# BauerLab/VARSCOT

Measured on AMD Instinct MI355X. Metric: guides/sec (candidate sites/sec alongside) at <=8 mismatches on a 3.0 Gbp reference, higher is better.
Workload: dtype u32

## Files before the change

### include/varscot_hip_debug.h

```cpp
#ifndef VARSCOT_HIP_DEBUG_H
#define VARSCOT_HIP_DEBUG_H

#include "varscot_hip.h"

#ifdef __cplusplus
extern "C" {
#endif

typedef struct {
    uint32_t seed_groups_per_cu;
    uint32_t seed_reserve;
    uint32_t sort_cap;
    uint32_t sort_max_bits;
    int32_t sort_xcd;
    uint32_t sort_debug;
    int32_t sort_optimistic;
    uint32_t sort_slot_cap;
    uint64_t score_chunk;
    int32_t score_slices;
    uint32_t score_slice_shift;
    int32_t seed_shared;
    int32_t seed_group_out;
    int32_t seed_tight;
    int32_t rf_form;
    uint32_t reserved[1];
} vsc_debug_params;

int vsc_ctx_set_debug_params(vsc_ctx *ctx, const vsc_debug_params *params);
int vsc_ctx_get_debug_params(const vsc_ctx *ctx, vsc_debug_params *out);

int vsc_ctx_create_masked(int device_id, const uint32_t *cu_mask, uint32_t n_words, vsc_ctx **out);

void vsc_debug_set_host_timing(int on);

typedef struct {
    int32_t rccl;
    const char *rccl_library;
} vsc_multi_debug_params;
int vsc_multi_create_debug(const int *device_ids, int n, const vsc_multi_debug_params *params, vsc_multi **out);

#ifdef __cplusplus
}
#endif
#endif
```

### varscot_amd/_lib.py

```python
import ctypes as C
import os

import numpy as np

_HERE = os.path.dirname(os.path.abspath(__file__))
LIB_PATH = os.environ.get("VSC_LIB_PATH") or os.path.join(_HERE, "libvarscot_hip.so")

VSC_OK = 0
ERRORS = {-22: "VSC_ERR_INVALID", -12: "VSC_ERR_NOMEM", -5: "VSC_ERR_DEVICE", -34: "VSC_ERR_RANGE",
          -19: "VSC_ERR_NODEVICE"}

HIT_DTYPE = np.dtype([("guide", "<u4"), ("contig", "<u4"), ("pos", "<u4"), ("info", "<u4")])
CONTIG_DTYPE = np.dtype([("offset", "<u8"), ("length", "<u4"), ("reserved", "<u4")])
N_FEATURES = 442
SUMMARY_DTYPE = np.dtype([("mit_sum", "<u8"), ("nm", "<u8", (9,)), ("mit_ub", "<u8"), ("on_target", "<u4"),
                          ("reserved", "<u4")])
assert SUMMARY_DTYPE.itemsize == 96
LOCUS_DTYPE = np.dtype([("contig", "<u4"), ("pos", "<u4"), ("strand", "<u4"), ("reserved", "<u4")])


class SearchParams(C.Structure):
    _fields_ = [("max_mismatches", C.c_uint32), ("has_extra_pam", C.c_uint8), ("extra_pam", C.c_char * 2),
                ("algorithm", C.c_uint8)]


ALGO_AUTO, ALGO_SCAN, ALGO_SEED = 0, 1, 2


class Select(C.Structure):
    _fields_ = [("top_k", C.c_uint32), ("min_score", C.c_uint32), ("reserved", C.c_uint32 * 2)]


SELECT = Select
assert C.sizeof(Select) == 16


class RfModel(C.Structure):
    _fields_ = [("n_trees", C.c_uint32), ("n_nodes", C.c_uint32), ("node_status", C.c_void_p), ("feature", C.c_void_p),
                ("left", C.c_void_p), ("right", C.c_void_p), ("split", C.c_void_p), ("node_class", C.c_void_p)]


class Timing(C.Structure):
    _fields_ = [("scan_ms", C.c_double), ("prep_ms", C.c_double), ("sort_ms", C.c_double),
                ("finalize_ms", C.c_double), ("score_ms", C.c_double), ("total_ms", C.c_double),
                ("index_ms", C.c_double), ("sites", C.c_uint64), ("pairs", C.c_uint64), ("hits", C.c_uint64),
                ("genome_bytes", C.c_uint64), ("passes", C.c_uint32), ("algorithm", C.c_uint32),
                ("sort_bytes", C.c_uint64), ("sort_levels", C.c_uint32), ("sort_bin_bits", C.c_uint32),
                ("read_passes", C.c_uint32), ("sort_fallbacks", C.c_uint32), ("list_entries", C.c_uint64), ("seed_cut", C.c_uint32),
                ("reserved", C.c_uint32)]

    def as_dict(self):
        return {k: getattr(self, k) for k, _ in self._fields_ if k != "reserved"}


class MultiTiming(C.Structure):
    _fields_ = [("search_wall_ms", C.c_double), ("search_ms_max", C.c_double), ("exchange_ms", C.c_double),
                ("merge_ms", C.c_double), ("total_ms", C.c_double), ("hits", C.c_uint64), ("exchanged_bytes", C.c_uint64),
                ("n_devices", C.c_uint32), ("used_rccl", C.c_uint32), ("score_ms_max", C.c_double), ("callback_ms", C.c_double),
                ("batches", C.c_uint32), ("reserved", C.c_uint32)]

    def as_dict(self):
        return {k: getattr(self, k) for k, _ in self._fields_ if k != "reserved"}


class MultiScore(C.Structure):
    _fields_ = [("mode", C.c_uint32), ("reserved", C.c_uint32), ("guide_activity", C.c_void_p), ("model", C.POINTER(RfModel))]


MULTI_SCORE_NONE, MULTI_SCORE_ROWS, MULTI_SCORE_VOTES = 0, 1, 2


class DebugParams(C.Structure):
    _fields_ = [("seed_groups_per_cu", C.c_uint32), ("seed_reserve", C.c_uint32), ("sort_cap", C.c_uint32),
                ("sort_max_bits", C.c_uint32), ("sort_xcd", C.c_int32), ("sort_debug", C.c_uint32),
                ("sort_optimistic", C.c_int32), ("sort_slot_cap", C.c_uint32), ("score_chunk", C.c_uint64),
                ("score_slices", C.c_int32), ("score_slice_shift", C.c_uint32), ("seed_shared", C.c_int32),
                ("seed_group_out", C.c_int32), ("seed_tight", C.c_int32), ("rf_form", C.c_int32),
                ("reserved", C.c_uint32 * 1)]
    SIGNED_DEFAULT = ("sort_xcd", "sort_optimistic", "score_slices", "seed_shared", "seed_group_out", "seed_tight", "rf_form")

    @classmethod
    def defaults(cls):
        d = cls()
        for k in cls.SIGNED_DEFAULT:
            setattr(d, k, -1)
        return d


class MultiDebugParams(C.Structure):
    _fields_ = [("rccl", C.c_int32), ("rccl_library", C.c_char_p)]


BATCH_FN = C.CFUNCTYPE(C.c_int, C.c_void_p, C.c_void_p, C.c_uint32, C.c_uint32)
ROWS_BATCH_FN = C.CFUNCTYPE(C.c_int, C.c_void_p, C.c_void_p, C.c_uint32, C.c_uint32, C.c_void_p)
MULTI_BATCH_FN = C.CFUNCTYPE(C.c_int, C.c_void_p, C.c_void_p, C.c_uint32, C.c_uint32, C.c_void_p)

_u32p = C.POINTER(C.c_uint32)
_vp = C.c_void_p
SYMBOLS = [
    ("vsc_abi_version", C.c_int, []),
    ("vsc_device_count", C.c_int, []),
    ("vsc_ctx_create", C.c_int, [C.c_int, C.POINTER(_vp)]),
    ("vsc_ctx_destroy", C.c_int, [_vp]),
    ("vsc_ctx_release_scratch", C.c_int, [_vp]),
    ("vsc_ctx_set_stream", C.c_int, [_vp, _vp]),
    ("vsc_last_error", C.c_char_p, [_vp]),
    ("vsc_ctx_timing", C.c_int, [_vp, C.POINTER(Timing)]),
    ("vsc_layout_contigs", C.c_uint64, [_vp, C.c_uint32, _vp]),
    ("vsc_planes_init", None, [_vp, _vp, _vp, C.c_uint64]),
    ("vsc_pack_bases", None, [C.c_char_p, C.c_uint64, C.c_uint64, _vp, _vp, _vp]),
    ("vsc_unpack_bases", None, [_vp, _vp, _vp, C.c_uint64, C.c_uint64, _vp]),
    ("vsc_pack_guide", C.c_uint64, [C.c_char_p]),
    ("vsc_genome_load", C.c_int, [_vp, _vp, _vp, _vp, C.c_uint64, C.c_uint64, C.c_uint64, _vp, C.c_uint32,
                                  C.POINTER(_vp)]),
    ("vsc_genome_free", C.c_int, [_vp]),
    ("vsc_genome_build_index", C.c_int, [_vp, _vp, C.POINTER(SearchParams)]),
    ("vsc_genome_index_save", C.c_int, [_vp, _vp, C.c_char_p]),
    ("vsc_genome_index_load", C.c_int, [_vp, _vp, C.c_char_p]),
    ("vsc_genome_device_bytes", C.c_uint64, [_vp]),
    ("vsc_search", C.c_int, [_vp, _vp, _vp, C.c_uint32, C.POINTER(SearchParams), C.POINTER(_vp)]),
    ("vsc_search_stream", C.c_int, [_vp, _vp, _vp, C.c_uint32, C.POINTER(SearchParams), C.c_uint32, BATCH_FN, _vp]),
    ("vsc_search_stream_rows", C.c_int, [_vp, _vp, _vp, C.c_uint32, C.POINTER(SearchParams), C.c_uint32, ROWS_BATCH_FN, _vp]),
    ("vsc_search_summary", C.c_int, [_vp, _vp, _vp, C.c_uint32, C.POINTER(SearchParams), _vp, _vp]),
    ("vsc_search_select", C.c_int, [_vp, _vp, _vp, C.c_uint32, C.POINTER(SearchParams), C.POINTER(Select), _vp, _vp, C.POINTER(_vp)]),
    ("vsc_mit_specificity", C.c_double, [C.c_uint64]),
    ("vsc_hits_count", C.c_uint64, [_vp]),
    ("vsc_hits_data_dev", _vp, [_vp]),
    ("vsc_hits_data", C.c_int, [_vp, C.POINTER(_vp)]),
    ("vsc_hits_copy", C.c_int, [_vp, _vp, C.c_int]),
    ("vsc_hits_merge", C.c_int, [_vp, _vp, C.c_int, _vp, C.c_uint32, C.c_uint32, C.POINTER(_vp)]),
    ("vsc_hits_pack_exchange", C.c_int, [_vp, _vp, _vp, C.c_uint32, _vp, C.c_int, _vp]),
    ("vsc_hits_merge_packed", C.c_int, [_vp, _vp, _vp, C.c_int, _vp, C.c_uint32, C.c_uint32, C.c_uint32, C.POINTER(_vp)]),
    ("vsc_hits_merge_packed_votes", C.c_int, [_vp, _vp, _vp, _vp, C.c_int, _vp, C.c_uint32, C.c_uint32, C.c_uint32, C.POINTER(_vp), _vp, C.c_int]),
    ("vsc_hits_free", C.c_int, [_vp]),
    ("vsc_score_hits", C.c_int, [_vp, _vp, _vp, _vp, C.c_uint32, C.c_uint64, C.c_uint64, _vp, _vp, _vp]),
    ("vsc_score_hits_packed", C.c_int, [_vp, _vp, _vp, _vp, C.c_uint32, C.c_uint64, C.c_uint64, _vp, _vp, _vp]),
    ("vsc_unpack_features", None, [_vp, C.c_uint64, _vp]),
    ("vsc_score_pairs", C.c_int, [_vp, _vp, _vp, _vp, C.c_uint64, _vp, _vp, _vp]),
    ("vsc_multi_create", C.c_int, [C.POINTER(C.c_int), C.c_int, C.POINTER(_vp)]),
    ("vsc_multi_destroy", C.c_int, [_vp]),
    ("vsc_multi_release_scratch", C.c_int, [_vp]),
    ("vsc_multi_size", C.c_int, [_vp]),
    ("vsc_multi_ctx", _vp, [_vp, C.c_int]),
    ("vsc_multi_result_ctx", _vp, [_vp]),
    ("vsc_multi_last_error", C.c_char_p, [_vp]),
    ("vsc_multi_uses_rccl", C.c_int, [_vp]),
    ("vsc_multi_get_timing", C.c_int, [_vp, C.POINTER(MultiTiming)]),
    ("vsc_multi_genome_load", C.c_int, [_vp, _vp, _vp, _vp, C.c_uint64, _vp, C.c_uint32, C.POINTER(_vp)]),
    ("vsc_multi_genome_free", C.c_int, [_vp]),
    ("vsc_multi_genome_build_index", C.c_int, [_vp, _vp, C.POINTER(SearchParams)]),
    ("vsc_multi_search", C.c_int, [_vp, _vp, _vp, C.c_uint32, C.POINTER(SearchParams), C.POINTER(_vp)]),
    ("vsc_multi_search_summary", C.c_int, [_vp, _vp, _vp, C.c_uint32, C.POINTER(SearchParams), _vp, _vp]),
    ("vsc_multi_search_select", C.c_int, [_vp, _vp, _vp, C.c_uint32, C.POINTER(SearchParams), C.POINTER(Select), _vp, _vp, C.POINTER(_vp)]),
    ("vsc_multi_search_stream", C.c_int, [_vp, _vp, _vp, C.c_uint32, C.POINTER(SearchParams), C.c_uint32, C.POINTER(MultiScore), MULTI_BATCH_FN, _vp]),
    ("vsc_windows_build", C.c_int, [C.c_char_p, C.c_uint32, C.c_uint32, C.c_uint32, _vp, _vp, _vp, _vp, _vp, C.c_uint32,
                                    C.POINTER(_vp), C.c_char_p, C.c_size_t]),
    ("vsc_windows_count", C.c_uint32, [_vp]),
    ("vsc_windows_words", C.c_uint64, [_vp]),
    ("vsc_windows_plane", _vp, [_vp, C.c_int]),
    ("vsc_windows_contigs", _vp, [_vp]),
    ("vsc_windows_name", _vp, [_vp, C.c_uint32, C.POINTER(C.c_uint32)]),
    ("vsc_windows_name_offsets", _vp, [_vp]),
    ("vsc_windows_free", None, [_vp]),
    ("vsc_rf_predict", C.c_int, [_vp, C.POINTER(RfModel), _vp, _vp, C.c_uint64, _vp, _vp, _vp]),
    ("vsc_rf_predict_packed", C.c_int, [_vp, C.POINTER(RfModel), _vp, C.c_int, _vp, C.c_uint64, _vp, _vp, _vp]),
    ("vsc_score_classify_hits", C.c_int, [_vp, _vp, _vp, _vp, C.c_uint32, _vp, C.POINTER(RfModel), C.c_uint64, C.c_uint64, _vp, _vp, _vp]),
    ("vsc_sam_order", None, [_vp, C.c_uint64, _vp, _vp]),
]
DEBUG_SYMBOLS = [
    ("vsc_ctx_set_debug_params", C.c_int, [_vp, C.POINTER(DebugParams)]),
    ("vsc_ctx_get_debug_params", C.c_int, [_vp, C.POINTER(DebugParams)]),
    ("vsc_debug_set_host_timing", None, [C.c_int]),
    ("vsc_ctx_create_masked", C.c_int, [C.c_int, _vp, C.c_uint32, C.POINTER(_vp)]),
    ("vsc_multi_create_debug", C.c_int, [C.POINTER(C.c_int), C.c_int, C.POINTER(MultiDebugParams), C.POINTER(_vp)]),
]

_lib = None


class VarscotError(RuntimeError):
    def __init__(self, code, message=""):
        self.code = code
        super().__init__("%s (%d)%s" % (ERRORS.get(code, "VSC_ERR"), code, ": " + message if message else ""))


def lib():
    global _lib
    if _lib is None:
        if not os.path.exists(LIB_PATH):
            raise ImportError(
                "libvarscot_hip.so is not built (%s). Build it with `make -C varscot_amd/csrc` or "
                "`python -c 'import __graft_entry__ as g; g.build()'`; there is no CPU fallback." % LIB_PATH)
        if os.environ.get("VSC_NO_TORCH_PRELOAD") != "1":
            try:
                import torch
            except ImportError:
                pass
        L = C.CDLL(LIB_PATH)
        for name, restype, argtypes in SYMBOLS + DEBUG_SYMBOLS:
            fn = getattr(L, name)
            fn.restype = restype
            fn.argtypes = argtypes
        _lib = L
    return _lib


def check(code, ctx=None):
    if code != VSC_OK:
        msg = ""
        if ctx:
            msg = lib().vsc_last_error(ctx).decode(errors="replace")
        raise VarscotError(code, msg)


def ptr(a):
    if a is None:
        return None
    assert a.flags["C_CONTIGUOUS"]
    return a.ctypes.data_as(C.c_void_p)
```

### varscot_amd/csrc/vsc_api.cpp

```cpp
#include <algorithm>
#include <atomic>
#include <chrono>
#include <cstdlib>
#include <cmath>
#include <cstdio>
#include <cstring>
#include <new>
#include <string>
#include <vector>

#include "vsc_internal.h"
#include "vsc_objects.h"

using namespace vsc;

namespace {

struct HostTimer {
    bool on = vsc::host_timing_on();
    std::chrono::steady_clock::time_point t0 = std::chrono::steady_clock::now();
    void lap(const char *what)
    {
        if (!on) return;
        auto t1 = std::chrono::steady_clock::now();
// ... 11 lines not shown

namespace {

int fail(vsc_ctx *ctx, int code, const char *what, hipError_t e = hipSuccess)
{
    if (ctx) {
        char buf[512];
        if (e != hipSuccess)
            std::snprintf(buf, sizeof buf, "%s: %s", what, hipGetErrorString(e));
        else
            std::snprintf(buf, sizeof buf, "%s", what);
        ctx->err = buf;
    }
    return code;
}

#define VSC_HIP(ctx, call)                                                 \
    do {                                                                   \
        hipError_t e_ = (call);                                            \
        if (e_ != hipSuccess) return fail((ctx), e_ == hipErrorOutOfMemory ? VSC_ERR_NOMEM : VSC_ERR_DEVICE, #call, e_); \
    } while (0)

hipError_t ensure_hl(vsc_ctx *ctx, const vsc_genome *genome)
{
    vsc_genome *g = const_cast<vsc_genome *>(genome);
    if (g->d_hl) return hipSuccess;
    hipError_t e = hipMalloc((void **)&g->d_hl, g->dev_words * sizeof(uint2));
    if (e != hipSuccess) return e;
    g->device_bytes += g->dev_words * sizeof(uint2);
    return launch_interleave(g->d_hi, g->d_lo, g->dev_words, g->d_hl, ctx->stream);
}

hipError_t take_records(vsc_ctx *ctx, vsc_hits *hits, uint64_t n)
{
    const size_t bytes = n * sizeof(vsc_hit);
    int best = -1;
    for (size_t i = 0; i < ctx->spare_records.size(); ++i)
        if (ctx->spare_records[i].cap >= bytes && (best < 0 || ctx->spare_records[i].cap < ctx->spare_records[best].cap))
            best = (int)i;
    if (best >= 0) {
        hits->storage = ctx->spare_records[best];
        ctx->spare_records.erase(ctx->spare_records.begin() + best);
    } else {
        for (auto &b : ctx->spare_records) b.release();
        ctx->spare_records.clear();
        hipError_t e = hits->storage.ensure(bytes);
        if (e != hipSuccess) return e;
    }
    hits->d_records = (vsc_hit *)hits->storage.p;
    return hipSuccess;
}

double hit_probability(unsigned m)
{
    double p = 0, c = 1;
    for (unsigned j = 0; j <= m && j <= 21; ++j) {
        if (j > 0) c = c * (21 - (j - 1)) / j;
        p += c * std::pow(0.75, (double)j) * std::pow(0.25, (double)(21 - j));
    }
    return p;
}

PamMasks pam_masks(int a, int b)
{
    PamMasks m;
    m.ah = (a & 2) ? 0xFFFFFFFFu : 0u;
    m.al = (a & 1) ? 0xFFFFFFFFu : 0u;
    m.bh = (b & 2) ? 0xFFFFFFFFu : 0u;
    m.bl = (b & 1) ? 0xFFFFFFFFu : 0u;
    return m;
}

int base_code(char c)
{
    switch (c) {
    case 'A': case 'a': return 0;
    case 'C': case 'c': return 1;
    case 'G': case 'g': return 2;
    case 'T': case 't': return 3;
    default: return 4;
    }
}

void guide_planes(uint64_t g, uint32_t *h, uint32_t *l)
{
    uint32_t hh = 0, ll = 0;
    for (int i = 0; i < VSC_READ_LEN; ++i) {
        const unsigned c = (unsigned)(g >> (2 * i)) & 3u;
        hh |= (c >> 1) << i;
        ll |= (c & 1u) << i;
    }
    *h = hh;
    *l = ll;
}

}

template <class F> int guarded(vsc_ctx *ctx, F &&body) noexcept
{
    try {
        return body();
    } catch (const std::bad_alloc &) {
        try {
            if (ctx) ctx->err = "out of host memory";
        } catch (...) {
        }
        return VSC_ERR_NOMEM;
    } catch (...) {
        try {
            if (ctx) ctx->err = "unexpected C++ exception";
        } catch (...) {
        }
        return VSC_ERR_DEVICE;
    }
}


extern "C" {

int vsc_abi_version(void) { return VSC_ABI_VERSION; }

int vsc_device_count(void)
{
    int n = 0;
    if (hipGetDeviceCount(&n) != hipSuccess) return 0;
    return n;
}

int vsc_ctx_create(int device_id, vsc_ctx **out) { return vsc_ctx_create_masked(device_id, nullptr, 0, out); }

int vsc_ctx_create_masked(int device_id, const uint32_t *cu_mask, uint32_t n_mask_words, vsc_ctx **out)
{
    if (!out) return VSC_ERR_INVALID;
    *out = nullptr;
    int n = 0;
    if (hipGetDeviceCount(&n) != hipSuccess || n <= 0) return VSC_ERR_NODEVICE;
    if (device_id < 0 || device_id >= n) return VSC_ERR_INVALID;
    vsc_ctx *ctx = new (std::nothrow) vsc_ctx();
    if (!ctx) return VSC_ERR_NOMEM;
    ctx->device = device_id;
    hipDeviceProp_t prop;
    if (hipSetDevice(device_id) != hipSuccess || hipGetDeviceProperties(&prop, device_id) != hipSuccess ||
        (cu_mask && n_mask_words ? hipExtStreamCreateWithCUMask(&ctx->stream, n_mask_words, cu_mask) : hipStreamCreate(&ctx->stream)) != hipSuccess) {
        delete ctx;
        return VSC_ERR_DEVICE;
    }
    ctx->own_stream = true;
    ctx->n_cus = prop.multiProcessorCount;
    for (auto &e : ctx->ev)
        if (hipEventCreate(&e) != hipSuccess) {
            vsc_ctx_destroy(ctx);
            return VSC_ERR_DEVICE;
        }
    *out = ctx;
    return VSC_OK;
}

int vsc_ctx_release_scratch(vsc_ctx *ctx)
{
    if (!ctx) return VSC_ERR_INVALID;
    (void)hipSetDevice(ctx->device);
    (void)hipStreamSynchronize(ctx->stream);
    for (DeviceBuf *b : {&ctx->counters, &ctx->guides, &ctx->score_guides, &ctx->keys_a, &ctx->keys_b, &ctx->vals_a, &ctx->vals_b,
                         &ctx->score_mit, &ctx->score_flags, &ctx->score_feat, &ctx->score_sched, &ctx->sort_segs, &ctx->sort_tabs,
                         &ctx->sort_over, &ctx->seed_off,
                         &ctx->seed_poff, &ctx->seed_lrest, &ctx->sum_rows, &ctx->sum_excl, &ctx->sel_hist, &ctx->sel_tabs, &ctx->sel_keys,
                         &ctx->sel_masks})
        b->release();
    for (auto &b : ctx->spare_records) b.release();
    ctx->spare_records.clear();
    ctx->forest.nodes.release();
    ctx->forest.ranks.release();
    ctx->forest.fingerprint = 0;
    return VSC_OK;
}

int vsc_ctx_destroy(vsc_ctx *ctx)
{
    if (!ctx) return VSC_OK;
    (void)vsc_ctx_release_scratch(ctx);
    for (auto &e : ctx->ev)
        if (e) (void)hipEventDestroy(e);
    if (ctx->own_stream && ctx->stream) (void)hipStreamDestroy(ctx->stream);
    delete ctx;
    return VSC_OK;
}

int vsc_ctx_set_stream(vsc_ctx *ctx, void *hip_stream)
{
    if (!ctx) return VSC_ERR_INVALID;
    if (ctx->own_stream && ctx->stream) {
        (void)hipStreamSynchronize(ctx->stream);
        (void)hipStreamDestroy(ctx->stream);
    }
    ctx->stream = (hipStream_t)hip_stream;
    ctx->own_stream = false;
    return VSC_OK;
}

const char *vsc_last_error(const vsc_ctx *ctx) { return ctx ? ctx->err.c_str() : "null context"; }

int vsc_ctx_set_debug_params(vsc_ctx *ctx, const vsc_debug_params *params)
{
    if (!ctx) return VSC_ERR_INVALID;
    ctx->dbg = params ? *params : default_debug_params();
    return VSC_OK;
}

int vsc_ctx_get_debug_params(const vsc_ctx *ctx, vsc_debug_params *out)
{
    if (!ctx || !out) return VSC_ERR_INVALID;
    *out = ctx->dbg;
    return VSC_OK;
}

void vsc_debug_set_host_timing(int on) { vsc::g_host_timing.store(on ? 1 : 0, std::memory_order_relaxed); }

int vsc_ctx_timing(const vsc_ctx *ctx, vsc_timing *out)
{
    if (!ctx || !out) return VSC_ERR_INVALID;
    *out = ctx->timing;
    return VSC_OK;
}

int vsc_genome_load(vsc_ctx *ctx, const uint32_t *hi, const uint32_t *lo, const uint32_t *nmask, uint64_t first_word,
                    uint64_t n_words, uint64_t own_words, const vsc_contig *contigs, uint32_t n_contigs,
                    vsc_genome **out)
{
    return guarded(ctx, [&]() -> int {
    if (!ctx || !out) return VSC_ERR_INVALID;
    *out = nullptr;
    ctx->err.clear();
    if (!hi || !lo || !nmask || !contigs || n_contigs == 0 || n_words == 0 || own_words == 0 || own_words > n_words)
        return fail(ctx, VSC_ERR_INVALID, "vsc_genome_load: null or empty argument");
    if (own_words < n_words && own_words % kTileWords != 0)
        return fail(ctx, VSC_ERR_INVALID, "vsc_genome_load: a shard followed by halo words must own a multiple of 64 words");
    const uint64_t n_tiles = (own_words + kTileWords - 1) / kTileWords;
    const uint64_t dev_words = std::max<uint64_t>(n_tiles * kTileWords, n_words) + kPadWords;
    if ((first_word + dev_words) * 32 >= (1ull << 32) - 4096)
        return fail(ctx, VSC_ERR_RANGE, "vsc_genome_load: genome exceeds the 32-bit position space (4 Gbases)");
    std::vector<uint32_t> off(n_contigs), end(n_contigs);
    for (uint32_t c = 0; c < n_contigs; ++c) {
        const uint64_t e = contigs[c].offset + contigs[c].length;
        if (e >= (1ull << 32) - 4096) return fail(ctx, VSC_ERR_RANGE, "vsc_genome_load: contig table exceeds 4 Gbases");
        if (c > 0 && contigs[c].offset < contigs[c - 1].offset + contigs[c - 1].length + 1)
            return fail(ctx, VSC_ERR_INVALID, "vsc_genome_load: contigs must be ascending and separated by >= 1 N position");
        off[c] = (uint32_t)contigs[c].offset;
        end[c] = (uint32_t)e;
    }
    VSC_HIP(ctx, hipSetDevice(ctx->device));
    vsc_genome *g = new (std::nothrow) vsc_genome();
    if (!g) return fail(ctx, VSC_ERR_NOMEM, "vsc_genome_load: out of host memory");
    g->ctx = ctx;
    g->first_word = first_word;
    g->own_words = own_words;
    g->dev_words = dev_words;
    g->n_tiles = (uint32_t)n_tiles;
    g->n_contigs = n_contigs;
    const size_t pb = dev_words * sizeof(uint32_t), cb = (size_t)n_contigs * sizeof(uint32_t);
    hipError_t e = hipSuccess;
    auto step = [&](hipError_t r) {
        if (e == hipSuccess) e = r;
    };
    step(hipMalloc((void **)&g->d_hi, pb));
    step(hipMalloc((void **)&g->d_lo, pb));
    step(hipMalloc((void **)&g->d_nm, pb));
    step(hipMalloc((void **)&g->d_contig_off, cb));
    step(hipMalloc((void **)&g->d_contig_end, cb));
    if (e == hipSuccess) {
        step(hipMemsetAsync(g->d_hi, 0, pb, ctx->stream));
        step(hipMemsetAsync(g->d_lo, 0, pb, ctx->stream));
        step(hipMemsetAsync(g->d_nm, 0xFF, pb, ctx->stream));
        step(hipMemcpyAsync(g->d_hi, hi, n_words * sizeof(uint32_t), hipMemcpyHostToDevice, ctx->stream));
        step(hipMemcpyAsync(g->d_lo, lo, n_words * sizeof(uint32_t), hipMemcpyHostToDevice, ctx->stream));
        step(hipMemcpyAsync(g->d_nm, nmask, n_words * sizeof(uint32_t), hipMemcpyHostToDevice, ctx->stream));
        step(hipMemcpyAsync(g->d_contig_off, off.data(), cb, hipMemcpyHostToDevice, ctx->stream));
        step(hipMemcpyAsync(g->d_contig_end, end.data(), cb, hipMemcpyHostToDevice, ctx->stream));
        step(hipStreamSynchronize(ctx->stream));
    }
    if (e != hipSuccess) {
        vsc_genome_free(g);
        return fail(ctx, e == hipErrorOutOfMemory ? VSC_ERR_NOMEM : VSC_ERR_DEVICE, "vsc_genome_load", e);
    }
    g->device_bytes = 3 * pb + 2 * cb;
    *out = g;
    return VSC_OK;
    });
}

}

int vsc::genome_table_only(vsc_ctx *ctx, const vsc_contig *contigs, uint32_t n_contigs, vsc_genome **out)
{
    if (!ctx || !out || !contigs || n_contigs == 0) return VSC_ERR_INVALID;
    *out = nullptr;
    std::vector<uint32_t> off(n_contigs), end(n_contigs);
    for (uint32_t c = 0; c < n_contigs; ++c) {
        off[c] = (uint32_t)contigs[c].offset;
        end[c] = (uint32_t)(contigs[c].offset + contigs[c].length);
    }
    VSC_HIP(ctx, hipSetDevice(ctx->device));
    vsc_genome *g = new (std::nothrow) vsc_genome();
    if (!g) return fail(ctx, VSC_ERR_NOMEM, "out of host memory");
    g->ctx = ctx;
    g->n_contigs = n_contigs;
    const size_t cb = (size_t)n_contigs * sizeof(uint32_t);
    hipError_t e = hipMalloc((void **)&g->d_contig_off, cb);
    if (e == hipSuccess) e = hipMalloc((void **)&g->d_contig_end, cb);
    if (e == hipSuccess) e = hipMemcpy(g->d_contig_off, off.data(), cb, hipMemcpyHostToDevice);
    if (e == hipSuccess) e = hipMemcpy(g->d_contig_end, end.data(), cb, hipMemcpyHostToDevice);
    if (e != hipSuccess) {
        vsc_genome_free(g);
        return fail(ctx, e == hipErrorOutOfMemory ? VSC_ERR_NOMEM : VSC_ERR_DEVICE, "contig table upload", e);
    }
    g->device_bytes = 2 * cb;
    *out = g;
    return VSC_OK;
}

extern "C" {

int vsc_genome_free(vsc_genome *g)
{
    if (!g) return VSC_OK;
    if (g->ctx) (void)hipSetDevice(g->ctx->device);
    for (void *p : {(void *)g->d_hi, (void *)g->d_lo, (void *)g->d_nm, (void *)g->d_contig_off, (void *)g->d_contig_end, (void *)g->d_hl,
                    (void *)g->d_ix_chunk_tab, (void *)g->d_ix_vert, (void *)g->d_ix_sites, (void *)g->d_ix_edge})
        if (p) (void)hipFree(p);
    delete g;
    return VSC_OK;
}

uint64_t vsc_genome_device_bytes(const vsc_genome *g) { return g ? g->device_bytes + g->index_bytes : 0; }

namespace {
// ... 392 lines not shown
        if (!why.empty()) return fail(ctx, VSC_ERR_RANGE, ("vsc_genome_build_index: " + why).c_str());
        return fail(ctx, e == hipErrorOutOfMemory ? VSC_ERR_NOMEM : VSC_ERR_DEVICE, "vsc_genome_build_index", e);
    }
    ctx->timing.index_ms = genome->index_ms;
    return VSC_OK;
    });
}

int vsc_genome_index_save(vsc_ctx *ctx, const vsc_genome *genome, const char *path)
{
    return guarded(ctx, [&]() -> int {
    if (!ctx || !genome || genome->ctx != ctx || !path) return VSC_ERR_INVALID;
    ctx->err.clear();
    if (!genome->has_index) return fail(ctx, VSC_ERR_INVALID, "vsc_genome_index_save: the genome has no seed index (vsc_genome_build_index)");
    VSC_HIP(ctx, hipSetDevice(ctx->device));
    IndexFileHeader h{};
    std::memcpy(h.magic, kIndexMagic, sizeof h.magic);
    h.abi = VSC_ABI_VERSION;
    h.seg_bases = kSegBases;
    h.sliced_chunk = kSlicedChunk;
    h.sliced_sites = kSlicedSites;
    h.layout = (uint8_t)kIndexLayout;
    h.sites = genome->index_sites;
    h.own_words = genome->own_words;
    h.vert_bytes = genome->ix_vert_bytes;
    h.edge_words = genome->ix_edge_words;
    h.chunks = genome->ix_chunks;
    h.n_contigs = genome->n_contigs;
    h.has_extra_pam = genome->index_has_extra_pam;
    h.extra_pam[0] = genome->index_extra_pam[0];
    h.extra_pam[1] = genome->index_extra_pam[1];
    VSC_HIP(ctx, genome_fingerprint(ctx, genome, &h.fingerprint));
    FileCloser fc{std::fopen(path, "wb")};
    if (!fc.f) return fail(ctx, VSC_ERR_INVALID, (std::string("vsc_genome_index_save: cannot write ") + path).c_str());
    bool ok = std::fwrite(&h, sizeof h, 1, fc.f) == 1;
    std::vector<char> host(kIndexIoChunk);
    const uint64_t S = genome->index_sites;
    if (ok) VSC_HIP(ctx, index_io(fc.f, genome->d_ix_sites, 3 * S * sizeof(uint2), true, host, &ok));
    if (ok) VSC_HIP(ctx, index_io(fc.f, genome->d_ix_edge, h.edge_words * sizeof(uint32_t), true, host, &ok));
    if (ok) VSC_HIP(ctx, index_io(fc.f, genome->d_ix_chunk_tab, (uint64_t)h.chunks * sizeof(uint4), true, host, &ok));
    if (ok) VSC_HIP(ctx, index_io(fc.f, genome->d_ix_vert, h.vert_bytes, true, host, &ok));
    if (ok) ok = std::fflush(fc.f) == 0;
    if (!ok) return fail(ctx, VSC_ERR_DEVICE, (std::string("vsc_genome_index_save: write to ") + path + " failed").c_str());
    return VSC_OK;
    });
}

int vsc_genome_index_load(vsc_ctx *ctx, vsc_genome *genome, const char *path)
{
    return guarded(ctx, [&]() -> int {
    if (!ctx || !genome || genome->ctx != ctx || !path) return VSC_ERR_INVALID;
    ctx->err.clear();
    VSC_HIP(ctx, hipSetDevice(ctx->device));
    const auto t0 = std::chrono::steady_clock::now();
    FileCloser fc{std::fopen(path, "rb")};
    if (!fc.f) return fail(ctx, VSC_ERR_INVALID, (std::string("vsc_genome_index_load: cannot read ") + path).c_str());
    IndexFileHeader h{};
    if (std::fread(&h, sizeof h, 1, fc.f) != 1 || std::memcmp(h.magic, kIndexMagic, sizeof h.magic) != 0)
        return fail(ctx, VSC_ERR_INVALID, (std::string("vsc_genome_index_load: ") + path + " is not a seed index file").c_str());
    if (h.abi != VSC_ABI_VERSION || h.seg_bases != (uint32_t)kSegBases || h.sliced_chunk != (uint32_t)kSlicedChunk ||
        h.sliced_sites != (uint32_t)kSlicedSites || h.layout != (uint8_t)kIndexLayout)
        return fail(ctx, VSC_ERR_INVALID, "vsc_genome_index_load: the file was written by another version of the library");
    uint64_t fp = 0;
    VSC_HIP(ctx, genome_fingerprint(ctx, genome, &fp));
    if (h.own_words != genome->own_words || h.n_contigs != genome->n_contigs || h.fingerprint != fp)
        return fail(ctx, VSC_ERR_INVALID, "vsc_genome_index_load: the file belongs to another genome");
    const uint64_t S = h.sites;
    if (3 * S >= (1ull << 32) || h.edge_words != (3 * S + 31) / 32 + 1 || h.vert_bytes % (kVertWords * sizeof(uint32_t)) != 0)
        return fail(ctx, VSC_ERR_INVALID, "vsc_genome_index_load: inconsistent header");
    {
        const long at = std::ftell(fc.f);
        const uint64_t want = (uint64_t)sizeof h + 3 * S * sizeof(uint2) + h.edge_words * sizeof(uint32_t) +
                              (uint64_t)h.chunks * sizeof(uint4) + h.vert_bytes;
        if (at < 0 || std::fseek(fc.f, 0, SEEK_END) != 0) return fail(ctx, VSC_ERR_INVALID, "vsc_genome_index_load: cannot seek in the file");
        const long size = std::ftell(fc.f);
        if (size < 0 || (uint64_t)size != want || std::fseek(fc.f, at, SEEK_SET) != 0)
            return fail(ctx, VSC_ERR_INVALID, (std::string("vsc_genome_index_load: ") + path + " is truncated or does not match its header").c_str());
    }
    free_index(genome);
    hipError_t e = hipSuccess;
    auto step = [&](hipError_t r) {
        if (e == hipSuccess) e = r;
    };
    const uint64_t sb = std::max<uint64_t>(3 * S, 1) * sizeof(uint2), eb = h.edge_words * sizeof(uint32_t);
    const uint64_t cb = std::max<uint64_t>(h.chunks, 1) * sizeof(uint4), vb = std::max<uint64_t>(h.vert_bytes, kVertWords * sizeof(uint32_t));
    step(hipMalloc((void **)&genome->d_ix_sites, sb));
    step(hipMalloc((void **)&genome->d_ix_edge, eb));
    step(hipMalloc((void **)&genome->d_ix_chunk_tab, cb));
    step(hipMalloc((void **)&genome->d_ix_vert, vb));
    bool ok = true;
    std::vector<char> host(kIndexIoChunk);
    if (e == hipSuccess) step(index_io(fc.f, genome->d_ix_sites, 3 * S * sizeof(uint2), false, host, &ok));
    if (e == hipSuccess && ok) step(index_io(fc.f, genome->d_ix_edge, eb, false, host, &ok));
    if (e == hipSuccess && ok) step(index_io(fc.f, genome->d_ix_chunk_tab, (uint64_t)h.chunks * sizeof(uint4), false, host, &ok));
    if (e == hipSuccess && ok) step(index_io(fc.f, genome->d_ix_vert, h.vert_bytes, false, host, &ok));
    if (e != hipSuccess || !ok) {
        free_index(genome);
        if (e != hipSuccess) return fail(ctx, e == hipErrorOutOfMemory ? VSC_ERR_NOMEM : VSC_ERR_DEVICE, "vsc_genome_index_load", e);
        return fail(ctx, VSC_ERR_INVALID, (std::string("vsc_genome_index_load: ") + path + " is truncated").c_str());
    }
    {
        std::vector<uint32_t> ctab((size_t)h.chunks * 4);
        if (h.chunks) VSC_HIP(ctx, hipMemcpy(ctab.data(), genome->d_ix_chunk_tab, ctab.size() * sizeof(uint32_t), hipMemcpyDeviceToHost));
        std::string why;
        if (!chunk_table_ok(ctab, S, h.vert_bytes, &why)) {
            free_index(genome);
            return fail(ctx, VSC_ERR_INVALID, (std::string("vsc_genome_index_load: ") + path + " is damaged (" + why + ")").c_str());
        }
        class_counts(genome, ctab);
    }
    genome->ix_chunks = h.chunks;
    genome->ix_vert_bytes = vb;
    genome->ix_edge_words = h.edge_words;
    genome->index_sites = S;
    genome->sites = S;
    genome->has_index = true;
    genome->index_has_extra_pam = h.has_extra_pam;
    genome->index_extra_pam[0] = h.extra_pam[0];
    genome->index_extra_pam[1] = h.extra_pam[1];
    genome->index_bytes = sb + eb + cb + vb;
    genome->index_ms = std::chrono::duration<double, std::milli>(std::chrono::steady_clock::now() - t0).count();
    ctx->timing.index_ms = genome->index_ms;
    return VSC_OK;
    });
}

}

namespace {

unsigned ceil_log2(uint64_t x)
{
    unsigned b = 0;
    while (b < 63 && (1ull << b) < x) ++b;
    return b;
}

struct SortRows {
    uint32_t *side_src = nullptr;
    DeviceBuf *side_other = nullptr;
    const uint2 *guides = nullptr;
    uint32_t guide_first = 0;
    uint4 *rows = nullptr;
    uint64_t rows_first = 0;
};

struct SortInfo {
    unsigned levels = 0;
    unsigned bin_bits = 0;
    uint64_t bytes = 0;
    unsigned slot_fallbacks = 0;
};

hipError_t bin_sort(vsc_ctx *ctx, const vsc_genome *genome, std::vector<SortSeg> segs, uint64_t *src, uint64_t *other,
                    unsigned key_bits, unsigned pos_pad, uint32_t pos_base, vsc_hit *out, hipEvent_t ev_sorted, SortInfo *info,
                    DeviceBuf *other_buf = nullptr, bool *slots = nullptr, const SortRows *rows = nullptr)
{
    uint32_t *side_src = rows ? rows->side_src : nullptr, *side_other = nullptr;
    hipStream_t st = ctx->stream;
    unsigned rem = key_bits;
    bool sorted_marked = false;
    const vsc_debug_params &dbg = ctx->dbg;
    uint64_t sort_cap = kSortCap;
    unsigned max_bits = kSortMaxBinBits;
    if (dbg.sort_cap) sort_cap = std::min<uint64_t>(kSortCap, std::max<uint32_t>(16, dbg.sort_cap));
    if (dbg.sort_max_bits) max_bits = std::min<unsigned>(kSortMaxBinBits, std::max<uint32_t>(1, dbg.sort_max_bits));
    uint64_t slot_cap = dbg.sort_slot_cap ? dbg.sort_slot_cap : (sort_cap + sort_cap / 4 + 15) / 16 * 16;
    slot_cap = std::max<uint64_t>(slot_cap, 16);
    for (unsigned level = 1; !segs.empty(); ++level) {
        if (level > 48) return hipErrorUnknown;
        uint64_t n_max = 0, n_all = 0;
        for (const SortSeg &s : segs) {
            n_max = std::max<uint64_t>(n_max, s.n_in);
            n_all += s.n_in;
        }
        unsigned bits = 0;
        if (n_max > sort_cap) {
            if (rem == 0) return hipErrorUnknown;
            const uint64_t want = std::max<uint64_t>(1, sort_cap * 7 / 10);
            bits = std::min<unsigned>({std::max(1u, ceil_log2((n_max + want - 1) / want)), max_bits, rem});
            while (bits > 1 && ((uint64_t)segs.size() << bits) > (1ull << 22)) --bits;
        }
        const size_t n_segs = segs.size();
        const size_t n_bins = n_segs << bits;
        bool use_slots = level == 1 && bits && slots && other_buf && (dbg.sort_optimistic == 1 || (dbg.sort_optimistic != 0 && *slots));
        if (level == 1 && bits && other_buf) {
            uint64_t span = 1;
            for (const SortSeg &sg : segs) span = std::max<uint64_t>(span, sg.out_off + sg.n_in);
            const uint64_t slot_records = (uint64_t)n_bins * slot_cap;
            if (use_slots && dbg.sort_optimistic != 1) {
                size_t free_b = 0, total_b = 0;
                if (hipMemGetInfo(&free_b, &total_b) != hipSuccess) free_b = 0;
                const uint64_t room = (uint64_t)free_b + other_buf->cap;
                const uint64_t slot_bytes = slot_records * (sizeof(uint64_t) + (rows ? sizeof(uint32_t) : 0));
                if (slot_records > 4 * n_all + (1ull << 20) || slot_bytes + (1ull << 30) > room + (rows ? rows->side_other->cap : 0)) {
                    use_slots = false;
                    *slots = false;
                }
            }
            hipError_t ge = other_buf->ensure((size_t)(use_slots ? std::max(slot_records, span) : span) * sizeof(uint64_t));
            if (ge == hipErrorOutOfMemory && use_slots) {
                (void)hipGetLastError();
                use_slots = false;
                *slots = false;
                ge = other_buf->ensure((size_t)span * sizeof(uint64_t));
            }
            if (ge != hipSuccess) return ge;
            other = (uint64_t *)other_buf->p;
            if (rows) {
                VSC_TRY(rows->side_other->ensure(other_buf->cap / sizeof(uint64_t) * sizeof(uint32_t)));
                side_other = (uint32_t *)rows->side_other->p;
            }
        }
        std::vector<uint32_t> &tile0 = ctx->host_tile0;
        tile0.assign(n_segs + 1, 0);
        uint64_t tiles = 0;
        for (size_t i = 0; i < n_segs; ++i) {
            tile0[i] = (uint32_t)tiles;
            tiles += (segs[i].n_in + kSortTile - 1) / kSortTile;
        }
        if (tiles >= (1ull << 31)) return hipErrorInvalidValue;
        tile0[n_segs] = (uint32_t)tiles;
        const size_t seg_bytes = (n_segs * sizeof(SortSeg) + 255) / 256 * 256;
        VSC_TRY(ctx->sort_segs.ensure(seg_bytes + tile0.size() * sizeof(uint32_t)));
        SortSeg *d_segs = (SortSeg *)ctx->sort_segs.p;
        uint32_t *d_tile0 = (uint32_t *)((char *)ctx->sort_segs.p + seg_bytes);
        ctx->host_segs = segs;
        VSC_TRY(hipMemcpyAsync(d_segs, ctx->host_segs.data(), n_segs * sizeof(SortSeg), hipMemcpyHostToDevice, st));
        VSC_TRY(hipMemcpyAsync(d_tile0, tile0.data(), tile0.size() * sizeof(uint32_t), hipMemcpyHostToDevice, st));
        VSC_TRY(ctx->sort_over.ensure(256 + n_bins * sizeof(SortSeg)));
        uint32_t *d_n_over = (uint32_t *)ctx->sort_over.p;
        if (bits) VSC_TRY(ctx->sort_tabs.ensure(3 * n_bins * sizeof(uint32_t)));
        uint32_t flags[3] = {0, 0, 0};
        for (;;) {
            if (dbg.sort_debug)
                std::fprintf(stderr, "[vsc sort] level %u: %zu segments, %llu records, largest %llu, %u bits (of %u left), cap %llu%s\n", level,
                             n_segs, (unsigned long long)n_all, (unsigned long long)n_max, bits, rem, (unsigned long long)sort_cap,
                             use_slots ? ", slot mode" : "");
            VSC_TRY(hipMemsetAsync(d_n_over, 0, 3 * sizeof(uint32_t), st));
            FinArgs f{};
            f.segs = d_segs;
            f.n_segs = (uint32_t)n_segs;
            f.src = src;
            f.side_src = side_src;
            if (rows) {
                f.guides = rows->guides;
                f.guide_first = rows->guide_first;
                f.rows = rows->rows;
                f.rows_first = rows->rows_first;
            }
            if (bits) {
                SortArgs a{};
                a.segs = d_segs;
                a.seg_tile0 = d_tile0;
                a.n_segs = (uint32_t)n_segs;
                a.n_tiles = (uint32_t)tiles;
                a.in = src;
                a.out = other;
                a.side_in = rows ? side_src : nullptr;
                a.side_out = rows ? side_other : nullptr;
                a.hist = (uint32_t *)ctx->sort_tabs.p;
                a.cursor = a.hist + n_bins;
                a.bin_start = a.cursor + n_bins;
                a.bin_bits = bits;
                a.bin_shift = kRecPosShift + pos_pad + rem - bits;
                if (dbg.sort_xcd != 0 && tiles >= 64) a.xcd_tiles = (uint32_t)((tiles + 7) / 8);
                if (use_slots) {
                    a.hist = a.cursor;
                    a.slot_cap = (uint32_t)slot_cap;
                    a.overflow = d_n_over + 2;
                    VSC_TRY(hipMemsetAsync(a.cursor, 0, n_bins * sizeof(uint32_t), st));
                    VSC_TRY(launch_bin_partition(a, st));
                    VSC_TRY(launch_bin_scan(a, st));
                } else {
                    VSC_TRY(hipMemsetAsync(a.hist, 0, n_bins * sizeof(uint32_t), st));
                    VSC_TRY(launch_bin_hist(a, st));
                    VSC_TRY(launch_bin_scan(a, st));
                    if (dbg.sort_debug >= 2) {
                        std::vector<uint32_t> h(n_bins);
                        VSC_TRY(hipMemcpyAsync(h.data(), a.hist, n_bins * sizeof(uint32_t), hipMemcpyDeviceToHost, st));
                        VSC_TRY(hipStreamSynchronize(st));
                        for (size_t i = 0; i < n_segs; ++i) {
                            std::vector<uint64_t> recs(segs[i].n_in);
                            VSC_TRY(hipMemcpy(recs.data(), src + segs[i].in_off, recs.size() * sizeof(uint64_t), hipMemcpyDeviceToHost));
                            std::vector<uint32_t> want((size_t)1 << bits, 0);
                            for (uint64_t r : recs) {
                                if (r >> 63) continue;
                                want[(r >> a.bin_shift) & (((uint64_t)1 << bits) - 1)]++;
                            }
                            for (size_t b = 0; b < want.size(); ++b)
                                if (want[b] != h[(i << bits) + b])
                                    std::fprintf(stderr, "[vsc sort]   seg %zu (in_off %llu n %u) bin %zu: device %u host %u\n", i,
                                                 (unsigned long long)segs[i].in_off, segs[i].n_in, b, h[(i << bits) + b], want[b]);
                        }
                    }
                    VSC_TRY(launch_bin_partition(a, st));
                }
                f.src = other;
                f.side_src = side_other;
                f.hist = a.hist;
                f.bin_start = a.bin_start;
                f.bin_bits = bits;
                f.slot_cap = a.slot_cap;
                f.overflow = a.overflow;
            }
            if (!sorted_marked && ev_sorted) {
                VSC_TRY(hipEventRecord(ev_sorted, st));
                sorted_marked = true;
            }
            const unsigned rem_after = rem - bits;
            f.sub_bits = std::min<unsigned>(rows ? kSortSubBitsRows : kSortSubBits, rem_after);
            f.sub_shift = kRecPosShift + pos_pad + rem_after - f.sub_bits;
            f.pos_pad = pos_pad;
            f.pos_base = pos_base;
            f.low_bits = rem_after - f.sub_bits;
            f.over = (SortSeg *)((char *)ctx->sort_over.p + 256);
            f.over_cap = (uint32_t)std::min<size_t>(n_bins, 0xFFFFFFFFu);
            f.n_over = d_n_over;
            f.cursor = d_n_over + 1;
            f.cap = (uint32_t)sort_cap;
            f.contig_off = genome->d_contig_off;
            f.n_contigs = genome->n_contigs;
            f.out = out;
            VSC_TRY(launch_bin_finalize(f, 2 * ctx->n_cus, st));
            if (bits) {
                VSC_TRY(hipMemcpyAsync(flags, d_n_over, sizeof flags, hipMemcpyDeviceToHost, st));
                VSC_TRY(hipStreamSynchronize(st));
                if (use_slots && flags[2]) {
                    use_slots = false;
                    *slots = false;
                    if (info) {
                        info->slot_fallbacks++;
                        info->bytes += 16 * n_all;
                    }
                    continue;
                }
            }
            if (info && bits) {
                if (info->levels == 0) info->bin_bits = bits;
                info->levels++;
                info->bytes += (use_slots ? 16 : 24) * n_all;
            }
            if (info) info->bytes += 24 * n_all;
            if (info && rows) info->bytes += (bits ? 8 : 0) * n_all + (4 + 12 + 64) * n_all;
            break;
        }
        if (!bits) break;
        rem -= bits;
        const uint32_t n_over = flags[0];
        if (n_over == 0) break;
        segs.resize(n_over);
        VSC_TRY(hipMemcpyAsync(segs.data(), (char *)ctx->sort_over.p + 256, (size_t)n_over * sizeof(SortSeg), hipMemcpyDeviceToHost, st));
        VSC_TRY(hipStreamSynchronize(st));
        std::swap(src, other);
        std::swap(side_src, side_other);
        if (rows && !side_other) {
            uint64_t span = 1;
            for (const SortSeg &sg : segs) span = std::max<uint64_t>(span, sg.out_off + sg.n_in);
            VSC_TRY(rows->side_other->ensure(span * sizeof(uint32_t)));
            side_other = (uint32_t *)rows->side_other->p;
        }
    }
    return hipSuccess;
}

hipError_t result_room(vsc_ctx *ctx, vsc_hits *hits, uint64_t used, uint64_t n, uint64_t projected)
{
    const uint64_t need = used + n;
    if (hits->storage.p && hits->storage.cap >= need * sizeof(vsc_hit)) return hipSuccess;
    if (used == 0) {
        if (hits->storage.p) {
            ctx->spare_records.push_back(hits->storage);
            hits->storage = DeviceBuf{};
        }
        VSC_TRY(take_records(ctx, hits, std::max(need, projected)));
        return hipSuccess;
    }
    DeviceBuf bigger;
    VSC_TRY(bigger.ensure(std::max(need, projected) * sizeof(vsc_hit)));
    hipError_t e = hipMemcpyAsync(bigger.p, hits->storage.p, used * sizeof(vsc_hit), hipMemcpyDeviceToDevice, ctx->stream);
    if (e == hipSuccess) e = hipStreamSynchronize(ctx->stream);
    if (e != hipSuccess) {
        bigger.release();
        return e;
    }
    hits->storage.release();
    hits->storage = bigger;
    hits->d_records = (vsc_hit *)bigger.p;
    return hipSuccess;
}

struct PassFound {
    HostTimer ht;
    int algo = 0, n_parts = 0;
    uint32_t max_mm = 0, guide_base = 0;
    uint64_t cap = 0, n = 0;
    std::vector<SortSeg> segs;
    unsigned key_bits = 0, pos_pad = 0;
    uint32_t pos_base = 0;
    bool bases = false;
    bool selected = false;
    std::vector<uint64_t> sel_off;
};

uint32_t neighbours(int k) { return k < 0 ? 0u : (k == 0 ? 1u : (k == 1 ? 22u : 211u)); }

SeedPlan seed_cut(const vsc_genome *genome, const uint32_t *gp, uint32_t n_guides, uint32_t m, int n_cus, const vsc_debug_params &dbg,
                  int *k2_max)
{
    SeedPlan plan{};
    plan.max_mm = m;
    ScanArgs pa{};
    vsc_search_params ip{};
    ip.has_extra_pam = genome->index_has_extra_pam;
    ip.extra_pam[0] = genome->index_extra_pam[0];
    ip.extra_pam[1] = genome->index_extra_pam[1];
    fill_pam(pa, &ip);
    plan.n_pam = pa.n_pam;
    plan.pam_codes = pam_code_set(pa);
    plan.tight = dbg.seed_tight != 0;
    if (!plan.tight) {
        plan.k0 = plan.k1 = m / kSegments;
        *k2_max = (int)plan.k0;
    } else {
        uint32_t left_reads[kSeedClasses][VSC_MAX_MISMATCHES + 1] = {};
        int left_max = -1;
        for (uint32_t i = 0; i < n_guides; ++i) {
            const uint32_t x = gp[2 * (size_t)i], l = gp[2 * (size_t)i + 1];
            const uint32_t mine = (((x >> 21) & 1u) << 3) | (((l >> 21) & 1u) << 2) | (((x >> 22) & 1u) << 1) | ((l >> 22) & 1u);
            for (uint32_t c = 0; c < plan.n_pam; ++c) {
                const uint32_t diff = mine ^ ((plan.pam_codes >> (4 * c)) & 15u);
                const uint32_t spent = ((diff & 12u) ? 1u : 0u) + ((diff & 3u) ? 1u : 0u);
                if (spent > m) continue;
                left_reads[c][m - spent]++;
                left_max = std::max(left_max, (int)(m - spent));
            }
        }
        double cost[9];
        double chunks_all = 0, sites_all = 0;
        uint64_t reads_any = 0;
        for (uint32_t c = 0; c < plan.n_pam; ++c) {
            chunks_all += (double)genome->ix_class_chunks[c] / kSegments;
            sites_all += (double)genome->ix_class_sites[c];
            uint64_t reads_c = 0;
            for (int left = 0; left <= (int)m; ++left) reads_c += left_reads[c][left];
            reads_any = std::max(reads_any, reads_c);
        }
        const double block_bytes = (double)kVertWords * 4 / kSlicedSites;
        for (int cut = 0; cut < 9; ++cut) {
            const int k0 = cut % 3, k1 = cut / 3;
            cost[cut] = -1;
            if (left_max - k0 - k1 - 2 > 2) continue;
            double bytes = 0, visits = 0;
            for (uint32_t c = 0; c < plan.n_pam; ++c) {
                double e2 = 0;
                for (int left = 0; left <= (int)m; ++left) e2 += (double)left_reads[c][left] * neighbours(left - k0 - k1 - 2);
                const double per_list = e2 / kBucketsPerSeg;
                bytes += (1.0 - std::exp(-per_list)) * (double)genome->ix_class_sites[c] * block_bytes;
                visits += per_list * (double)genome->ix_class_chunks[c] / kSegments;
            }
            for (int k : {k0, k1}) {
                const double per_list = (double)reads_any * neighbours(k) / kBucketsPerSeg;
                bytes += (1.0 - std::exp(-per_list)) * sites_all * block_bytes;
                visits += per_list * chunks_all;
            }
            cost[cut] = std::max(bytes / 4.2e12, visits * 215.0 / ((double)n_cus * 4 * 2.0e9));
        }
        int best = -1;
        for (int cut = 0; cut < 9; ++cut)
            if (cost[cut] >= 0 && (best < 0 || cost[cut] < cost[best])) best = cut;
        const int forced = dbg.seed_tight >= 1 ? dbg.seed_tight - 1 : -1;
        if (forced >= 0 && forced < 9 && cost[forced] >= 0) best = forced;
        if (best < 0) best = 4 * (int)(m ? (m - 1) / kSegments : 0u);
        plan.k0 = (uint32_t)(best % 3);
        plan.k1 = (uint32_t)(best / 3);
        *k2_max = std::min<int>(2, (int)m - (int)plan.k0 - (int)plan.k1 - 2);
    }
    plan.n_nbr = neighbours(std::max<int>(std::max<int>((int)plan.k0, (int)plan.k1), *k2_max));
    return plan;
}

hipError_t seed_plan(vsc_ctx *ctx, const vsc_genome *genome, const uint32_t *gp, uint32_t n_guides, const PassFound &f, SeedArgs &sa,
                     int *n_groups, bool *shared)
{
    int k2_max = 0;
    const SeedPlan plan = seed_cut(genome, gp, n_guides, f.max_mm, ctx->n_cus, ctx->dbg, &k2_max);
    const uint64_t n_pairs = (uint64_t)n_guides * (neighbours((int)plan.k0) + neighbours((int)plan.k1) + plan.n_pam * neighbours(k2_max));
    const uint64_t list_cap = n_pairs + (uint64_t)kLists * (kGuideUnroll - 1) + 2 * kGuideUnroll;
    VSC_TRY(ctx->seed_off.ensure((kLists + 1) * sizeof(uint32_t)));
    VSC_TRY(ctx->seed_poff.ensure((kLists + 1) * sizeof(uint32_t)));
    VSC_TRY(ctx->seed_lrest.ensure(list_cap * sizeof(uint2)));
    VSC_TRY(hipMemsetAsync(ctx->seed_lrest.p, 0xFF, list_cap * sizeof(uint2), ctx->stream));
    VSC_TRY(launch_seed_lists((const uint2 *)ctx->guides.p, n_guides, plan, (uint32_t *)ctx->seed_off.p, (uint32_t *)ctx->seed_poff.p,
                              (uint2 *)ctx->seed_lrest.p, ctx->stream));
    VSC_TRY(hipEventRecord(ctx->ev[7], ctx->stream));
    sa.chunk_tab = genome->d_ix_chunk_tab;
    sa.n_chunks = genome->ix_chunks;
    sa.vert = genome->d_ix_vert;
    sa.list_rest = (const uint2 *)ctx->seed_lrest.p;
    sa.sites = genome->d_ix_sites;
    sa.edge_bits = genome->d_ix_edge;
    sa.guides = (const uint2 *)ctx->guides.p;
    sa.poff = (const uint32_t *)ctx->seed_poff.p;
    sa.max_mm = f.max_mm;
    sa.k_half = f.max_mm / 2;
    sa.k_seg0 = plan.k0;
    sa.k_seg1 = plan.k1;
    sa.contig_end = genome->d_contig_end;
    sa.n_contigs = genome->n_contigs;
    sa.counters = (unsigned long long *)ctx->counters.p;
    sa.n_parts = (uint32_t)f.n_parts;
    uint32_t groups_per_cu = kSlicedWavesPerSimd;
    if (ctx->dbg.seed_groups_per_cu) groups_per_cu = ctx->dbg.seed_groups_per_cu;
    *shared = (uint64_t)n_guides * neighbours((int)std::max(plan.k0, plan.k1)) / kBucketsPerSeg >= 72;
    if (ctx->dbg.seed_shared >= 0) *shared = ctx->dbg.seed_shared == 1;
    const uint32_t n_grabs = (sa.n_chunks + kSlicedGrab - 1) / kSlicedGrab;
    const uint32_t n_waves_max = (uint32_t)ctx->n_cus * groups_per_cu * kWavesPerGroup;
    const uint32_t n_waves = std::max<uint32_t>(1, std::min<uint32_t>(n_waves_max, *shared ? n_grabs * kWavesPerGroup : n_grabs));
    *n_groups = (int)((n_waves + kWavesPerGroup - 1) / kWavesPerGroup);
    sa.group_out = *shared && ctx->dbg.seed_group_out != 0 ? 1u : 0u;
    const uint32_t owners = sa.group_out ? (uint32_t)*n_groups : (uint32_t)*n_groups * kWavesPerGroup;
    const uint64_t per_wave = f.cap / ((uint64_t)owners * 8 * f.n_parts);
    uint32_t want_reserve = (uint32_t)std::min<uint64_t>(f.n_parts > 8 ? (sa.group_out ? 1024 : 128) : 1024, std::max<uint64_t>(kWave, per_wave));
    if (ctx->dbg.seed_reserve) want_reserve = std::min<uint32_t>(1024, std::max<uint32_t>(kWave, ctx->dbg.seed_reserve));
    sa.reserve_log2 = 6;
    while ((2u << sa.reserve_log2) <= want_reserve) ++sa.reserve_log2;
    sa.reserve = 1u << sa.reserve_log2;
    sa.pos_pad = f.pos_pad;
    sa.pos_base = f.pos_base;
    uint64_t part_cap = f.cap / f.n_parts + f.cap / f.n_parts / 7 + 4096;
    part_cap = std::max<uint64_t>(part_cap, (uint64_t)(1.2 * genome->seen_rate[f.max_mm] * std::min<uint32_t>(n_guides, kRegionReads)) + 4096);
    sa.part_cap = part_cap + (uint64_t)owners * sa.reserve;
    return hipSuccess;
}

int find_pass(vsc_ctx *ctx, const vsc_genome *genome, const uint64_t *guides, uint32_t n_guides, uint32_t guide_base,
              const vsc_search_params *params, bool keep_bases, vsc_timing &t, PassFound &f)
{
    const int algo = (int)t.algorithm;
    const uint32_t m = params->max_mismatches;
    f.algo = algo;
    f.max_mm = m;
    f.guide_base = guide_base;
    f.bases = keep_bases;
    const uint32_t n_pad = (n_guides + kGuideUnroll - 1) / kGuideUnroll * kGuideUnroll;
    std::vector<uint32_t> gp((size_t)(n_pad + kGuideUnroll) * 2, 0xFFFFFFFFu);
    for (uint32_t i = 0; i < n_guides; ++i) guide_planes(guides[i], &gp[2 * (size_t)i], &gp[2 * (size_t)i + 1]);
    VSC_HIP(ctx, ctx->guides.ensure(gp.size() * sizeof(uint32_t)));
    VSC_HIP(ctx, ctx->counters.ensure(kCounterWords * sizeof(unsigned long long)));
    VSC_HIP(ctx, hipEventRecord(ctx->ev[0], ctx->stream));
    VSC_HIP(ctx, hipMemcpyAsync(ctx->guides.p, gp.data(), gp.size() * sizeof(uint32_t), hipMemcpyHostToDevice, ctx->stream));

    const double own_bases = (double)genome->n_tiles * kTileBases;
    const double sites_est = genome->sites ? (double)genome->sites : own_bases / 4;
    f.cap = (uint64_t)(1.5 * sites_est * n_guides * hit_probability(m)) + (1u << 20);
    const double seen_rate = genome->seen_rate[m];
    if (algo == VSC_ALGO_SCAN) f.cap = std::max<uint64_t>(f.cap, (uint64_t)(1.2 * seen_rate * n_guides) + 4096);
    unsigned long long cnt[kCntPart + 4 * kParts] = {};
    f.n_parts = (int)((n_guides + kRegionReads - 1) / kRegionReads);
    f.pos_base = (uint32_t)(genome->first_word * 32);
    const unsigned pos_bits = std::max(1u, ceil_log2((uint64_t)genome->dev_words * 32));
    f.pos_pad = pos_bits < 32 ? 32 - pos_bits : 0;
    f.key_bits = pos_bits + 1 + ceil_log2(std::min<uint32_t>(n_guides, kRegionReads));

    ScanArgs a{};
    SeedArgs sa{};
    int n_groups = 1;
    bool seed_shared = false;
    if (algo == VSC_ALGO_SCAN) {
        fill_pam(a, params);
        fill_genome(a, ctx, genome);
        a.guides = (const uint4 *)ctx->guides.p;
        a.n_guides_padded = n_pad;
        a.max_mm = m;
        a.k_half = m / 2;
        n_groups = scan_groups(ctx, a.n_tiles);
        t.genome_bytes += (uint64_t)genome->n_tiles * kTileWords * 3 * sizeof(uint32_t);
        VSC_HIP(ctx, hipEventRecord(ctx->ev[7], ctx->stream));
    } else {
        VSC_HIP(ctx, seed_plan(ctx, genome, gp.data(), n_guides, f, sa, &n_groups, &seed_shared));
        f.cap = sa.part_cap * f.n_parts;
    }

    f.ht.lap("prep enqueue");
    uint32_t list_total = 0;
    for (unsigned tries = 0;; ++tries) {
        if (algo == VSC_ALGO_SEED && (sa.part_cap >= (1ull << 32) - (1u << 20) || sa.part_cap >= ((uint64_t)sa.reserve << 20) - sa.reserve))
            return fail(ctx, VSC_ERR_RANGE, "vsc_search: more than 2^32 hits in a block of 64 reads");
        VSC_HIP(ctx, ctx->keys_a.ensure(f.cap * sizeof(uint64_t)));
        VSC_HIP(ctx, hipMemsetAsync(ctx->counters.p, 0, kCounterWords * sizeof(unsigned long long), ctx->stream));
        VSC_HIP(ctx, hipEventRecord(ctx->ev[1], ctx->stream));
        if (algo == VSC_ALGO_SCAN) {
            VSC_HIP(ctx, ctx->vals_a.ensure(f.cap * sizeof(uint32_t)));
            a.hit_keys = (uint64_t *)ctx->keys_a.p;
            a.hit_vals = (uint32_t *)ctx->vals_a.p;
            a.hit_cap = f.cap;
            VSC_HIP(ctx, launch_scan(a, n_groups, false, ctx->stream));
        } else {
            sa.hit_recs = (uint64_t *)ctx->keys_a.p;
            if (keep_bases) {
                VSC_HIP(ctx, ctx->vals_a.ensure(f.cap * sizeof(uint32_t)));
                sa.hit_side = (uint32_t *)ctx->vals_a.p;
            }
            VSC_HIP(ctx, launch_seed_sliced(sa, n_groups, seed_shared, ctx->stream));
        }
        VSC_HIP(ctx, hipEventRecord(ctx->ev[2], ctx->stream));
        VSC_HIP(ctx, hipMemcpyAsync(cnt, ctx->counters.p, sizeof cnt, hipMemcpyDeviceToHost, ctx->stream));
        if (algo == VSC_ALGO_SEED)
            VSC_HIP(ctx, hipMemcpyAsync(&list_total, (const uint32_t *)ctx->seed_poff.p + kLists, sizeof list_total, hipMemcpyDeviceToHost, ctx->stream));
        VSC_HIP(ctx, hipStreamSynchronize(ctx->stream));
        f.ht.lap("search kernel + sync");
        t.passes++;
        if (!cnt[kCntOverflow]) break;
        if (tries >= 2) return fail(ctx, VSC_ERR_DEVICE, "vsc_search: hit buffer overflowed repeatedly");
        if (algo == VSC_ALGO_SEED) {
            uint64_t need = 0;
            for (int q = 0; q < f.n_parts; ++q) need = std::max<uint64_t>(need, cnt[kCntPart + 4 * q] + cnt[kCntPart + 4 * q + 2]);
            sa.part_cap = need + (need >> 6) + 4096 + (uint64_t)(sa.group_out ? n_groups : n_groups * kWavesPerGroup) * sa.reserve;
            f.cap = sa.part_cap * f.n_parts;
        } else {
            f.cap = cnt[kCntHits] + (cnt[kCntHits] >> 6) + 4096;
        }
    }
    float ms = 0;
    VSC_HIP(ctx, hipEventElapsedTime(&ms, ctx->ev[0], ctx->ev[7]));
    t.prep_ms += ms;
    VSC_HIP(ctx, hipEventElapsedTime(&ms, ctx->ev[1], ctx->ev[2]));
    t.scan_ms += ms;

    if (algo == VSC_ALGO_SCAN) {
        genome->sites = cnt[kCntSites];
        t.sites = cnt[kCntSites];
        t.pairs += cnt[kCntSites] * n_guides;
        f.n = cnt[kCntHits];
        genome->seen_rate[m] = (double)f.n / n_guides;
        if (f.n >= (1ull << 32)) return fail(ctx, VSC_ERR_RANGE, "vsc_search: more than 2^32 hits in one scan pass (split the read set)");
        if (f.n > 0) f.segs.push_back(SortSeg{0, 0, 0, (uint32_t)f.n, guide_base});
    } else {
        t.list_entries = list_total;
        t.seed_cut = sa.k_seg0 | (sa.k_seg1 << 4);
        t.sites = genome->index_sites;
        t.pairs += cnt[kCntSites];
        t.genome_bytes += cnt[kCntVisited] * kVertWords * sizeof(uint32_t) / kSlicedSites;
        double fullest = 0;
        for (int q = 0; q < f.n_parts; ++q) {
            const uint64_t placed = cnt[kCntPart + 4 * q], real = placed - cnt[kCntPart + 4 * q + 1];
            fullest = std::max(fullest, (double)placed / std::min<uint32_t>(kRegionReads, n_guides - (uint32_t)q * kRegionReads));
            if (placed) f.segs.push_back(SortSeg{(uint64_t)q * sa.part_cap, (uint64_t)q * sa.part_cap, f.n, (uint32_t)placed,
                                                 guide_base + (uint32_t)q * kRegionReads});
            f.n += real;
        }
        genome->seen_rate[m] = fullest;
    }
    t.hits += f.n;
    return VSC_OK;
}

hipError_t end_pass(vsc_ctx *ctx, PassFound &f, const char *lap, vsc_timing &t)
{
    VSC_TRY(hipEventRecord(ctx->ev[4], ctx->stream));
    VSC_TRY(hipStreamSynchronize(ctx->stream));
    f.ht.lap(lap);
    float ms = 0;
    VSC_TRY(hipEventElapsedTime(&ms, ctx->ev[3], ctx->ev[4]));
    t.finalize_ms += ms;
    VSC_TRY(hipEventElapsedTime(&ms, ctx->ev[0], ctx->ev[4]));
    t.total_ms += ms;
    t.read_passes++;
    return hipSuccess;
}

int sort_pass(vsc_ctx *ctx, const vsc_genome *genome, PassFound &f, vsc_hits *hits, uint64_t used, uint64_t projected, vsc_timing &t)
{
    SortInfo info;
    if (f.n > 0) {
        uint64_t *src = (uint64_t *)ctx->keys_a.p, *other = nullptr;
        if (f.algo == VSC_ALGO_SCAN && !f.selected) {
            VSC_HIP(ctx, ctx->keys_b.ensure(f.cap * sizeof(uint64_t)));
            const unsigned bits0 = ceil_log2((uint64_t)f.n_parts);
            const size_t n_bins = (size_t)1 << bits0;
            VSC_HIP(ctx, ctx->sort_segs.ensure(512));
            VSC_HIP(ctx, ctx->sort_tabs.ensure(3 * n_bins * sizeof(uint32_t)));
            const uint32_t tile0[2] = {0u, (uint32_t)((f.n + kSortTile - 1) / kSortTile)};
            VSC_HIP(ctx, hipMemcpyAsync(ctx->sort_segs.p, f.segs.data(), sizeof(SortSeg), hipMemcpyHostToDevice, ctx->stream));
            VSC_HIP(ctx, hipMemcpyAsync((char *)ctx->sort_segs.p + 256, tile0, sizeof tile0, hipMemcpyHostToDevice, ctx->stream));
            SortArgs l0{};
            l0.segs = (const SortSeg *)ctx->sort_segs.p;
            l0.seg_tile0 = (const uint32_t *)((char *)ctx->sort_segs.p + 256);
            l0.n_segs = 1;
            l0.n_tiles = tile0[1];
            l0.pair_keys = (const uint64_t *)ctx->keys_a.p;
            l0.pair_vals = (const uint32_t *)ctx->vals_a.p;
            l0.out = (uint64_t *)ctx->keys_b.p;
            l0.hist = (uint32_t *)ctx->sort_tabs.p;
            l0.cursor = l0.hist + n_bins;
            l0.bin_start = l0.cursor + n_bins;
            l0.bin_bits = bits0;
            l0.bin_shift = kRecKeyBits;
            l0.pos_pad = f.pos_pad;
            l0.pos_base = f.pos_base;
            VSC_HIP(ctx, hipMemsetAsync(l0.hist, 0, n_bins * sizeof(uint32_t), ctx->stream));
            VSC_HIP(ctx, launch_bin_hist(l0, ctx->stream));
            VSC_HIP(ctx, launch_bin_scan(l0, ctx->stream));
            VSC_HIP(ctx, launch_bin_partition(l0, ctx->stream));
            std::vector<uint32_t> tabs(3 * n_bins);
            VSC_HIP(ctx, hipMemcpyAsync(tabs.data(), l0.hist, tabs.size() * sizeof(uint32_t), hipMemcpyDeviceToHost, ctx->stream));
            VSC_HIP(ctx, hipStreamSynchronize(ctx->stream));
            f.segs.clear();
            for (int q = 0; q < f.n_parts; ++q) {
                const uint32_t count = tabs[q], start = tabs[2 * n_bins + q];
                if (count) f.segs.push_back(SortSeg{start, start, start, count, f.guide_base + (uint32_t)q * kRegionReads});
            }
            src = (uint64_t *)ctx->keys_b.p;
            other = (uint64_t *)ctx->keys_a.p;
            info.bytes += 12 * f.n + 20 * f.n;
        }
        for (SortSeg &s : f.segs) s.final_off += used;
        f.ht.lap("sort buffers");
        VSC_HIP(ctx, result_room(ctx, hits, used, f.n, projected));
        f.ht.lap("record storage");
        bool *slots = f.algo == VSC_ALGO_SEED && !f.selected ? &genome->sort_slots_ok[f.max_mm] : nullptr;
        SortRows rows;
        if (f.bases) {
            if (ctx->score_feat.ensure(f.n * VSC_PACKED_FEATURE_BYTES) != hipSuccess) {
                (void)hipGetLastError();
                for (auto &b : ctx->spare_records) b.release();
                ctx->spare_records.clear();
                for (DeviceBuf *b : {&ctx->score_mit, &ctx->score_flags, &ctx->score_sched, &ctx->keys_b, &ctx->vals_b}) b->release();
                VSC_HIP(ctx, ctx->score_feat.ensure(f.n * VSC_PACKED_FEATURE_BYTES));
            }
            rows.side_src = (uint32_t *)ctx->vals_a.p;
            rows.side_other = &ctx->vals_b;
            rows.guides = (const uint2 *)ctx->guides.p;
            rows.guide_first = f.guide_base;
            rows.rows = (uint4 *)ctx->score_feat.p;
            rows.rows_first = used;
        }
        VSC_HIP(ctx, bin_sort(ctx, genome, std::move(f.segs), src, other, f.key_bits, f.pos_pad, f.pos_base, hits->d_records, ctx->ev[3],
                              &info, f.algo == VSC_ALGO_SEED || f.selected ? &ctx->keys_b : nullptr, slots, f.bases ? &rows : nullptr));
    } else {
        VSC_HIP(ctx, hipEventRecord(ctx->ev[3], ctx->stream));
    }
    VSC_HIP(ctx, end_pass(ctx, f, "sort + finalize + sync", t));
    float ms = 0;
    VSC_HIP(ctx, hipEventElapsedTime(&ms, ctx->ev[2], ctx->ev[3]));
    t.sort_ms += ms;
    t.sort_levels = std::max(t.sort_levels, info.levels);
    t.sort_bin_bits = std::max(t.sort_bin_bits, info.bin_bits);
    t.sort_bytes += info.bytes;
    t.sort_fallbacks += info.slot_fallbacks;
    return VSC_OK;
}

int summarize_pass(vsc_ctx *ctx, PassFound &f, bool excluded, vsc_timing &t, bool last = true)
{
    std::vector<SumSeg> ss;
    std::vector<uint32_t> tile0(1, 0);
    for (const SortSeg &sg : f.segs) {
        ss.push_back(SumSeg{sg.in_off, sg.n_in, sg.guide_base - f.guide_base});
        tile0.push_back(tile0.back() + (sg.n_in + kSumTile - 1) / kSumTile);
    }
    SummaryArgs a{};
    if (!ss.empty()) {
        const size_t tile0_at = (ss.size() * sizeof(SumSeg) + 255) / 256 * 256;
        VSC_HIP(ctx, ctx->sort_segs.ensure(tile0_at + tile0.size() * sizeof(uint32_t)));
        VSC_HIP(ctx, hipMemcpyAsync(ctx->sort_segs.p, ss.data(), ss.size() * sizeof(SumSeg), hipMemcpyHostToDevice, ctx->stream));
        VSC_HIP(ctx, hipMemcpyAsync((char *)ctx->sort_segs.p + tile0_at, tile0.data(), tile0.size() * sizeof(uint32_t),
                                    hipMemcpyHostToDevice, ctx->stream));
        a.recs = (const uint64_t *)ctx->keys_a.p;
        a.vals = f.algo == VSC_ALGO_SCAN ? (const uint32_t *)ctx->vals_a.p : nullptr;
        a.segs = (const SumSeg *)ctx->sort_segs.p;
        a.seg_tile0 = (const uint32_t *)((char *)ctx->sort_segs.p + tile0_at);
        a.n_segs = (uint32_t)ss.size();
        a.n_tiles = tile0.back();
        a.pos_pad = f.pos_pad;
        a.pos_base = f.pos_base;
        a.excl = excluded ? (const uint64_t *)ctx->sum_excl.p + f.guide_base : nullptr;
        a.out = (unsigned long long *)ctx->sum_rows.p + (size_t)f.guide_base * kSumWords;
    }
    VSC_HIP(ctx, hipEventRecord(ctx->ev[3], ctx->stream));
    VSC_HIP(ctx, launch_summary(a, ctx->stream));
    if (last) VSC_HIP(ctx, end_pass(ctx, f, "summary + sync", t));
    else VSC_HIP(ctx, hipStreamSynchronize(ctx->stream));
    return VSC_OK;
}

int select_pass(vsc_ctx *ctx, PassFound &f, uint32_t n_reads, const vsc_select &sel, bool excluded)
{
    f.selected = true;
    if (f.n == 0) return VSC_OK;
    hipStream_t st = ctx->stream;
    std::vector<SumSeg> ss;
    std::vector<uint32_t> tile0(1, 0);
    for (const SortSeg &sg : f.segs) {
        ss.push_back(SumSeg{sg.in_off, sg.n_in, sg.guide_base - f.guide_base});
        tile0.push_back(tile0.back() + (sg.n_in + kSumTile - 1) / kSumTile);
    }
    const size_t tile0_at = (ss.size() * sizeof(SumSeg) + 255) / 256 * 256;
    VSC_HIP(ctx, ctx->sort_segs.ensure(tile0_at + tile0.size() * sizeof(uint32_t)));
    VSC_HIP(ctx, hipMemcpyAsync(ctx->sort_segs.p, ss.data(), ss.size() * sizeof(SumSeg), hipMemcpyHostToDevice, st));
    VSC_HIP(ctx, hipMemcpyAsync((char *)ctx->sort_segs.p + tile0_at, tile0.data(), tile0.size() * sizeof(uint32_t), hipMemcpyHostToDevice, st));
    const size_t words = ((size_t)n_reads + 63) / 64 * 64;
    VSC_HIP(ctx, ctx->sel_tabs.ensure(4 * words * sizeof(uint32_t) + 2 * words * sizeof(uint64_t)));
    VSC_HIP(ctx, ctx->sel_hist.ensure((size_t)n_reads * kSelBins * sizeof(uint32_t)));
    VSC_HIP(ctx, ctx->vals_b.ensure((size_t)tile0.back() * kSumTile * sizeof(uint32_t)));
    SelectArgs a{};
    a.recs = (const uint64_t *)ctx->keys_a.p;
    a.vals = f.algo == VSC_ALGO_SCAN ? (const uint32_t *)ctx->vals_a.p : nullptr;
    a.segs = (const SumSeg *)ctx->sort_segs.p;
    a.seg_tile0 = (const uint32_t *)((char *)ctx->sort_segs.p + tile0_at);
    a.n_segs = (uint32_t)ss.size();
    a.n_tiles = tile0.back();
    a.pos_pad = f.pos_pad;
    a.pos_base = f.pos_base;
    a.excl = excluded ? (const uint64_t *)ctx->sum_excl.p + f.guide_base : nullptr;
    a.min_score = sel.min_score;
    a.top_k = sel.top_k;
    a.n_reads = n_reads;
    a.tiles_per_block = std::min<uint32_t>(kSelMaxTilesPerBlock, std::max<uint32_t>(kSelMinTilesPerBlock, a.n_tiles / (16u * (uint32_t)ctx->n_cus)));
    a.score = (uint32_t *)ctx->vals_b.p;
    a.hist = (uint32_t *)ctx->sel_hist.p;
    a.thr = (uint32_t *)ctx->sel_tabs.p;
    a.count = a.thr + words;
    a.cursor = a.count + words;
    a.thr_region = a.cursor + words;
    uint64_t *d_off = (uint64_t *)(a.thr_region + words);
    a.cand_off = d_off;
    a.surv_off = d_off + words;
    VSC_HIP(ctx, hipMemsetAsync(a.hist, 0, (size_t)n_reads * kSelBins * sizeof(uint32_t), st));
    VSC_HIP(ctx, hipMemsetAsync(a.cursor, 0, words * sizeof(uint32_t), st));
    VSC_HIP(ctx, hipMemsetAsync(a.thr_region, 0xFF, words * sizeof(uint32_t), st));
    VSC_HIP(ctx, launch_select_score(a, st));
    VSC_HIP(ctx, launch_select_threshold(a, st));
    std::vector<uint32_t> count(n_reads);
    VSC_HIP(ctx, hipMemcpyAsync(count.data(), a.count, (size_t)n_reads * sizeof(uint32_t), hipMemcpyDeviceToHost, st));
    VSC_HIP(ctx, hipStreamSynchronize(st));
    f.ht.lap("select: scores + thresholds + sync");
    f.sel_off.assign(2 * words, 0);
    uint64_t n_cand = 0, n_surv = 0;
    for (uint32_t i = 0; i < n_reads; ++i) {
        f.sel_off[i] = n_cand;
        f.sel_off[words + i] = n_surv;
        n_cand += count[i];
        n_surv += sel.top_k ? std::min<uint32_t>(count[i], sel.top_k) : count[i];
    }
    f.segs.clear();
    for (uint32_t q = 0; q * (uint32_t)kRegionReads < n_reads; ++q) {
        const uint64_t begin = f.sel_off[words + (size_t)q * kRegionReads];
        const uint32_t next = (q + 1) * (uint32_t)kRegionReads;
        const uint64_t end = next < n_reads ? f.sel_off[words + next] : n_surv;
        if (end - begin >= (1ull << 32)) return fail(ctx, VSC_ERR_RANGE, "vsc_search_select: more than 2^32 selected hits in a block of 64 reads");
        if (end > begin) f.segs.push_back(SortSeg{begin, begin, begin, (uint32_t)(end - begin), f.guide_base + q * (uint32_t)kRegionReads});
    }
    f.n = n_surv;
    f.cap = n_surv;
    if (n_surv == 0) return VSC_OK;
    VSC_HIP(ctx, ctx->sel_keys.ensure(n_cand * sizeof(uint64_t)));
    VSC_HIP(ctx, ctx->sel_masks.ensure(n_cand * sizeof(uint32_t)));
    a.cand_key = (uint64_t *)ctx->sel_keys.p;
    a.cand_mask = (uint32_t *)ctx->sel_masks.p;
    a.out = (uint64_t *)ctx->keys_a.p;
    VSC_HIP(ctx, hipMemcpyAsync(d_off, f.sel_off.data(), f.sel_off.size() * sizeof(uint64_t), hipMemcpyHostToDevice, st));
    VSC_HIP(ctx, launch_select_compact(a, st));
    VSC_HIP(ctx, launch_select_resolve(a, st));
    return VSC_OK;
}

int excluded_loci(vsc_ctx *ctx, const vsc_genome *genome, const vsc_locus *exclude, uint32_t n_guides, const char *who, std::vector<uint64_t> &excl)
{
    if (!exclude || !n_guides) return VSC_OK;
    std::vector<uint32_t> off(genome->n_contigs), end(genome->n_contigs);
    if (genome->n_contigs) {
        VSC_HIP(ctx, hipMemcpy(off.data(), genome->d_contig_off, off.size() * sizeof(uint32_t), hipMemcpyDeviceToHost));
        VSC_HIP(ctx, hipMemcpy(end.data(), genome->d_contig_end, end.size() * sizeof(uint32_t), hipMemcpyDeviceToHost));
    }
    excl.assign(n_guides, ~0ull);
    for (uint32_t i = 0; i < n_guides; ++i) {
        const vsc_locus &l = exclude[i];
        if (l.contig == UINT32_MAX) continue;
        if (l.contig >= genome->n_contigs || l.strand > 1)
            return fail(ctx, VSC_ERR_INVALID, (std::string(who) + ": excluded locus outside the genome's contigs or strands").c_str());
        if (l.pos >= end[l.contig] - off[l.contig]) continue;
        excl[i] = (uint64_t)l.strand << 32 | (off[l.contig] + l.pos);
    }
    return VSC_OK;
}

int upload_summary_state(vsc_ctx *ctx, uint32_t n_guides, bool rows, const std::vector<uint64_t> &excl)
{
    if (!n_guides) return VSC_OK;
    if (rows) {
        const size_t row_bytes = (size_t)n_guides * sizeof(vsc_guide_summary);
        VSC_HIP(ctx, ctx->sum_rows.ensure(row_bytes));
        VSC_HIP(ctx, hipMemsetAsync(ctx->sum_rows.p, 0, row_bytes, ctx->stream));
    }
    if (!excl.empty()) {
        VSC_HIP(ctx, ctx->sum_excl.ensure(excl.size() * sizeof(uint64_t)));
        VSC_HIP(ctx, hipMemcpyAsync(ctx->sum_excl.p, excl.data(), excl.size() * sizeof(uint64_t), hipMemcpyHostToDevice, ctx->stream));
    }
    return VSC_OK;
}

int search_setup(vsc_ctx *ctx, const vsc_genome *genome, const uint64_t *guides, uint32_t n_guides,
                 const vsc_search_params *params, const char *who, vsc_timing *t)
{
    ctx->err.clear();
    if (!genome || !params || (n_guides && !guides)) return fail(ctx, VSC_ERR_INVALID, (std::string(who) + ": null argument").c_str());
    if (genome->ctx != ctx) return fail(ctx, VSC_ERR_INVALID, (std::string(who) + ": genome belongs to another context").c_str());
    if (params->max_mismatches > VSC_MAX_MISMATCHES)
        return fail(ctx, VSC_ERR_INVALID, "Maximum number of mismatches must lie between 0 and 8.");
    if (params->algorithm > VSC_ALGO_SEED) return fail(ctx, VSC_ERR_INVALID, (std::string(who) + ": unknown algorithm").c_str());
    if (n_guides >= (1u << 31)) return fail(ctx, VSC_ERR_RANGE, (std::string(who) + ": too many reads").c_str());
    VSC_HIP(ctx, hipSetDevice(ctx->device));
    *t = vsc_timing{};
    t->index_ms = ctx->timing.index_ms;
    const double own_bases = (double)genome->n_tiles * kTileBases;
    int algo = params->algorithm;
    if (algo == VSC_ALGO_AUTO) {
        const bool worth_building = (double)n_guides * own_bases >= 2.0e10;
        algo = (index_matches(genome, params) || worth_building) ? VSC_ALGO_SEED : VSC_ALGO_SCAN;
    }
    if (n_guides && algo == VSC_ALGO_SEED && !index_matches(genome, params)) {
        std::string why;
        hipError_t e = build_index(ctx, const_cast<vsc_genome *>(genome), params, &why);
        if (e != hipSuccess) {
            if (params->algorithm == VSC_ALGO_SEED || why.empty())
                return fail(ctx, e == hipErrorOutOfMemory ? VSC_ERR_NOMEM : VSC_ERR_DEVICE,
                            why.empty() ? "vsc_search: building the seed index" : why.c_str(), why.empty() ? e : hipSuccess);
            algo = VSC_ALGO_SCAN;
        } else {
            t->index_ms = genome->index_ms;
        }
    }
    t->algorithm = (uint32_t)algo;
    return VSC_OK;
}

template <class Deliver>
int stream_batches(vsc_ctx *ctx, const vsc_genome *genome, const uint64_t *guides, uint32_t n_guides, const vsc_search_params *params,
                   uint32_t batch_reads, bool rows, const char *who, bool have_callback, Deliver &&deliver)
{
    return guarded(ctx, [&]() -> int {
    if (!ctx) return VSC_ERR_INVALID;
    vsc_timing t{};
    const int rc = search_setup(ctx, genome, guides, n_guides, params, who, &t);
    if (rc != VSC_OK) return rc;
    if (!have_callback) return fail(ctx, VSC_ERR_INVALID, (std::string(who) + ": null callback").c_str());
    if (batch_reads == 0 || batch_reads > (uint32_t)kMaxPassReads) batch_reads = kMaxPassReads;
    for (uint32_t first = 0; first < n_guides; first += batch_reads) {
        const uint32_t count = std::min<uint32_t>(batch_reads, n_guides - first);
        vsc_hits *hits = new (std::nothrow) vsc_hits();
        if (!hits) return fail(ctx, VSC_ERR_NOMEM, (std::string(who) + ": out of host memory").c_str());
        hits->ctx = ctx;
        PassFound f;
        int prc = find_pass(ctx, genome, guides + first, count, first, params, rows && t.algorithm == VSC_ALGO_SEED, t, f);
        if (prc == VSC_OK) prc = sort_pass(ctx, genome, f, hits, 0, 0, t);
        if (prc == VSC_OK) {
            hits->n = f.n;
            if (f.n == 0) hits->host_valid = true;
            ctx->timing = t;
            ctx->timing.score_ms = 0;
            prc = deliver(hits, first, count, t);
            if (prc != VSC_OK && ctx->err.empty()) ctx->err = std::string(who) + ": the batch callback failed";
        }
        vsc_hits_free(hits);
        if (prc != VSC_OK) return prc;
    }
    ctx->timing = t;
    return VSC_OK;
    });
}

}

extern "C" {

int vsc_search(vsc_ctx *ctx, const vsc_genome *genome, const uint64_t *guides, uint32_t n_guides,
               const vsc_search_params *params, vsc_hits **out)
{
    return guarded(ctx, [&]() -> int {
    if (!ctx || !out) return VSC_ERR_INVALID;
    *out = nullptr;
    vsc_timing t{};
    const int rc = search_setup(ctx, genome, guides, n_guides, params, "vsc_search", &t);
    if (rc != VSC_OK) return rc;
    vsc_hits *hits = new (std::nothrow) vsc_hits();
    if (!hits) return fail(ctx, VSC_ERR_NOMEM, "vsc_search: out of host memory");
    hits->ctx = ctx;
    uint64_t used = 0;
    for (uint32_t first = 0; first < n_guides; first += kMaxPassReads) {
        const uint32_t count = std::min<uint32_t>(kMaxPassReads, n_guides - first);
        const uint64_t projected = first ? (uint64_t)((double)used / first * n_guides * 1.02) + 4096 : 0;
        PassFound f;
        int prc = find_pass(ctx, genome, guides + first, count, first, params, false, t, f);
        if (prc == VSC_OK) prc = sort_pass(ctx, genome, f, hits, used, projected, t);
        if (prc != VSC_OK) {
            vsc_hits_free(hits);
            return prc;
        }
        used += f.n;
    }
    hits->n = used;
    if (used == 0) hits->host_valid = true;
    ctx->timing = t;
    *out = hits;
    return VSC_OK;
    });
}

int vsc_search_summary(vsc_ctx *ctx, const vsc_genome *genome, const uint64_t *guides, uint32_t n_guides,
                       const vsc_search_params *params, const vsc_locus *exclude, vsc_guide_summary *out)
{
    return guarded(ctx, [&]() -> int {
    if (!ctx) return VSC_ERR_INVALID;
    if (n_guides && !out) return fail(ctx, VSC_ERR_INVALID, "vsc_search_summary: null argument");
    vsc_timing t{};
    const int rc = search_setup(ctx, genome, guides, n_guides, params, "vsc_search_summary", &t);
    if (rc != VSC_OK) return rc;
    std::vector<uint64_t> excl;
    const int erc = excluded_loci(ctx, genome, exclude, n_guides, "vsc_search_summary", excl);
    if (erc != VSC_OK) return erc;
    const int urc = upload_summary_state(ctx, n_guides, true, excl);
    if (urc != VSC_OK) return urc;
    for (uint32_t first = 0; first < n_guides; first += kMaxPassReads) {
        const uint32_t count = std::min<uint32_t>(kMaxPassReads, n_guides - first);
        PassFound f;
        int prc = find_pass(ctx, genome, guides + first, count, first, params, false, t, f);
        if (prc == VSC_OK) prc = summarize_pass(ctx, f, !excl.empty(), t);
        if (prc != VSC_OK) return prc;
    }
    if (n_guides) {
        VSC_HIP(ctx, hipMemcpyAsync(out, ctx->sum_rows.p, (size_t)n_guides * sizeof(vsc_guide_summary), hipMemcpyDeviceToHost, ctx->stream));
        VSC_HIP(ctx, hipStreamSynchronize(ctx->stream));
    }
    ctx->timing = t;
    return VSC_OK;
    });
}

int vsc_search_select(vsc_ctx *ctx, const vsc_genome *genome, const uint64_t *guides, uint32_t n_guides,
                      const vsc_search_params *params, const vsc_select *select, const vsc_locus *exclude,
                      vsc_guide_summary *summary, vsc_hits **out)
{
    return guarded(ctx, [&]() -> int {
    if (!ctx || !out) return VSC_ERR_INVALID;
    *out = nullptr;
    vsc_timing t{};
    const int rc = search_setup(ctx, genome, guides, n_guides, params, "vsc_search_select", &t);
    if (rc != VSC_OK) return rc;
    if (!select) return fail(ctx, VSC_ERR_INVALID, "vsc_search_select: null argument");
    if (select->reserved[0] || select->reserved[1]) return fail(ctx, VSC_ERR_INVALID, "vsc_search_select: reserved fields must be 0");
    std::vector<uint64_t> excl;
    const int erc = excluded_loci(ctx, genome, exclude, n_guides, "vsc_search_select", excl);
    if (erc != VSC_OK) return erc;
    const int urc = upload_summary_state(ctx, n_guides, summary != nullptr, excl);
    if (urc != VSC_OK) return urc;
    const bool selecting = select->top_k || select->min_score || !excl.empty();
    vsc_hits *hits = new (std::nothrow) vsc_hits();
    if (!hits) return fail(ctx, VSC_ERR_NOMEM, "vsc_search_select: out of host memory");
    hits->ctx = ctx;
    uint64_t used = 0;
    for (uint32_t first = 0; first < n_guides; first += kMaxPassReads) {
        const uint32_t count = std::min<uint32_t>(kMaxPassReads, n_guides - first);
        const uint64_t projected = first ? (uint64_t)((double)used / first * n_guides * 1.02) + 4096 : 0;
        PassFound f;
        int prc = find_pass(ctx, genome, guides + first, count, first, params, false, t, f);
        if (prc == VSC_OK && summary) prc = summarize_pass(ctx, f, !excl.empty(), t, false);
        if (prc == VSC_OK && selecting) prc = select_pass(ctx, f, count, *select, !excl.empty());
        if (prc == VSC_OK) prc = sort_pass(ctx, genome, f, hits, used, projected, t);
        if (prc != VSC_OK) {
            vsc_hits_free(hits);
            return prc;
        }
        used += f.n;
    }
    if (summary && n_guides) {
        hipError_t e = hipMemcpyAsync(summary, ctx->sum_rows.p, (size_t)n_guides * sizeof(vsc_guide_summary), hipMemcpyDeviceToHost, ctx->stream);
        if (e == hipSuccess) e = hipStreamSynchronize(ctx->stream);
        if (e != hipSuccess) {
            vsc_hits_free(hits);
            VSC_HIP(ctx, e);
        }
    }
    hits->n = used;
    if (used == 0) hits->host_valid = true;
    ctx->timing = t;
    *out = hits;
    return VSC_OK;
    });
}

double vsc_mit_specificity(uint64_t mit_sum)
{
    return (100.0 / (100.0 + (double)mit_sum * 0x1p-24)) * 100.0;
}

int vsc_search_stream(vsc_ctx *ctx, const vsc_genome *genome, const uint64_t *guides, uint32_t n_guides,
                      const vsc_search_params *params, uint32_t batch_reads, vsc_batch_fn on_batch, void *user)
{
    return stream_batches(ctx, genome, guides, n_guides, params, batch_reads, false, "vsc_search_stream", on_batch != nullptr,
                          [&](vsc_hits *hits, uint32_t first, uint32_t count, vsc_timing &t) {
                              const int prc = on_batch(user, hits, first, count);
                              t.score_ms += ctx->timing.score_ms;
                              return prc;
                          });
}

int vsc_search_stream_rows(vsc_ctx *ctx, const vsc_genome *genome, const uint64_t *guides, uint32_t n_guides,
                           const vsc_search_params *params, uint32_t batch_reads, vsc_rows_batch_fn on_batch, void *user)
{
    return stream_batches(ctx, genome, guides, n_guides, params, batch_reads, true, "vsc_search_stream_rows", on_batch != nullptr,
                          [&](vsc_hits *hits, uint32_t first, uint32_t count, vsc_timing &t) {
                              if (hits->n && t.algorithm != VSC_ALGO_SEED) {
                                  int prc = vsc_score_hits_packed(ctx, genome, hits, guides, n_guides, 0, hits->n, nullptr, nullptr, nullptr);
                                  if (prc == VSC_OK && ctx->score_feat.cap < hits->n * VSC_PACKED_FEATURE_BYTES)
                                      prc = fail(ctx, VSC_ERR_NOMEM, "vsc_search_stream_rows: the batch's rows do not fit the device at once (smaller batches)");
                                  t.score_ms += ctx->timing.score_ms;
                                  if (prc != VSC_OK) return prc;
                              }
                              return on_batch(user, hits, first, count, hits->n ? ctx->score_feat.p : nullptr);
                          });
}

uint64_t vsc_hits_count(const vsc_hits *hits) { return hits ? hits->n : 0; }

const void *vsc_hits_data_dev(const vsc_hits *hits) { return hits ? hits->d_records : nullptr; }

int vsc_hits_data(vsc_hits *hits, const vsc_hit **out)
{
    return guarded(nullptr, [&]() -> int {
    if (!hits || !out) return VSC_ERR_INVALID;
    *out = nullptr;
    if (!hits->host_valid) {
        vsc_ctx *ctx = hits->ctx;
        try {
            hits->host.resize(hits->n);
        } catch (...) {
            return fail(ctx, VSC_ERR_NOMEM, "vsc_hits_data: out of host memory");
        }
        if (hits->n) {
            VSC_HIP(ctx, hipSetDevice(ctx->device));
            VSC_HIP(ctx, hipMemcpyAsync(hits->host.data(), hits->d_records, hits->n * sizeof(vsc_hit),
                                        hipMemcpyDeviceToHost, ctx->stream));
            VSC_HIP(ctx, hipStreamSynchronize(ctx->stream));
        }
        hits->host_valid = true;
    }
// ... 886 lines not shown
```

### varscot_amd/csrc/vsc_internal.h

```cpp
#pragma once

#include <hip/hip_runtime.h>
#include <stdint.h>

#include "varscot_hip.h"

namespace vsc {

constexpr int kWave = 64;
constexpr int kWavesPerGroup = 4;
constexpr int kSitesPerLane = 8;
constexpr int kBatch = kWave * kSitesPerLane;
constexpr int kQueueCap = kBatch + kWave;
constexpr int kHitCap = 128;
constexpr int kTileWords = kWave;
constexpr int kTileBases = kTileWords * 32;
constexpr int kChunkTiles = 8;
constexpr int kGuideUnroll = 4;
constexpr uint32_t kMask23 = 0x7FFFFFu;
constexpr int kSiteStrandBit = 23;
constexpr int kSiteEdgeBit = 24;
constexpr uint32_t kPadWords = 4;

constexpr int kSegments = 3;
constexpr int kSegBases = 7;
constexpr int kBucketsPerSeg = 1 << (2 * kSegBases);
constexpr int kBuckets = kSegments * kBucketsPerSeg;
constexpr int kSeedHitCap = 256;
constexpr int kSlicedSites = 32;
constexpr int kSlicedChunk = kWave * kSlicedSites;
constexpr int kRestBases = VSC_READ_LEN - kSegBases;
constexpr int kCmpBases = 2 * kSegBases;
constexpr int kVertWords = 2 * kCmpBases;
constexpr int kSeedClasses = 3;
constexpr int kLists = (kSegments - 1 + kSeedClasses) * kBucketsPerSeg;
constexpr int kListBudgetShift = 16;
constexpr uint32_t kListNoBudget = 15;
constexpr int kTokLaneShift = 26;
constexpr int kTokSlotShift = 14;
constexpr uint32_t kTokReadMask = (1u << kTokSlotShift) - 1u;
constexpr int kSlicedResolve = 3;
constexpr int kSlicedTokCap = 512;
constexpr uint32_t kChunkBucketMask = 0xFFFFu;
constexpr int kChunkMinusShift = 16;
constexpr int kChunkEdgeBit = 28;
constexpr int kChunkClassShift = 29;
constexpr uint32_t kIndexLayout = 2;
constexpr int kSlicedWavesPerSimd = 6;
constexpr int kSlicedGrab = 8;

enum { kCntHits = 0, kCntChunk = 1, kCntSites = 2, kCntOverflow = 3, kCntVisited = 4, kCntPad = 5, kCntLost = 6, kCntGroups = 7, kCntSlots = 8 };
constexpr int kRegionBits = 6;
constexpr int kRegionReads = 1 << kRegionBits;
constexpr int kParts = 256;
constexpr int kMaxPassReads = kParts * kRegionReads;
constexpr int kCntPart = 8;
constexpr int kCursors = 32;
constexpr int kCursorStride = 16;
constexpr int kCursorBase = kCntPart + 4 * kParts + 8;
constexpr int kCounterWords = kCursorBase + kCursors * kCursorStride;

constexpr int kRecPosShift = 23;
constexpr int kRecStrandShift = 55;
constexpr int kRecReadShift = 56;
constexpr int kRecKeyBits = 33 + kRegionBits;
constexpr uint64_t kRecSentinel = ~0ull;

constexpr int kSortThreads = 512;
constexpr int kSortItems = 16;
constexpr int kSortTile = kSortThreads * kSortItems;
constexpr int kFinThreads = 512;
constexpr int kFinItems = 16;
constexpr int kSortCap = kFinThreads * kFinItems - 128;
constexpr int kSortMaxBinBits = 11;
constexpr int kSortSubBits = 13;
constexpr int kSortSubBitsRows = 12;
constexpr int kHistTiles = 8;

struct PamMasks {
    uint32_t ah, al;
    uint32_t bh, bl;
};

struct ScanArgs {
    const uint32_t *hi, *lo, *nm;
    uint32_t first_pos;
    uint32_t n_tiles;
    const uint4 *guides;
    uint32_t n_guides_padded;
    uint32_t max_mm;
    uint32_t k_half;
    uint32_t n_pam;
    PamMasks pam[3];
    const uint32_t *contig_end;
    uint32_t n_contigs;
    uint64_t *hit_keys;
    uint32_t *hit_vals;
    unsigned long long hit_cap;
    unsigned long long *counters;
    uint32_t *site_x, *site_l, *site_pos;
};

struct SortSeg {
    uint64_t in_off;
    uint64_t out_off;
    uint64_t final_off;
    uint32_t n_in;
    uint32_t guide_base;
};

struct SortArgs {
    const SortSeg *segs;
    const uint32_t *seg_tile0;
    uint32_t n_segs, n_tiles;
    const uint64_t *in;
    const uint64_t *pair_keys;
    const uint32_t *pair_vals;
    uint64_t *out;
    const uint32_t *side_in;
    uint32_t *side_out;
    uint32_t *hist;
    uint32_t *cursor;
    uint32_t *bin_start;
    uint32_t bin_bits, bin_shift;
    uint32_t pos_pad;
    uint32_t pos_base;
    uint32_t xcd_tiles;
    uint32_t slot_cap;
    uint32_t *overflow;
};

struct FinArgs {
    const SortSeg *segs;
    uint32_t n_segs;
    const uint64_t *src;
    const uint32_t *hist;
    const uint32_t *bin_start;
    uint32_t bin_bits;
    uint32_t sub_shift, sub_bits;
    uint32_t low_bits;
    uint32_t pos_pad;
    uint32_t pos_base;
    SortSeg *over;
    uint32_t over_cap;
    uint32_t cap;
    uint32_t *n_over;
    uint32_t *cursor;
    const uint32_t *contig_off;
    uint32_t n_contigs;
    vsc_hit *out;
    uint32_t slot_cap;
    const uint32_t *overflow;
    const uint32_t *side_src;
    const uint2 *guides;
    uint32_t guide_first;
    uint4 *rows;
    uint64_t rows_first;
};

struct ScoreArgs {
    const vsc_hit *hits;
    uint64_t n;
    const uint2 *hl;
    uint32_t first_pos;
    uint64_t n_plane_words;
    const uint32_t *contig_off;
    const uint2 *guides;
    double *mit;
    uint8_t *mit_flags;
    uint8_t *features;
    const uint64_t *seg_prefix;
    const uint64_t *seg_start;
    uint32_t n_segs;
};

struct SeedPlan {
    uint32_t max_mm, k0, k1, tight;
    uint32_t n_nbr;
    uint32_t n_pam;
    uint32_t pam_codes;
};

struct SeedArgs {
    const uint4 *chunk_tab;
    const uint32_t *vert;
    const uint2 *list_rest;
    const uint2 *sites;
    const uint32_t *edge_bits;
    const uint2 *guides;
    uint32_t n_chunks;
    const uint32_t *poff;
    uint32_t max_mm, k_half;
    uint32_t k_seg0, k_seg1;
    const uint32_t *contig_end;
    uint32_t n_contigs;
    uint64_t *hit_recs;
    uint32_t *hit_side;
    uint32_t group_out;
    uint32_t reserve;
    uint32_t reserve_log2;
    uint32_t pos_pad;
    uint32_t pos_base;
    uint32_t n_parts;
    unsigned long long part_cap;
    unsigned long long *counters;
};

constexpr int kRfRows = 512;
constexpr int kRfMaxTests = 1024;
constexpr int kRfMaxNodes = 1024;
constexpr int kRfTileBytes = 26624;
constexpr int kRfPairFirstBit = 3;
constexpr int kRfPairMaxTests = 8 * (32 - kRfPairFirstBit);
constexpr int kRfPairBitsBytes = 16384;
constexpr int kRfPairTileBytes = 24512;
constexpr int kRfChains = 2;
constexpr int kRfRowWords = 20;
struct RfTest {
    uint8_t word, shift, width, thr;
    uint16_t dense_col;
    uint16_t pad;
};

struct RfArgs {
    const uint32_t *nodes;
    const uint8_t *depth;
    uint32_t n_trees, n_nodes;
    uint32_t compact;
    const RfTest *tests;
    const uint32_t *test_begin;
    uint32_t n_tests;
    const uint8_t *dense;
    const uint4 *packed;
    const uint8_t *act_rank;
    uint64_t n;
    uint32_t *votes;
    uint16_t *votes16;
    uint32_t tree_splits;
    ScoreArgs score;
};

constexpr int kSumWords = 12;
constexpr int kSumCounts = 11;
constexpr int kSumThreads = 256;
constexpr int kSumItems = 8;
constexpr int kSumTile = kSumThreads * kSumItems;
constexpr int kSumTilesPerBlock = 8;
constexpr int kSumCountBits = 7;

struct SumSeg {
    uint64_t in_off;
    uint32_t n;
    uint32_t first_read;
};

struct SummaryArgs {
    const uint64_t *recs;
    const uint32_t *vals;
    const SumSeg *segs;
    const uint32_t *seg_tile0;
    uint32_t n_segs, n_tiles;
    uint32_t pos_pad, pos_base;
    const uint64_t *excl;
    unsigned long long *out;
};

constexpr int kSelBins = 128;
constexpr int kSelThreads = 256;
constexpr int kSelMaxTilesPerBlock = 128;
constexpr int kSelMinTilesPerBlock = 8;
constexpr uint32_t kSelDropped = ~0u;
constexpr int kSelKeyPosBits = 33;

struct SelectArgs {
    const uint64_t *recs;
    const uint32_t *vals;
    const SumSeg *segs;
    const uint32_t *seg_tile0;
    uint32_t n_segs, n_tiles;
    uint32_t pos_pad, pos_base;
    const uint64_t *excl;
    uint32_t min_score;
    uint32_t top_k;
    uint32_t n_reads;
    uint32_t tiles_per_block;
    uint32_t *score;
    uint32_t *hist;
    uint32_t *thr;
    uint32_t *thr_region;
    uint32_t *count;
    uint32_t *cursor;
    const uint64_t *cand_off;
    const uint64_t *surv_off;
    uint64_t *cand_key;
    uint32_t *cand_mask;
    uint64_t *out;
};

hipError_t launch_scan(const ScanArgs &args, int n_groups, bool extract, hipStream_t stream);
hipError_t launch_summary(const SummaryArgs &args, hipStream_t stream);
hipError_t launch_select_score(const SelectArgs &args, hipStream_t stream);
hipError_t launch_select_threshold(const SelectArgs &args, hipStream_t stream);
hipError_t launch_select_compact(const SelectArgs &args, hipStream_t stream);
hipError_t launch_select_resolve(const SelectArgs &args, hipStream_t stream);
hipError_t launch_bin_hist(const SortArgs &args, hipStream_t stream);
hipError_t launch_bin_scan(const SortArgs &args, hipStream_t stream);
hipError_t launch_bin_partition(const SortArgs &args, hipStream_t stream);
hipError_t launch_bin_finalize(const FinArgs &args, int max_groups, hipStream_t stream);
hipError_t launch_rf_predict(const RfArgs &args, hipStream_t stream);
hipError_t launch_interleave(const uint32_t *hi, const uint32_t *lo, uint64_t n, uint2 *hl, hipStream_t stream);
hipError_t launch_score(const ScoreArgs &args, hipStream_t stream);
hipError_t launch_score_packed(const ScoreArgs &args, uint4 *packed, hipStream_t stream);
hipError_t launch_score_schedule(const ScoreArgs &args, uint32_t g_lo, uint32_t g_hi, uint32_t slice_shift, uint32_t n_slices,
                                 uint64_t *bounds, uint64_t *seg_start, uint64_t *seg_prefix, hipStream_t stream);
hipError_t launch_score_pairs(const uint2 *on, const uint2 *off, const uint32_t *masks, uint64_t n, double *mit,
                              uint8_t *mit_flags, uint8_t *features, hipStream_t stream);
hipError_t launch_xpack(const vsc_hit *in, uint64_t n, const uint32_t *contig_off, uint64_t *out, hipStream_t stream);
hipError_t launch_key_bounds(const vsc_hit *in, const uint64_t *range_dev, uint32_t K, uint64_t *bound, hipStream_t stream);
hipError_t launch_merge_packed(const uint64_t *seg_src, const uint64_t *seg_dst, const uint32_t *seg_n, uint32_t n_segs, uint32_t n_shards,
                               uint32_t first_key, const uint32_t *contig_off, const uint32_t *contig_end, uint32_t n_contigs, vsc_hit *out,
                               uint32_t *bad , const uint64_t *seg_side, uint16_t *side_out, hipStream_t stream);
hipError_t launch_plane_hash(const uint32_t *hi, const uint32_t *lo, const uint32_t *nm, uint64_t n_words, unsigned long long *out,
                             hipStream_t stream);
hipError_t launch_seed_keys(const uint4 *rec, uint64_t n, int seg, uint32_t pam_codes, uint32_t n_pam, uint64_t *sort_records, hipStream_t stream);
hipError_t launch_seed_lists(const uint2 *guides, uint32_t n_guides, const SeedPlan &plan, uint32_t *count, uint32_t *poff, uint2 *list_rest,
                             hipStream_t stream);
hipError_t launch_seed_pack16(const uint32_t *x, const uint32_t *l, const uint32_t *pos, uint64_t n, uint4 *rec, hipStream_t stream);
hipError_t launch_seed_gather16(const uint4 *rec, const uint64_t *sorted, uint64_t n, uint4 *out, hipStream_t stream);
hipError_t launch_seed_compact(const uint4 *sites16, uint64_t n_per_table, uint64_t n, uint2 *sites8, uint32_t *edge_bits,
                               hipStream_t stream);
hipError_t launch_seed_chunk_flags(uint4 *chunk_tab, uint32_t n_chunks, const uint32_t *edge_bits, hipStream_t stream);
hipError_t launch_seed_transpose(const uint4 *sites, const uint4 *chunk_tab, uint32_t n_chunks, uint32_t *vert,
                                 hipStream_t stream);
hipError_t launch_seed_sliced(const SeedArgs &args, int n_groups, bool shared, hipStream_t stream);
hipError_t launch_merge(const vsc_hit *in, const uint64_t *shard_off_dev, uint32_t n_shards, uint32_t K, uint64_t *bound,
                        uint64_t *key_off, vsc_hit *out, hipStream_t stream);

}
```

### varscot_amd/csrc/vsc_objects.h

```cpp
#pragma once

#include <string>
#include <vector>

#include "varscot_hip_debug.h"
#include "vsc_internal.h"

namespace vsc {

struct DeviceBuf {
    void *p = nullptr;
    size_t cap = 0;
    hipError_t ensure(size_t bytes)
    {
        if (bytes <= cap) return hipSuccess;
        if (p) (void)hipFree(p);
        p = nullptr;
        cap = 0;
        size_t want = bytes + (bytes < ((size_t)32 << 30) ? bytes / 8 : bytes / 32);
        hipError_t e = hipMalloc(&p, want);
        if (e != hipSuccess && want != bytes) {
            (void)hipGetLastError();
            want = bytes;
            e = hipMalloc(&p, want);
        }
        if (e == hipSuccess) cap = want;
        return e;
    }
    void release()
    {
        if (p) (void)hipFree(p);
        p = nullptr;
        cap = 0;
    }
};

inline vsc_debug_params default_debug_params()
{
    vsc_debug_params d{};
    d.sort_xcd = -1;
    d.sort_optimistic = -1;
    d.score_slices = -1;
    d.seed_shared = -1;
    d.seed_group_out = -1;
    d.seed_tight = -1;
    d.rf_form = -1;
    return d;
}

bool host_timing_on();

}

struct vsc_ctx {
    int device = 0;
    int n_cus = 0;
    hipStream_t stream = nullptr;
    bool own_stream = false;
    hipEvent_t ev[8] = {nullptr, nullptr, nullptr, nullptr, nullptr, nullptr, nullptr, nullptr};
    std::string err;
    vsc_timing timing{};
    vsc_debug_params dbg = vsc::default_debug_params();
    vsc::DeviceBuf counters, guides, keys_a, keys_b, vals_a, score_mit, score_flags, score_feat;
    vsc::DeviceBuf vals_b;
    vsc::DeviceBuf score_guides;
    uint64_t score_guides_hash = 0;
    uint32_t score_guides_n = ~0u;
    vsc::DeviceBuf sort_segs, sort_tabs, sort_over, score_sched;
    std::vector<vsc::SortSeg> host_segs;
    std::vector<uint32_t> host_tile0;
    vsc::DeviceBuf seed_off, seed_poff, seed_lrest;
    vsc::DeviceBuf sum_rows, sum_excl;
    vsc::DeviceBuf sel_hist, sel_tabs, sel_keys, sel_masks;
    struct Forest {
        vsc::DeviceBuf nodes, ranks;
        size_t depth_at = 0, tests_at = 0, begin_at = 0;
        uint32_t n_tests = 0, n_trees = 0, n_nodes = 0;
        uint32_t form = 0;
        uint32_t node_stride = 0;
        std::vector<double> thresholds;
        uint64_t fingerprint = 0;
        uint64_t ranks_key = 0;
        uint32_t ranks_n = ~0u;
    } forest;
    std::vector<vsc::DeviceBuf> spare_records;
};

struct vsc_genome {
    vsc_ctx *ctx = nullptr;
    uint32_t *d_hi = nullptr, *d_lo = nullptr, *d_nm = nullptr;
    uint32_t *d_contig_off = nullptr, *d_contig_end = nullptr;
    uint2 *d_hl = nullptr;
    uint64_t first_word = 0, own_words = 0, dev_words = 0;
    uint32_t n_tiles = 0, n_contigs = 0;
    uint64_t device_bytes = 0;
    mutable uint64_t sites = 0;
    mutable double seen_rate[VSC_MAX_MISMATCHES + 1] = {};
    mutable bool sort_slots_ok[VSC_MAX_MISMATCHES + 1] = {true, true, true, true, true, true, true, true, true};
    bool has_index = false;
    uint8_t index_has_extra_pam = 0;
    char index_extra_pam[2] = {0, 0};
    uint64_t index_sites = 0;
    uint4 *d_ix_chunk_tab = nullptr;
    uint32_t *d_ix_vert = nullptr;
    uint2 *d_ix_sites = nullptr;
    uint32_t *d_ix_edge = nullptr;
    uint32_t ix_chunks = 0;
    uint64_t ix_class_sites[4] = {};
    uint64_t ix_class_chunks[4] = {};
    uint64_t ix_vert_bytes = 0, ix_edge_words = 0;
    uint64_t index_bytes = 0;
    double index_ms = 0;
};

struct vsc_hits {
    vsc_ctx *ctx = nullptr;
    vsc_hit *d_records = nullptr;
    vsc::DeviceBuf storage;
    uint64_t n = 0;
    std::vector<vsc_hit> host;
    bool host_valid = false;
};


namespace vsc {
int genome_table_only(vsc_ctx *ctx, const vsc_contig *contigs, uint32_t n_contigs, vsc_genome **out);
int merge_packed_shards(vsc_ctx *ctx, const vsc_genome *genome, const void *const *shard_records, const void *const *shard_side,
                        const uint32_t *key_counts, uint32_t n_shards, uint32_t first_key, uint32_t n_keys, vsc_hits **out,
                        DeviceBuf *side_out);
}
```

### varscot_amd/csrc/vsc_seed.hip

```cpp
#include "vsc_internal.h"
#include "vsc_device.h"

#include <type_traits>

namespace vsc {

__device__ __forceinline__ uint32_t segment_key(uint32_t x, uint32_t l, int s)
{
    return (((x >> (kSegBases * s)) & 0x7Fu) << kSegBases) | ((l >> (kSegBases * s)) & 0x7Fu);
}

__device__ __forceinline__ uint32_t pam_code(uint32_t x, uint32_t l)
{
    return (((x >> 21) & 1u) << 3) | (((l >> 21) & 1u) << 2) | (((x >> 22) & 1u) << 1) | ((l >> 22) & 1u);
}

__global__ __launch_bounds__(256) void seed_key_kernel(const uint4 *rec, uint64_t n, int seg, uint32_t pam_codes, uint32_t n_pam, uint64_t *out)
{
    const uint64_t i = (uint64_t)blockIdx.x * blockDim.x + threadIdx.x;
    if (i >= n) return;
    const uint4 r = rec[i];
    const uint32_t code = pam_code(r.x, r.y);
    uint32_t cls = 0;
    for (uint32_t c = n_pam; c-- > 0;)
// ... 453 lines not shown

__device__ __forceinline__ uint32_t ring_slot(uint32_t p)
{
    return p & (uint32_t)(kSlicedTokCap - 1);
}

template <bool kFull>
__device__ __forceinline__ SlicedFetch sliced_fetch(const SeedArgs &a, const SeedWave &w, uint32_t head, uint32_t n)
{
    SlicedFetch f;
    if (!kFull) {
        f.word = 0;
        f.hi = 0;
        f.site0 = 0;
        f.gp = make_uint2(0u, 0u);
        f.rec = make_uint2(0u, 0u);
    }
    if (kFull || w.lane < n) {
        const uint2 tk = w.tok[ring_slot(head + w.lane)];
        f.word = tk.x;
        f.hi = tk.y;
        f.gp = a.guides[tk.y & kTokReadMask];
        f.site0 = w.first[(tk.y >> kTokSlotShift) & (uint32_t)(kSlicedGrab - 1)] + (tk.y >> kTokLaneShift) * kSlicedSites;
        f.rec = a.sites[f.site0 + (uint32_t)__builtin_ctz(tk.x)];
    }
    return f;
}

__device__ __forceinline__ uint32_t ring_tail(const SeedWave &w) { return ring_slot(w.thead + w.ntok); }

template <bool kFull>
__device__ __forceinline__ void sliced_consume(const SeedArgs &a, SeedWave &w, const SlicedFetch &f)
{
    bool hit = kFull || f.word != 0;
    const uint32_t rest = f.word & (f.word - 1);
    const uint64_t again = __ballot(rest != 0);
    if (again != 0) {
        if (rest != 0) w.tok[ring_slot(lanes_below(again, ring_tail(w)))] = make_uint2(rest, f.hi);
        w.ntok += (uint32_t)__popcll(again);
    }
    const uint32_t gid_of = f.hi & kTokReadMask;
    const uint32_t info = w.info[(f.hi >> kTokSlotShift) & (uint32_t)(kSlicedGrab - 1)];
    const uint32_t bucket = info & kChunkBucketMask;
    const uint32_t sh = (uint32_t)kSegBases * (bucket >> (2 * kSegBases));
    const uint32_t low = (1u << sh) - 1u;
    const uint32_t rest_hi = f.rec.x & 0xFFFFu, rest_lo = f.rec.x >> 16;
    const uint32_t site_hi = (rest_hi & low) | (((bucket >> kSegBases) & 0x7Fu) << sh) | ((rest_hi >> sh) << (sh + kSegBases));
    const uint32_t site_lo = (rest_lo & low) | ((bucket & 0x7Fu) << sh) | ((rest_lo >> sh) << (sh + kSegBases));
    const uint32_t t = ((site_hi ^ f.gp.x) | (site_lo ^ f.gp.y)) & kMask23;
    const uint32_t rank_in_chunk = (f.hi >> kTokLaneShift) * kSlicedSites + (uint32_t)__builtin_ctz(f.word | 0x80000000u);
    const uint32_t strand = rank_in_chunk >= ((info >> kChunkMinusShift) & 0xFFFu) ? 1u : 0u;
    const uint32_t pos = f.rec.y;
    const uint32_t mask = strand ? reverse23(t) : t;
    const bool maybe_edge = hit && ((info >> kChunkEdgeBit) & 1u) && (uint32_t)__popc(mask >> (VSC_READ_LEN / 2)) > a.k_half;
    if (__ballot(maybe_edge) != 0) {
        if (maybe_edge) {
            const uint32_t site = f.site0 + (uint32_t)__builtin_ctz(f.word);
            if (((a.edge_bits[site >> 5] >> (site & 31u)) & 1u) && is_contig_end(a.contig_end, a.n_contigs, pos + VSC_READ_LEN)) hit = false;
        }
    }
    const uint32_t low23 = a.hit_side ? (site_hi & kMask23) : mask;
    const uint64_t rec = ((uint64_t)(gid_of & (uint32_t)(kRegionReads - 1)) << kRecReadShift) | ((uint64_t)strand << kRecStrandShift) |
                         ((uint64_t)((pos - a.pos_base) << a.pos_pad) << kRecPosShift) | low23;
    sliced_store(a, w, hit, gid_of >> kRegionBits, rec, site_lo & kMask23);
}

template <bool kDrain>
__device__ __forceinline__ void sliced_resolve(const SeedArgs &a, SeedWave &w)
{
    wave_sync();
    bool have = false;
    SlicedFetch f = sliced_fetch<false>(a, w, 0, 0);
    for (;;) {
        uint32_t n = min(w.ntok, (uint32_t)kWave);
        if (!kDrain && n < (uint32_t)kWave) n = 0;
        if (n == 0 && !have) break;
        SlicedFetch nf = f;
        if (kDrain) nf = sliced_fetch<false>(a, w, w.thead, n);
        else if (n) nf = sliced_fetch<true>(a, w, w.thead, n);
        w.thead = ring_slot(w.thead + n);
        w.ntok -= n;
        if (have) sliced_consume<!kDrain>(a, w, f);
        wave_sync();
        f = nf;
        have = n != 0;
    }
    w.ntok = uniform(w.ntok);
    w.thead = uniform(w.thead);
}

__device__ __forceinline__ uint2 sliced_load_list(const SeedArgs &a, uint32_t g0, uint32_t g1, uint32_t lane)
{
    uint2 e = make_uint2(0xFFFFFFFFu, 0xFFFFFFFFu);
    if (g0 + lane < g1) e = a.list_rest[g0 + lane];
    return e;
}

__device__ __forceinline__ void sliced_load_sites(const SeedArgs &a, const v4u &ct, bool wanted, uint32_t lane,
                                                  uint32_t (&v)[kVertWords])
{
    const uint32_t nb = (ct.y + kSlicedSites - 1) / kSlicedSites;
    const bool mine = wanted && lane < nb;
    const uint4 *vp = (const uint4 *)(a.vert + (size_t)ct.w * kVertWords) + lane;
#pragma unroll
    for (int j = 0; j < kVertWords / 4; ++j) {
        uint4 x = make_uint4(0u, 0u, 0u, 0u);
        if (mine) x = vp[(size_t)j * nb];
        v[4 * j] = x.x;
        v[4 * j + 1] = x.y;
        v[4 * j + 2] = x.z;
        v[4 * j + 3] = x.w;
    }
}


static_assert(kMaxPassReads <= (1 << kTokSlotShift) && kSlicedGrab <= 8 && kTokSlotShift + 3 <= kTokLaneShift, "token fields");
static_assert((kSlicedTokCap & (kSlicedTokCap - 1)) == 0 && kSlicedTokCap >= (kSlicedResolve + kGuideUnroll) * kWave, "token ring");
template <bool kShared>
__global__ __launch_bounds__(kWave *kWavesPerGroup) __attribute__((amdgpu_waves_per_eu(kSlicedWavesPerSimd, kSlicedWavesPerSimd))) void seed_sliced_kernel(
    const SeedArgs a)
{
    __shared__ uint32_t s_grab[2];
    __shared__ uint2 s_tok[kWavesPerGroup][kSlicedTokCap];
    __shared__ uint2 s_list[kWavesPerGroup][kWave];
    __shared__ uint32_t s_parts[kWavesPerGroup][kParts];
    __shared__ uint32_t s_first[kWavesPerGroup][2 * kSlicedGrab];

    const uint32_t wave = threadIdx.x / kWave;
    SeedWave w;
    w.lane = threadIdx.x % kWave;
    w.tok = s_tok[wave];
    w.ntok = 0;
    w.thead = 0;
    w.parts = s_parts[kShared && a.group_out ? 0u : wave];
    w.first = s_first[wave];
    w.info = s_first[wave] + kSlicedGrab;
    for (uint32_t q = w.lane; q < (uint32_t)kParts; q += kWave) w.parts[q] = a.reserve;

    uint2 *const lt = s_list[wave];
    uint32_t kv[4];
#pragma unroll
    for (int i = 0; i < 4; ++i) asm volatile("v_mov_b32 %0, %1" : "=v"(kv[i]) : "s"(spread(i < 2 ? a.k_seg0 : a.k_seg1, i & 1)));
    const const_v4u_ptr ctab = (const_v4u_ptr)(uintptr_t)a.chunk_tab;
    const const_u32_ptr poff = (const_u32_ptr)(uintptr_t)a.poff;
    const const_v8u_ptr lgrp = (const_v8u_ptr)(uintptr_t)a.list_rest;
    constexpr bool kScalarLists = kShared;
    auto list_of = [](uint32_t z) {
        const uint32_t bucket = z & kChunkBucketMask;
        return bucket + (bucket >= 2u * kBucketsPerSeg ? ((z >> kChunkClassShift) & 3u) * (uint32_t)kBucketsPerSeg : 0u);
    };
    const uint32_t lane_tag = w.lane << kTokLaneShift;
    unsigned long long pairs = 0, visited = 0;

    const uint32_t slice_len = (a.n_chunks + kCursors - 1) / kCursors;
    uint32_t slice = uniform((kShared ? blockIdx.x : blockIdx.x * kWavesPerGroup + wave) % kCursors), exhausted = 0;
    const uint32_t wave_u = uniform(wave);
    for (uint32_t iter = 0;; ++iter) {
        uint32_t off = 0;
        if (kShared) {
            if (threadIdx.x == 0)
                s_grab[iter & 1u] = (uint32_t)atomicAdd(&a.counters[kCursorBase + slice * kCursorStride], (unsigned long long)kSlicedGrab);
            block_sync();
            off = s_grab[iter & 1u];
        } else if (w.lane == 0) {
            off = (uint32_t)atomicAdd(&a.counters[kCursorBase + slice * kCursorStride], (unsigned long long)kSlicedGrab);
        }
        off = uniform(off);
        const uint32_t slice_begin = slice * slice_len, slice_end = min(slice_begin + slice_len, a.n_chunks);
        if (slice_begin + off >= slice_end) {
            if (++exhausted == (uint32_t)kCursors) break;
            slice = (slice + 1) % kCursors;
            continue;
        }
        const uint32_t first = slice_begin + off;
        const uint32_t last = min(first + (uint32_t)kSlicedGrab, slice_end);
        auto my_part = [&](uint32_t g0, uint32_t g1, uint32_t r, uint32_t &q0, uint32_t &q1) {
            if (!kShared) {
                q0 = g0;
                q1 = g1;
                return;
            }
            const uint32_t n4 = (g1 - g0) / (uint32_t)kGuideUnroll;
            const uint32_t base = n4 / (uint32_t)kWavesPerGroup, rem = n4 % (uint32_t)kWavesPerGroup;
            q0 = g0 + (r * base + min(r, rem)) * (uint32_t)kGuideUnroll;
            q1 = q0 + (base + (r < rem ? 1u : 0u)) * (uint32_t)kGuideUnroll;
        };
        v4u t0 = ctab[first];
        v4u t1 = ctab[min(first + 1, last - 1)];
        uint32_t p0a, p0b;
        my_part(poff[list_of(t0.z)], poff[list_of(t0.z) + 1], wave_u, p0a, p0b);
        uint2 nl = make_uint2(0u, 0u);
        v8u ng = {};
        if (kScalarLists) ng = lgrp[(p0a < p0b ? p0a : 0u) / (uint32_t)kGuideUnroll];
        else nl = sliced_load_list(a, p0a, p0b, w.lane);
        uint32_t p1a = poff[list_of(t1.z)], p1b = poff[list_of(t1.z) + 1];
        v4u t2 = ctab[min(first + 2, last - 1)];
        for (uint32_t c = first; c < last; ++c) {
            const v4u cur = t0;
            const uint32_t g0 = p0a, g1 = p0b;
            uint32_t v[kVertWords];
            sliced_load_sites(a, cur, g0 != g1, w.lane, v);
            t0 = t1;
            my_part(p1a, p1b, (wave_u + (c + 1 - first)) % (uint32_t)kWavesPerGroup, p0a, p0b);
            uint2 tile = nl;
            v8u grp = ng;
            if (kScalarLists) ng = lgrp[(p0a < p0b && c + 1 < last ? p0a : 0u) / (uint32_t)kGuideUnroll];
            else nl = sliced_load_list(a, p0a, c + 1 < last ? p0b : p0a, w.lane);
            t1 = t2;
            p1a = poff[list_of(t1.z)];
            p1b = poff[list_of(t1.z) + 1];
            t2 = ctab[min(c + 3, last - 1)];
            if (g0 == g1) continue;
            const uint32_t slot_tag = (c - first) << kTokSlotShift;
            if (w.lane == 0) {
                w.first[c - first] = cur.x;
                w.info[c - first] = cur.z;
            }
            wave_sync();
            const uint32_t seg = uniform((cur.z & kChunkBucketMask) / (uint32_t)kBucketsPerSeg);
            const uint32_t budget_field = uniform((kListBudgetShift + 4u * ((cur.z >> kChunkClassShift) & 3u)) | (4u << 16));
            const int32_t left = (int32_t)cur.y - (int32_t)(w.lane * kSlicedSites);
            const uint32_t valid = left >= kSlicedSites ? 0xFFFFFFFFu : (left > 0 ? (1u << left) - 1u : 0u);
            pairs += (unsigned long long)cur.y * (g1 - g0);
            if (!kShared || (wave_u + (c - first)) % (uint32_t)kWavesPerGroup == 0) visited += cur.y;
            auto compare_four = [&](const uint32_t (&ex)[kGuideUnroll], const uint32_t (&ey)[kGuideUnroll]) {
                const uint32_t tail0 = uniform(w.thead + w.ntok);
                uint32_t tail = tail0;
                auto compare_group = [&](auto segment) {
                    constexpr uint32_t kSeg = decltype(segment)::value;
#pragma unroll
                    for (int u = 0; u < kGuideUnroll; ++u) {
                        const uint32_t ry = ey[u];
                        uint32_t budget;
                        asm("s_bfe_u32 %0, %1, %2" : "=s"(budget) : "s"(ry), "s"(budget_field) : "scc");
                        if (budget == kListNoBudget) continue;
                        const uint32_t word = sliced_within<kSeg>(v, ex[u], budget, valid, kv);
                        const uint64_t b = __ballot(word != 0);
                        if (b == 0) continue;
                        const uint32_t gid = ry & kTokReadMask;
                        if (word != 0) w.tok[ring_slot(lanes_below(b, tail))] = make_uint2(word, gid | slot_tag | lane_tag);
                        const uint32_t cnt = (uint32_t)__popcll(b);
                        const uint32_t tail_was = tail;
                        uint32_t tail_now;
                        asm("s_add_i32 %0, %1, %2" : "=s"(tail_now) : "s"(tail_was), "s"(cnt) : "scc");
                        tail = tail_now;
                    }
                };
                if (seg == 0) compare_group(std::integral_constant<uint32_t, 0>{});
                else if (seg == 1) compare_group(std::integral_constant<uint32_t, 1>{});
                else compare_group(std::integral_constant<uint32_t, 2>{});
                w.ntok += tail - tail0;
                if (w.ntok >= (uint32_t)kSlicedResolve * kWave) sliced_resolve<false>(a, w);
            };
            if (kScalarLists) {
                for (uint32_t gi = g0; gi < g1; gi += kGuideUnroll) {
                    const v8u e = grp;
                    grp = lgrp[(gi + kGuideUnroll < g1 ? gi + kGuideUnroll : gi) / (uint32_t)kGuideUnroll];
                    const uint32_t ex[kGuideUnroll] = {e[0], e[2], e[4], e[6]}, ey[kGuideUnroll] = {e[1], e[3], e[5], e[7]};
                    compare_four(ex, ey);
                }
                continue;
            }
            for (uint32_t tg = g0; tg < g1; tg += kWave) {
                wave_sync();
                lt[w.lane] = tile;
                wave_sync();
                if (tg + kWave < g1) tile = sliced_load_list(a, tg + kWave, g1, w.lane);
                const uint32_t in_tile = min(g1 - tg, (uint32_t)kWave);
                for (uint32_t gi = 0; gi < in_tile; gi += kGuideUnroll) {
                    uint2 rd[kGuideUnroll];
#pragma unroll
                    for (int u = 0; u < kGuideUnroll; ++u) rd[u] = lt[gi + u];
                    uint32_t ex[kGuideUnroll], ey[kGuideUnroll];
#pragma unroll
                    for (int u = 0; u < kGuideUnroll; ++u) {
                        ex[u] = uniform(rd[u].x);
                        ey[u] = uniform(rd[u].y);
                    }
                    compare_four(ex, ey);
                }
            }
        }
        if (w.ntok) sliced_resolve<true>(a, w);
    }
    if (kShared && a.group_out) {
        block_sync();
        sliced_finish_hits(a, w, wave_u, kWavesPerGroup);
    } else {
        sliced_finish_hits(a, w, 0, 1);
    }
    if (w.lane == 0 && pairs) {
        atomicAdd(&a.counters[kCntSites], pairs);
        atomicAdd(&a.counters[kCntVisited], visited);
    }
}

hipError_t launch_seed_sliced(const SeedArgs &args, int n_groups, bool shared, hipStream_t stream)
{
    const dim3 grid(n_groups), block(kWave * kWavesPerGroup);
    if (shared) hipLaunchKernelGGL((seed_sliced_kernel<true>), grid, block, 0, stream, args);
    else hipLaunchKernelGGL((seed_sliced_kernel<false>), grid, block, 0, stream, args);
    return hipGetLastError();
}

}
```

### varscot_amd/csrc/vsc_sort.hip

```cpp
#include "vsc_internal.h"
#include "vsc_device.h"

namespace vsc {

namespace {

constexpr int kLaneRun = 2;
__device__ __forceinline__ uint32_t tile_record(int k, uint32_t t)
{
    return (uint32_t)(k / kLaneRun) * (uint32_t)(kLaneRun * kSortThreads) + t * (uint32_t)kLaneRun + (uint32_t)(k % kLaneRun);
}

template <int kThreads>
__device__ __forceinline__ uint32_t block_exclusive_scan(uint32_t *s, uint32_t n, uint32_t *s_wave)
{
    const uint32_t t = threadIdx.x, lane = t % kWave, wave = t / kWave;
    const uint32_t per = n > (uint32_t)kThreads ? n / kThreads : 1u;
    const bool mine = t * per < n;
    uint32_t v[4] = {0u, 0u, 0u, 0u};
    uint32_t sum = 0;
    if (mine)
        for (uint32_t i = 0; i < per; ++i) {
            v[i] = s[t * per + i];
            sum += v[i];
        }
    uint32_t inc = sum;
#pragma unroll
    for (int d = 1; d < kWave; d <<= 1) {
        const uint32_t o = __shfl_up(inc, d, kWave);
        if (lane >= (uint32_t)d) inc += o;
    }
    if (lane == kWave - 1) s_wave[wave] = inc;
    block_sync();
    uint32_t before = 0, total = 0;
#pragma unroll
    for (int w = 0; w < kThreads / kWave; ++w) {
        const uint32_t x = s_wave[w];
        before += (uint32_t)w < wave ? x : 0u;
        total += x;
    }
    uint32_t run = before + inc - sum;
    if (mine)
        for (uint32_t i = 0; i < per; ++i) {
            s[t * per + i] = run;
            run += v[i];
        }
    block_sync();
    return total;
}

__device__ __forceinline__ uint32_t segment_of_tile(const uint32_t *seg_tile0, uint32_t n_segs, uint32_t tile)
{
    uint32_t lo = 0, hi = n_segs;
    while (hi - lo > 1) {
        const uint32_t mid = (lo + hi) >> 1;
        if (seg_tile0[mid] <= tile) lo = mid; else hi = mid;
    }
    return lo;
}

__device__ __forceinline__ uint64_t pack_pair(uint64_t key, uint32_t val, uint32_t pos_pad, uint32_t pos_base)
{
    const uint64_t high = (key >> 32) & ((1ull << (kRecKeyBits - 32)) - 1ull);
    return (((high << 32) | (uint32_t)(((uint32_t)key - pos_base) << pos_pad)) << kRecPosShift) | (val & kMask23);
}

}

template <bool kPairs>
__global__ __launch_bounds__(kSortThreads) void bin_hist_kernel(const SortArgs a)
{
    __shared__ uint32_t s_hist[1 << kSortMaxBinBits];
    const uint32_t t = threadIdx.x;
    const uint32_t nbins = 1u << a.bin_bits;
    for (uint32_t b = t; b < nbins; b += kSortThreads) s_hist[b] = 0;
    block_sync();
    const uint32_t tile_begin = blockIdx.x * kHistTiles, tile_end = min(tile_begin + (uint32_t)kHistTiles, a.n_tiles);
    uint32_t seg = segment_of_tile(a.seg_tile0, a.n_segs, tile_begin);
    for (uint32_t tile = tile_begin; tile < tile_end; ++tile) {
        if (tile >= a.seg_tile0[seg + 1]) {
            block_sync();
            for (uint32_t b = t; b < nbins; b += kSortThreads) {
                const uint32_t c = s_hist[b];
                if (c) atomicAdd(&a.hist[((size_t)seg << a.bin_bits) + b], c);
                s_hist[b] = 0;
            }
            block_sync();
            seg = segment_of_tile(a.seg_tile0, a.n_segs, tile);
        }
        const SortSeg sg = a.segs[seg];
        const uint32_t first = (tile - a.seg_tile0[seg]) * (uint32_t)kSortTile;
        const uint32_t n = min(sg.n_in - first, (uint32_t)kSortTile);
        uint64_t r[kSortItems];
#pragma unroll
        for (int k = 0; k < kSortItems; ++k) {
            const uint32_t i = tile_record(k, t);
            const uint64_t at = sg.in_off + first + (i < n ? i : 0u);
            const uint64_t v = kPairs ? a.pair_keys[at] : a.in[at];
            r[k] = i < n ? v : kRecSentinel;
        }
#pragma unroll
        for (int k = 0; k < kSortItems; ++k) {
            if (kPairs) {
                if (tile_record(k, t) < n) atomicAdd(&s_hist[(uint32_t)(r[k] >> a.bin_shift)], 1u);
            } else {
                if (!(r[k] >> 63)) atomicAdd(&s_hist[(uint32_t)(r[k] >> a.bin_shift) & (nbins - 1u)], 1u);
            }
        }
    }
    block_sync();
    for (uint32_t b = t; b < nbins; b += kSortThreads) {
        const uint32_t c = s_hist[b];
        if (c) atomicAdd(&a.hist[((size_t)seg << a.bin_bits) + b], c);
    }
}

hipError_t launch_bin_hist(const SortArgs &args, hipStream_t stream)
{
    if (args.n_tiles == 0) return hipSuccess;
    const unsigned blocks = (args.n_tiles + kHistTiles - 1) / kHistTiles;
    if (args.pair_keys)
        hipLaunchKernelGGL(bin_hist_kernel<true>, dim3(blocks), dim3(kSortThreads), 0, stream, args);
    else
        hipLaunchKernelGGL(bin_hist_kernel<false>, dim3(blocks), dim3(kSortThreads), 0, stream, args);
    return hipGetLastError();
}

__global__ __launch_bounds__(512) void bin_scan_kernel(const SortArgs a)
{
    __shared__ uint32_t s_cnt[1 << kSortMaxBinBits];
    __shared__ uint32_t s_wave[512 / kWave];
    const uint32_t nbins = 1u << a.bin_bits;
    const size_t base = (size_t)blockIdx.x << a.bin_bits;
    for (uint32_t b = threadIdx.x; b < nbins; b += 512) s_cnt[b] = a.hist[base + b];
    block_sync();
    block_exclusive_scan<512>(s_cnt, nbins, s_wave);
    for (uint32_t b = threadIdx.x; b < nbins; b += 512) {
        a.bin_start[base + b] = s_cnt[b];
        if (!a.slot_cap) a.cursor[base + b] = s_cnt[b];
    }
}

hipError_t launch_bin_scan(const SortArgs &args, hipStream_t stream)
{
    if (args.n_segs == 0) return hipSuccess;
    hipLaunchKernelGGL(bin_scan_kernel, dim3(args.n_segs), dim3(512), 0, stream, args);
    return hipGetLastError();
}

template <bool kPairs, bool kSide = false>
__global__ __launch_bounds__(kSortThreads) void bin_partition_kernel(const SortArgs a)
{
    __shared__ uint64_t s_rec[kSortTile];
    __shared__ uint32_t s_cnt[(1 << kSortMaxBinBits) + kWave];
    __shared__ uint32_t s_gbase[kPairs ? (1 << kSortMaxBinBits) : 1];
    __shared__ uint32_t s_over[(1 << kSortMaxBinBits) / 32 + 1];
    __shared__ uint32_t s_wave[kSortThreads / kWave];
    const uint32_t t = threadIdx.x;
    const uint32_t nbins = 1u << a.bin_bits;
    uint32_t tile = blockIdx.x;
    if (a.xcd_tiles) {
        tile = (blockIdx.x & 7u) * a.xcd_tiles + (blockIdx.x >> 3);
        if ((blockIdx.x >> 3) >= a.xcd_tiles || tile >= a.n_tiles) return;
    }
    const uint32_t seg = segment_of_tile(a.seg_tile0, a.n_segs, tile);
    const SortSeg sg = a.segs[seg];
    const uint32_t first = (tile - a.seg_tile0[seg]) * (uint32_t)kSortTile;
    const uint32_t n = min(sg.n_in - first, (uint32_t)kSortTile);
    for (uint32_t b = t; b < nbins + kWave; b += kSortThreads) s_cnt[b] = 0;
    for (uint32_t b = t; b < (1u << kSortMaxBinBits) / 32u + 1u; b += kSortThreads) s_over[b] = 0;
    block_sync();
    uint64_t r[kSortItems];
    uint32_t bin[kSortItems];
    uint32_t side[kSide ? kSortItems : 1];
#pragma unroll
    for (int k = 0; k < kSortItems; ++k) {
        const uint32_t i = tile_record(k, t);
        const bool in_tile = i < n;
        const uint64_t at = sg.in_off + first + (in_tile ? i : 0u);
        if (kSide) side[k] = a.side_in[at];
        if (kPairs) {
            const uint64_t key = a.pair_keys[at];
            r[k] = in_tile ? pack_pair(key, a.pair_vals[at], a.pos_pad, a.pos_base) : kRecSentinel;
            bin[k] = in_tile ? (uint32_t)(key >> a.bin_shift) : 0u;
        } else {
            const uint64_t v = a.in[at];
            r[k] = in_tile ? v : kRecSentinel;
            bin[k] = (uint32_t)(r[k] >> a.bin_shift) & (nbins - 1u);
        }
    }
    const uint32_t spare = nbins + (t % kWave);
#pragma unroll
    for (int k = 0; k < kSortItems; ++k) {
        const bool real = !(r[k] >> 63);
        const uint32_t rank = atomicAdd(&s_cnt[real ? bin[k] : spare], real ? 1u : 0u);
        bin[k] |= rank << 16;
    }
    block_sync();
    constexpr int kOwnBins = (1 << kSortMaxBinBits) / kSortThreads;
    uint32_t own_at[kOwnBins];
#pragma unroll
    for (int j = 0; j < kOwnBins; ++j) {
        const uint32_t b = t + (uint32_t)j * kSortThreads;
        const uint32_t c = b < nbins ? s_cnt[b] : 0u;
        uint32_t at = c ? atomicAdd(&a.cursor[((size_t)seg << a.bin_bits) + b], c) : 0u;
        if (a.slot_cap && c && at + c > a.slot_cap) {
            atomicOr(a.overflow, 1u);
            atomicOr(&s_over[b >> 5], 1u << (b & 31u));
            s_over[(1u << kSortMaxBinBits) / 32u] = 1u;
        }
        own_at[j] = at;
        if (kPairs && b < nbins) s_gbase[b] = at;
    }
    const uint32_t total = block_exclusive_scan<kSortThreads>(s_cnt, nbins, s_wave);
#pragma unroll
    for (int k = 0; k < kSortItems; ++k) {
        const uint32_t slot = s_cnt[bin[k] & 0xFFFFu] + (bin[k] >> 16);
        if (!(r[k] >> 63)) s_rec[slot] = r[k];
        if (kSide) bin[k] = slot;
    }
    block_sync();
    if (!kPairs) {
#pragma unroll
        for (int j = 0; j < kOwnBins; ++j) {
            const uint32_t b = t + (uint32_t)j * kSortThreads;
            if (b < nbins) s_cnt[b] = own_at[j] - s_cnt[b];
        }
        block_sync();
    }
    const bool any_over = s_over[(1u << kSortMaxBinBits) / 32u] != 0u;
    uint32_t slot_bin[kSide ? kSortItems / 2 : 1];
    if (kSide) {
#pragma unroll
        for (int j = 0; j < kSortItems / 2; ++j) slot_bin[j] = 0;
    }
    for (uint32_t i = t; i < total; i += kSortThreads) {
        const uint64_t x = s_rec[i];
        uint32_t b;
        if (kPairs) {
            uint32_t lo = 0, hi = nbins;
            while (hi - lo > 1) {
                const uint32_t mid = (lo + hi) >> 1;
                if (s_cnt[mid] <= i) lo = mid; else hi = mid;
            }
            b = lo;
        } else {
            b = (uint32_t)(x >> a.bin_shift) & (nbins - 1u);
        }
        const uint32_t in_bin = kPairs ? s_gbase[b] + (i - s_cnt[b]) : s_cnt[b] + i;
        const bool skip = any_over && ((s_over[b >> 5] >> (b & 31u)) & 1u);
        if (a.slot_cap) {
            if (!skip) a.out[(((uint64_t)seg << a.bin_bits) + b) * a.slot_cap + in_bin] = x;
        } else {
            a.out[sg.out_off + in_bin] = x;
        }
        if (kSide) {
            const uint32_t j = i / kSortThreads;
#pragma unroll
            for (int q = 0; q < kSortItems / 2; ++q)
                if ((uint32_t)q == (j >> 1)) slot_bin[q] |= b << ((j & 1u) * 16u);
        }
    }
    if (kSide) {
        block_sync();
        uint32_t *const s_side = (uint32_t *)s_rec;
#pragma unroll
        for (int k = 0; k < kSortItems; ++k)
            if (!(r[k] >> 63)) s_side[bin[k]] = side[k];
        block_sync();
#pragma unroll
        for (int j = 0; j < kSortItems; ++j) {
            const uint32_t i = t + (uint32_t)j * kSortThreads;
            if (i < total) {
                const uint32_t b = (slot_bin[j >> 1] >> ((j & 1) * 16)) & 0xFFFFu;
                const uint32_t in_bin = s_cnt[b] + i;
                const bool skip = any_over && ((s_over[b >> 5] >> (b & 31u)) & 1u);
                if (a.slot_cap) {
                    if (!skip) a.side_out[(((uint64_t)seg << a.bin_bits) + b) * a.slot_cap + in_bin] = s_side[i];
                } else {
                    a.side_out[sg.out_off + in_bin] = s_side[i];
                }
            }
        }
    }
}

hipError_t launch_bin_partition(const SortArgs &args, hipStream_t stream)
{
    if (args.n_tiles == 0) return hipSuccess;
    const unsigned blocks = args.xcd_tiles ? 8u * args.xcd_tiles : args.n_tiles;
    if (args.pair_keys)
        hipLaunchKernelGGL(bin_partition_kernel<true>, dim3(blocks), dim3(kSortThreads), 0, stream, args);
    else if (args.side_in)
        hipLaunchKernelGGL((bin_partition_kernel<false, true>), dim3(blocks), dim3(kSortThreads), 0, stream, args);
    else
        hipLaunchKernelGGL(bin_partition_kernel<false>, dim3(blocks), dim3(kSortThreads), 0, stream, args);
    return hipGetLastError();
}

__device__ __forceinline__ uint32_t sub_slot(const uint32_t *s_sub, uint32_t sb)
{
    return (s_sub[sb >> 1] >> ((sb & 1u) * 16u)) & 0xFFFFu;
}

constexpr int kFinalizeAhead = 4;
constexpr int kFinalizeNear = 4;
constexpr int kFinalizeRange = 64;

template <bool kRows>
__device__ __forceinline__ void finalize_bin(const FinArgs &a, const uint32_t which)
{
    __shared__ uint64_t s_rec[kSortCap];
    __shared__ uint32_t s_sub[(1 << (kRows ? kSortSubBitsRows : kSortSubBits)) / 2 + 1 + kWave];
    __shared__ uint4 s_stage[kRows ? (kFinThreads / kWave) * 64 : 1];
    __shared__ uint32_t s_wave[kFinThreads / kWave];
    __shared__ uint32_t s_range[2 + kFinalizeRange];
    __shared__ uint32_t s_edge[4];
    uint32_t t_ = threadIdx.x;
    asm volatile("" : "+v"(t_));
    const uint32_t t = t_;
    const uint32_t seg = which >> a.bin_bits, bin = which & ((1u << a.bin_bits) - 1u);
    const SortSeg sg = a.segs[seg];
    uint64_t src = sg.in_off, dst = sg.final_off;
    uint64_t compact = sg.in_off;
    uint32_t n_src = sg.n_in;
    if (a.hist) {
        const size_t idx = ((size_t)seg << a.bin_bits) + bin;
        n_src = a.hist[idx];
        const uint32_t st = a.bin_start[idx];
        src = a.slot_cap ? (uint64_t)idx * a.slot_cap : sg.out_off + st;
        dst = sg.final_off + st;
        compact = sg.in_off + st;
    }
    if (n_src == 0) return;
    if (n_src > a.cap) {
        if (t == 0) {
            const uint32_t slot = atomicAdd(a.n_over, 1u);
            if (slot < a.over_cap) {
                SortSeg o;
                o.in_off = src;
                o.out_off = a.slot_cap ? compact : src;
                o.final_off = dst;
                o.n_in = n_src;
                o.guide_base = sg.guide_base;
                a.over[slot] = o;
            }
        }
        return;
    }
    const uint32_t nsub = 1u << a.sub_bits;
    const uint32_t nwords = nsub > 1u ? nsub / 2u : 1u;
    for (uint32_t i = t; i <= nwords + kWave; i += kFinThreads) s_sub[i] = 0;
    if (t < 4) s_edge[t] = 0;
    const bool few_contigs = a.n_contigs <= (uint32_t)kFinThreads;
    const uint32_t my_contig = (few_contigs && t < a.n_contigs) ? a.contig_off[t] : 0xFFFFFFFFu;
    block_sync();
    const uint64_t *const in = a.src + src;
    uint64_t r[kFinItems];
    uint32_t rk[kFinItems];
#pragma unroll
    for (int k = 0; k < kFinItems; ++k) {
        const uint32_t i = k * kFinThreads + t;
        const uint64_t v = in[i < n_src ? i : 0u];
        r[k] = i < n_src ? v : kRecSentinel;
    }
    if (t == 0) {
        const uint32_t free_bits = a.sub_bits + a.low_bits;
        const uint32_t any = (uint32_t)(r[0] >> kRecPosShift) >> a.pos_pad;
        const uint32_t p_lo = free_bits >= 32u ? 0u : (any >> free_bits) << free_bits;
        const uint64_t p_hi = free_bits >= 32u ? 0xFFFFFFFFull : (uint64_t)(p_lo | ((1u << free_bits) - 1u)) + a.pos_base;
        s_edge[0] = free_bits >= 32u ? 0u : (uint32_t)min((uint64_t)p_lo + a.pos_base, (uint64_t)0xFFFFFFFFull);
        s_edge[1] = (uint32_t)min(p_hi, (uint64_t)0xFFFFFFFFull);
    }
#pragma unroll
    for (int k = 0; k < kFinItems; ++k) {
        const bool real = !(r[k] >> 63);
        const uint32_t sb = (uint32_t)(r[k] >> a.sub_shift) & (nsub - 1u);
        const uint32_t sh = (sb & 1u) * 16u;
        rk[k] = (atomicAdd(&s_sub[real ? sb >> 1 : nwords + 1u + (t % kWave)], real ? 1u << sh : 0u) >> sh) & 0xFFFFu;
    }
    block_sync();
    if (few_contigs) {
        const uint32_t p_lo = s_edge[0], p_hi = s_edge[1];
        const bool mine = t < a.n_contigs;
        const uint64_t le_lo = __ballot(mine && my_contig <= p_lo), le_hi = __ballot(mine && my_contig <= p_hi);
        if (t % kWave == 0) {
            if (le_lo) atomicAdd(&s_edge[2], (uint32_t)__popcll(le_lo));
            if (le_hi) atomicAdd(&s_edge[3], (uint32_t)__popcll(le_hi));
        }
    }
    uint32_t n;
    {
        const uint32_t per = nwords > (uint32_t)kFinThreads ? nwords / kFinThreads : 1u;
        static_assert((1 << kSortSubBits) / 2 <= 8 * kFinThreads, "a thread scans at most 8 words of the sub-bin table");
        const bool mine = t * per < nwords;
        uint32_t w[8];
        uint32_t sum = 0;
#pragma unroll
        for (int i = 0; i < 8; ++i) {
            w[i] = (mine && (uint32_t)i < per) ? s_sub[t * per + i] : 0u;
            sum += (w[i] & 0xFFFFu) + (w[i] >> 16);
        }
        const uint32_t lane = t % kWave, wave = t / kWave;
        uint32_t inc = sum;
#pragma unroll
        for (int d = 1; d < kWave; d <<= 1) {
            const uint32_t o = __shfl_up(inc, d, kWave);
            if (lane >= (uint32_t)d) inc += o;
        }
        if (lane == kWave - 1) s_wave[wave] = inc;
        block_sync();
        uint32_t before = 0, total = 0;
#pragma unroll
        for (int q = 0; q < kFinThreads / kWave; ++q) {
            const uint32_t x = s_wave[q];
            before += (uint32_t)q < wave ? x : 0u;
            total += x;
        }
        n = total;
        uint32_t run = before + inc - sum;
#pragma unroll
        for (int i = 0; i < 8; ++i) {
            const uint32_t lo = run;
            run += w[i] & 0xFFFFu;
            const uint32_t hi = run;
            run += w[i] >> 16;
            if (mine && (uint32_t)i < per) s_sub[t * per + i] = lo | (hi << 16);
        }
        if (t == 0 && nsub > 1u) s_sub[nwords] = n;
        if (few_contigs) {
            const uint32_t c_lo = max(s_edge[2], 1u) - 1u, c_hi = max(s_edge[3], 1u) - 1u;
            if (t == 0) {
                s_range[0] = c_lo;
                s_range[1] = c_hi - c_lo + 1u;
            }
            if (t >= c_lo && t < c_lo + (uint32_t)kFinalizeRange && t < a.n_contigs) s_range[2 + t - c_lo] = my_contig;
            if (t < (uint32_t)kFinalizeRange && a.n_contigs - c_lo + t < (uint32_t)kFinalizeRange) s_range[2 + a.n_contigs - c_lo + t] = 0xFFFFFFFFu;
        } else if (t == 0) {
            const uint32_t p_lo = s_edge[0], p_hi = s_edge[1];
            uint32_t lo = 0, hi = a.n_contigs;
            while (hi - lo > 1) {
                const uint32_t mid = (lo + hi) >> 1;
                if (a.contig_off[mid] <= p_lo) lo = mid; else hi = mid;
// ... 253 lines not shown
```

Baseline: 288,200.

## Overlap seed search with level-one sort partition by splitting chunks into pieces

Splits the seed-search chunk range into pieces: after the first piece finishes, its candidate records are partitioned on a second stream while the remaining chunks are searched. A small-block, raised-priority variant of the bin partition kernel lets the partition run beside the seed kernel. The intent is to hide level-one sort time behind the search. In exchange it adds a second stream, events, per-piece reserve capacity in the output buffer and more host bookkeeping, with possible contention between the two kernels.

Result: slower. 275,100 (-4.6%).

```diff
diff --git a/include/varscot_hip_debug.h b/include/varscot_hip_debug.h
--- a/include/varscot_hip_debug.h
+++ b/include/varscot_hip_debug.h
@@ -23,7 +23,7 @@
     int32_t seed_group_out;
     int32_t seed_tight;
     int32_t rf_form;
-    uint32_t reserved[1];
+    uint32_t seed_pieces;
 } vsc_debug_params;
 
 int vsc_ctx_set_debug_params(vsc_ctx *ctx, const vsc_debug_params *params);
diff --git a/varscot_amd/_lib.py b/varscot_amd/_lib.py
--- a/varscot_amd/_lib.py
+++ b/varscot_amd/_lib.py
@@ -76,7 +76,7 @@
                 ("sort_optimistic", C.c_int32), ("sort_slot_cap", C.c_uint32), ("score_chunk", C.c_uint64),
                 ("score_slices", C.c_int32), ("score_slice_shift", C.c_uint32), ("seed_shared", C.c_int32),
                 ("seed_group_out", C.c_int32), ("seed_tight", C.c_int32), ("rf_form", C.c_int32),
-                ("reserved", C.c_uint32 * 1)]
+                ("seed_pieces", C.c_uint32)]
     SIGNED_DEFAULT = ("sort_xcd", "sort_optimistic", "score_slices", "seed_shared", "seed_group_out", "seed_tight", "rf_form")
 
     @classmethod
diff --git a/varscot_amd/csrc/vsc_api.cpp b/varscot_amd/csrc/vsc_api.cpp
--- a/varscot_amd/csrc/vsc_api.cpp
+++ b/varscot_amd/csrc/vsc_api.cpp
@@ -187,6 +187,10 @@
             vsc_ctx_destroy(ctx);
             return VSC_ERR_DEVICE;
         }
+    if ((cu_mask && n_mask_words ? hipExtStreamCreateWithCUMask(&ctx->stream2, n_mask_words, cu_mask) : hipStreamCreate(&ctx->stream2)) != hipSuccess) {
+        vsc_ctx_destroy(ctx);
+        return VSC_ERR_DEVICE;
+    }
     *out = ctx;
     return VSC_OK;
 }
@@ -196,6 +200,8 @@
     if (!ctx) return VSC_ERR_INVALID;
     (void)hipSetDevice(ctx->device);
     (void)hipStreamSynchronize(ctx->stream);
+    if (ctx->stream2) (void)hipStreamSynchronize(ctx->stream2);
+    ctx->piece_tabs.release();
     for (DeviceBuf *b : {&ctx->counters, &ctx->guides, &ctx->score_guides, &ctx->keys_a, &ctx->keys_b, &ctx->vals_a, &ctx->vals_b,
                          &ctx->score_mit, &ctx->score_flags, &ctx->score_feat, &ctx->score_sched, &ctx->sort_segs, &ctx->sort_tabs,
                          &ctx->sort_over, &ctx->seed_off,
@@ -216,6 +222,10 @@
     (void)vsc_ctx_release_scratch(ctx);
     for (auto &e : ctx->ev)
         if (e) (void)hipEventDestroy(e);
+    for (auto &e : ctx->piece_ev)
+        if (e) (void)hipEventDestroy(e);
+    if (ctx->piece_snap) (void)hipHostFree(ctx->piece_snap);
+    if (ctx->stream2) (void)hipStreamDestroy(ctx->stream2);
     if (ctx->own_stream && ctx->stream) (void)hipStreamDestroy(ctx->stream);
     delete ctx;
     return VSC_OK;
@@ -914,21 +924,122 @@
     unsigned slot_fallbacks = 0;
 };
 
+struct PieceSort {
+    bool active = false;
+    bool declined = false;
+    unsigned bits = 0;
+    uint64_t part_cap = 0;
+    std::vector<uint32_t> done;
+    unsigned launched = 0;
+    unsigned first = 0;
+};
+
+struct SortCaps {
+    uint64_t sort_cap, slot_cap;
+    unsigned max_bits;
+};
+
+SortCaps sort_caps(const vsc_debug_params &dbg)
+{
+    SortCaps c{kSortCap, 0, kSortMaxBinBits};
+    if (dbg.sort_cap) c.sort_cap = std::min<uint64_t>(kSortCap, std::max<uint32_t>(16, dbg.sort_cap));
+    if (dbg.sort_max_bits) c.max_bits = std::min<unsigned>(kSortMaxBinBits, std::max<uint32_t>(1, dbg.sort_max_bits));
+    c.slot_cap = dbg.sort_slot_cap ? dbg.sort_slot_cap : (c.sort_cap + c.sort_cap / 4 + 15) / 16 * 16;
+    c.slot_cap = std::max<uint64_t>(c.slot_cap, 16);
+    return c;
+}
+
+unsigned level_bits(const SortCaps &c, uint64_t n_max, unsigned rem, size_t n_segs)
+{
+    if (n_max <= c.sort_cap || rem == 0) return 0;
+    const uint64_t want = std::max<uint64_t>(1, c.sort_cap * 7 / 10);
+    unsigned bits = std::min<unsigned>({std::max(1u, ceil_log2((n_max + want - 1) / want)), c.max_bits, rem});
+    while (bits > 1 && ((uint64_t)n_segs << bits) > (1ull << 22)) --bits;
+    return bits;
+}
+
+hipError_t size_level1(vsc_ctx *ctx, const SortCaps &c, size_t n_bins, uint64_t n_all, uint64_t span, bool with_side, size_t side_cap,
+                       DeviceBuf *other_buf, bool *slots, bool &use_slots)
+{
+    const vsc_debug_params &dbg = ctx->dbg;
+    const uint64_t slot_records = (uint64_t)n_bins * c.slot_cap;
+    if (use_slots && dbg.sort_optimistic != 1) {
+        size_t free_b = 0, total_b = 0;
+        if (hipMemGetInfo(&free_b, &total_b) != hipSuccess) free_b = 0;
+        const uint64_t room = (uint64_t)free_b + other_buf->cap;
+        const uint64_t slot_bytes = slot_records * (sizeof(uint64_t) + (with_side ? sizeof(uint32_t) : 0));
+        if (slot_records > 4 * n_all + (1ull << 20) || slot_bytes + (1ull << 30) > room + side_cap) {
+            use_slots = false;
+            *slots = false;
+        }
+    }
+    hipError_t ge = other_buf->ensure((size_t)(use_slots ? std::max(slot_records, span) : span) * sizeof(uint64_t));
+    if (ge == hipErrorOutOfMemory && use_slots) {
+        (void)hipGetLastError();
+        use_slots = false;
+        *slots = false;
+        ge = other_buf->ensure((size_t)span * sizeof(uint64_t));
+    }
+    return ge;
+}
+
+hipError_t piece_partition(vsc_ctx *ctx, const PieceSort &ps, unsigned slot, uint64_t part_cap, const std::vector<uint32_t> &to, const uint64_t *src,
+                           uint64_t *dst, unsigned bin_shift, uint64_t slot_cap, bool small, hipStream_t st)
+{
+    const size_t n_segs = to.size(), n_bins = n_segs << ps.bits;
+    const uint32_t tile_records = small ? kSortTileSmall : kSortTile;
+    if (ctx->piece_segs.size() < kMaxPieces) {
+        ctx->piece_segs.resize(kMaxPieces);
+        ctx->piece_tile0.resize(kMaxPieces);
+    }
+    VSC_TRY(ctx->piece_tabs.ensure(kMaxPieces * kPieceTabBytes));
+    std::vector<SortSeg> &segs = ctx->piece_segs[slot];
+    std::vector<uint32_t> &tile0 = ctx->piece_tile0[slot];
+    segs.resize(n_segs);
+    tile0.assign(n_segs + 1, 0);
+    uint64_t tiles = 0;
+    for (size_t q = 0; q < n_segs; ++q) {
+        const uint32_t n = to[q] - ps.done[q];
+        segs[q] = SortSeg{q * part_cap + ps.done[q], q * part_cap, 0, n, 0};
+        tile0[q] = (uint32_t)tiles;
+        tiles += (n + tile_records - 1) / tile_records;
+    }
+    if (tiles >= (1ull << 31)) return hipErrorInvalidValue;
+    tile0[n_segs] = (uint32_t)tiles;
+    if (tiles == 0) return hipSuccess;
+    char *const tab = (char *)ctx->piece_tabs.p + (size_t)slot * kPieceTabBytes;
+    VSC_TRY(hipMemcpyAsync(tab, segs.data(), n_segs * sizeof(SortSeg), hipMemcpyHostToDevice, st));
+    VSC_TRY(hipMemcpyAsync(tab + kParts * sizeof(SortSeg), tile0.data(), tile0.size() * sizeof(uint32_t), hipMemcpyHostToDevice, st));
+    SortArgs a{};
+    a.segs = (const SortSeg *)tab;
+    a.seg_tile0 = (const uint32_t *)(tab + kParts * sizeof(SortSeg));
+    a.n_segs = (uint32_t)n_segs;
+    a.n_tiles = (uint32_t)tiles;
+    a.in = src;
+    a.out = dst;
+    a.cursor = (uint32_t *)ctx->sort_tabs.p + n_bins;
+    a.hist = a.cursor;
+    a.bin_start = a.cursor + n_bins;
+    a.bin_bits = ps.bits;
+    a.bin_shift = bin_shift;
+    if (ctx->dbg.sort_xcd != 0 && tiles >= 64) a.xcd_tiles = (uint32_t)((tiles + 7) / 8);
+    a.slot_cap = (uint32_t)slot_cap;
+    a.overflow = (uint32_t *)ctx->sort_over.p + 2;
+    a.tile_records = tile_records;
+    return launch_bin_partition(a, st);
+}
+
 hipError_t bin_sort(vsc_ctx *ctx, const vsc_genome *genome, std::vector<SortSeg> segs, uint64_t *src, uint64_t *other,
                     unsigned key_bits, unsigned pos_pad, uint32_t pos_base, vsc_hit *out, hipEvent_t ev_sorted, SortInfo *info,
-                    DeviceBuf *other_buf = nullptr, bool *slots = nullptr, const SortRows *rows = nullptr)
+                    DeviceBuf *other_buf = nullptr, bool *slots = nullptr, const SortRows *rows = nullptr, const PieceSort *ps = nullptr)
 {
     uint32_t *side_src = rows ? rows->side_src : nullptr, *side_other = nullptr;
     hipStream_t st = ctx->stream;
     unsigned rem = key_bits;
     bool sorted_marked = false;
     const vsc_debug_params &dbg = ctx->dbg;
-    uint64_t sort_cap = kSortCap;
-    unsigned max_bits = kSortMaxBinBits;
-    if (dbg.sort_cap) sort_cap = std::min<uint64_t>(kSortCap, std::max<uint32_t>(16, dbg.sort_cap));
-    if (dbg.sort_max_bits) max_bits = std::min<unsigned>(kSortMaxBinBits, std::max<uint32_t>(1, dbg.sort_max_bits));
-    uint64_t slot_cap = dbg.sort_slot_cap ? dbg.sort_slot_cap : (sort_cap + sort_cap / 4 + 15) / 16 * 16;
-    slot_cap = std::max<uint64_t>(slot_cap, 16);
+    const SortCaps caps = sort_caps(dbg);
+    const uint64_t sort_cap = caps.sort_cap, slot_cap = caps.slot_cap;
     for (unsigned level = 1; !segs.empty(); ++level) {
         if (level > 48) return hipErrorUnknown;
         uint64_t n_max = 0, n_all = 0;
@@ -936,38 +1047,18 @@
             n_max = std::max<uint64_t>(n_max, s.n_in);
             n_all += s.n_in;
         }
-        unsigned bits = 0;
-        if (n_max > sort_cap) {
-            if (rem == 0) return hipErrorUnknown;
-            const uint64_t want = std::max<uint64_t>(1, sort_cap * 7 / 10);
-            bits = std::min<unsigned>({std::max(1u, ceil_log2((n_max + want - 1) / want)), max_bits, rem});
-            while (bits > 1 && ((uint64_t)segs.size() << bits) > (1ull << 22)) --bits;
-        }
+        if (n_max > sort_cap && rem == 0) return hipErrorUnknown;
+        const bool pieces = level == 1 && ps && ps->active;
+        const unsigned bits = pieces ? ps->bits : level_bits(caps, n_max, rem, segs.size());
         const size_t n_segs = segs.size();
         const size_t n_bins = n_segs << bits;
-        bool use_slots = level == 1 && bits && slots && other_buf && (dbg.sort_optimistic == 1 || (dbg.sort_optimistic != 0 && *slots));
-        if (level == 1 && bits && other_buf) {
+        bool use_slots = pieces || (level == 1 && bits && slots && other_buf && (dbg.sort_optimistic == 1 || (dbg.sort_optimistic != 0 && *slots)));
+        if (pieces) {
+            other = (uint64_t *)other_buf->p;
+        } else if (level == 1 && bits && other_buf) {
             uint64_t span = 1;
             for (const SortSeg &sg : segs) span = std::max<uint64_t>(span, sg.out_off + sg.n_in);
-            const uint64_t slot_records = (uint64_t)n_bins * slot_cap;
-            if (use_slots && dbg.sort_optimistic != 1) {
-                size_t free_b = 0, total_b = 0;
-                if (hipMemGetInfo(&free_b, &total_b) != hipSuccess) free_b = 0;
-                const uint64_t room = (uint64_t)free_b + other_buf->cap;
-                const uint64_t slot_bytes = slot_records * (sizeof(uint64_t) + (rows ? sizeof(uint32_t) : 0));
-                if (slot_records > 4 * n_all + (1ull << 20) || slot_bytes + (1ull << 30) > room + (rows ? rows->side_other->cap : 0)) {
-                    use_slots = false;
-                    *slots = false;
-                }
-            }
-            hipError_t ge = other_buf->ensure((size_t)(use_slots ? std::max(slot_records, span) : span) * sizeof(uint64_t));
-            if (ge == hipErrorOutOfMemory && use_slots) {
-                (void)hipGetLastError();
-                use_slots = false;
-                *slots = false;
-                ge = other_buf->ensure((size_t)span * sizeof(uint64_t));
-            }
-            if (ge != hipSuccess) return ge;
+            VSC_TRY(size_level1(ctx, caps, n_bins, n_all, span, rows != nullptr, rows ? rows->side_other->cap : 0, other_buf, slots, use_slots));
             other = (uint64_t *)other_buf->p;
             if (rows) {
                 VSC_TRY(rows->side_other->ensure(other_buf->cap / sizeof(uint64_t) * sizeof(uint32_t)));
@@ -994,12 +1085,13 @@
         uint32_t *d_n_over = (uint32_t *)ctx->sort_over.p;
         if (bits) VSC_TRY(ctx->sort_tabs.ensure(3 * n_bins * sizeof(uint32_t)));
         uint32_t flags[3] = {0, 0, 0};
+        if (pieces && ps->launched) VSC_TRY(hipStreamWaitEvent(st, ctx->piece_ev[3 * (ps->first + ps->launched - 1) + 2], 0));
         for (;;) {
             if (dbg.sort_debug)
                 std::fprintf(stderr, "[vsc sort] level %u: %zu segments, %llu records, largest %llu, %u bits (of %u left), cap %llu%s\n", level,
                              n_segs, (unsigned long long)n_all, (unsigned long long)n_max, bits, rem, (unsigned long long)sort_cap,
                              use_slots ? ", slot mode" : "");
-            VSC_TRY(hipMemsetAsync(d_n_over, 0, 3 * sizeof(uint32_t), st));
+            VSC_TRY(hipMemsetAsync(d_n_over, 0, (pieces && use_slots ? 2 : 3) * sizeof(uint32_t), st));
             FinArgs f{};
             f.segs = d_segs;
             f.n_segs = (uint32_t)n_segs;
@@ -1031,8 +1123,15 @@
                     a.hist = a.cursor;
                     a.slot_cap = (uint32_t)slot_cap;
                     a.overflow = d_n_over + 2;
-                    VSC_TRY(hipMemsetAsync(a.cursor, 0, n_bins * sizeof(uint32_t), st));
-                    VSC_TRY(launch_bin_partition(a, st));
+                    if (pieces) {
+                        std::vector<uint32_t> to(n_segs);
+                        for (size_t i = 0; i < n_segs; ++i) to[i] = segs[i].n_in;
+                        VSC_TRY(piece_partition(ctx, *ps, kMaxPieces - 1, ps->part_cap, to, src, other, a.bin_shift,
+                                                slot_cap, false, st));
+                    } else {
+                        VSC_TRY(hipMemsetAsync(a.cursor, 0, n_bins * sizeof(uint32_t), st));
+                        VSC_TRY(launch_bin_partition(a, st));
+                    }
                     VSC_TRY(launch_bin_scan(a, st));
                 } else {
                     VSC_TRY(hipMemsetAsync(a.hist, 0, n_bins * sizeof(uint32_t), st));
@@ -1163,6 +1262,7 @@
     bool bases = false;
     bool selected = false;
     std::vector<uint64_t> sel_off;
+    PieceSort pieces;
 };
 
 uint32_t neighbours(int k) { return k < 0 ? 0u : (k == 0 ? 1u : (k == 1 ? 22u : 211u)); }
@@ -1296,8 +1396,24 @@
     return hipSuccess;
 }
 
+constexpr unsigned kPiecesDefault = 2;
+constexpr double kPiecesFirst = 0.6;
+constexpr uint32_t kPiecesGroupsBeside = 5;
+constexpr uint64_t kPiecesMinRegion = 1ull << 20;
+
+struct StreamsIdle {
+    vsc_ctx *ctx;
+    bool armed;
+    ~StreamsIdle()
+    {
+        if (!armed) return;
+        if (ctx->stream2) (void)hipStreamSynchronize(ctx->stream2);
+        (void)hipStreamSynchronize(ctx->stream);
+    }
+};
+
 int find_pass(vsc_ctx *ctx, const vsc_genome *genome, const uint64_t *guides, uint32_t n_guides, uint32_t guide_base,
-              const vsc_search_params *params, bool keep_bases, vsc_timing &t, PassFound &f)
+              const vsc_search_params *params, bool keep_bases, vsc_timing &t, PassFound &f, bool to_records = false)
 {
     const int algo = (int)t.algorithm;
     const uint32_t m = params->max_mismatches;
@@ -1345,6 +1461,38 @@
     }
 
     f.ht.lap("prep enqueue");
+    unsigned n_pieces = 1;
+    const vsc_debug_params &dbg = ctx->dbg;
+    if (algo == VSC_ALGO_SEED && to_records && !keep_bases && ctx->stream2 && dbg.seed_pieces != 1 &&
+        (dbg.sort_optimistic == 1 || (dbg.sort_optimistic != 0 && genome->sort_slots_ok[m]))) {
+        const uint64_t region_est = std::max<uint64_t>(f.cap / f.n_parts * 2 / 3, (uint64_t)(seen_rate * std::min<uint32_t>(n_guides, kRegionReads)));
+        if (dbg.seed_pieces >= 2) n_pieces = std::min<unsigned>(dbg.seed_pieces, kMaxPieces);
+        else if (seed_shared && region_est >= kPiecesMinRegion) n_pieces = kPiecesDefault;
+    }
+    std::vector<uint32_t> piece_end(n_pieces, sa.n_chunks);
+    for (unsigned k = 0; k + 1 < n_pieces; ++k)
+        piece_end[k] = dbg.seed_pieces >= 2 ? (uint32_t)((uint64_t)sa.n_chunks * (k + 1) / n_pieces)
+                                            : (uint32_t)((double)sa.n_chunks * (kPiecesFirst + (1.0 - kPiecesFirst) * k / (n_pieces - 1)));
+    const uint32_t owners = sa.group_out ? (uint32_t)n_groups : (uint32_t)n_groups * kWavesPerGroup;
+    StreamsIdle idle{ctx, n_pieces > 1};
+    if (n_pieces > 1) {
+        sa.part_cap += (uint64_t)(n_pieces - 1) * owners * sa.reserve;
+        f.cap = sa.part_cap * f.n_parts;
+        while (ctx->piece_ev.size() < 3 * (size_t)n_pieces) {
+            hipEvent_t e = nullptr;
+            VSC_HIP(ctx, hipEventCreate(&e));
+            ctx->piece_ev.push_back(e);
+        }
+        if (!ctx->piece_snap) VSC_HIP(ctx, hipHostMalloc((void **)&ctx->piece_snap, kMaxPieces * kPieceSnapWords * sizeof(unsigned long long), hipHostMallocDefault));
+    }
+    auto piece_groups = [&](uint32_t len, uint32_t per_cu) {
+        const uint32_t n_grabs = (len + kSlicedGrab - 1) / kSlicedGrab;
+        const uint32_t n_waves_max = (uint32_t)ctx->n_cus * per_cu * kWavesPerGroup;
+        const uint32_t n_waves = std::max<uint32_t>(1, std::min<uint32_t>(n_waves_max, seed_shared ? n_grabs * kWavesPerGroup : n_grabs));
+        return std::min<int>(n_groups, (int)((n_waves + kWavesPerGroup - 1) / kWavesPerGroup));
+    };
+    const SortCaps caps = sort_caps(dbg);
+    PieceSort &ps = f.pieces;
     uint32_t list_total = 0;
     for (unsigned tries = 0;; ++tries) {
         if (algo == VSC_ALGO_SEED && (sa.part_cap >= (1ull << 32) - (1u << 20) || sa.part_cap >= ((uint64_t)sa.reserve << 20) - sa.reserve))
@@ -1364,9 +1512,62 @@
                 VSC_HIP(ctx, ctx->vals_a.ensure(f.cap * sizeof(uint32_t)));
                 sa.hit_side = (uint32_t *)ctx->vals_a.p;
             }
-            VSC_HIP(ctx, launch_seed_sliced(sa, n_groups, seed_shared, ctx->stream));
+            for (unsigned k = 0; k < n_pieces; ++k) {
+                sa.chunk_first = k ? piece_end[k - 1] : 0u;
+                sa.chunk_end = piece_end[k];
+                if (k) VSC_HIP(ctx, hipMemsetAsync((unsigned long long *)ctx->counters.p + kCursorBase, 0, kCursors * kCursorStride * sizeof(unsigned long long), ctx->stream));
+                const uint32_t per_cu = dbg.seed_groups_per_cu ? dbg.seed_groups_per_cu : (k ? kPiecesGroupsBeside : kSlicedWavesPerSimd);
+                VSC_HIP(ctx, launch_seed_sliced(sa, n_pieces > 1 ? piece_groups(sa.chunk_end - sa.chunk_first, per_cu) : n_groups, seed_shared, ctx->stream));
+                if (k + 1 < n_pieces) {
+                    VSC_HIP(ctx, hipMemcpyAsync(ctx->piece_snap + (size_t)k * kPieceSnapWords, ctx->counters.p, kPieceSnapWords * sizeof(unsigned long long),
+                                                hipMemcpyDeviceToHost, ctx->stream));
+                    VSC_HIP(ctx, hipEventRecord(ctx->piece_ev[3 * k], ctx->stream));
+                }
+            }
         }
         VSC_HIP(ctx, hipEventRecord(ctx->ev[2], ctx->stream));
+        ps = PieceSort{};
+        for (unsigned k = 0; k + 1 < n_pieces && !ps.declined; ++k) {
+            VSC_HIP(ctx, hipEventSynchronize(ctx->piece_ev[3 * k]));
+            const unsigned long long *snap = ctx->piece_snap + (size_t)k * kPieceSnapWords;
+            if (snap[kCntOverflow]) break;
+            std::vector<uint32_t> to(f.n_parts);
+            uint64_t n_max = 0, n_all = 0;
+            for (int q = 0; q < f.n_parts; ++q) {
+                to[q] = (uint32_t)snap[kCntPart + 4 * q];
+                n_max = std::max<uint64_t>(n_max, to[q]);
+                n_all += to[q];
+            }
+            if (!ps.active) {
+                if ((uint64_t)piece_end[k] * 4 < sa.n_chunks) continue;
+                const double scale = (double)sa.n_chunks / std::max<uint32_t>(1, piece_end[k]);
+                const unsigned bits = level_bits(caps, (uint64_t)(n_max * scale), f.key_bits, (size_t)f.n_parts);
+                if (!bits) continue;
+                const size_t n_bins = (size_t)f.n_parts << bits;
+                bool use_slots = true, slots_ok = true;
+                VSC_HIP(ctx, size_level1(ctx, caps, n_bins, (uint64_t)(n_all * scale), f.cap, false, 0, &ctx->keys_b, &slots_ok, use_slots));
+                if (!use_slots) {
+                    ps.declined = true;
+                    break;
+                }
+                VSC_HIP(ctx, ctx->sort_over.ensure(256 + n_bins * sizeof(SortSeg)));
+                VSC_HIP(ctx, ctx->sort_tabs.ensure(3 * n_bins * sizeof(uint32_t)));
+                VSC_HIP(ctx, hipMemsetAsync((uint32_t *)ctx->sort_tabs.p + n_bins, 0, n_bins * sizeof(uint32_t), ctx->stream2));
+                VSC_HIP(ctx, hipMemsetAsync((uint32_t *)ctx->sort_over.p + 2, 0, sizeof(uint32_t), ctx->stream2));
+                ps.active = true;
+                ps.bits = bits;
+                ps.part_cap = sa.part_cap;
+                ps.done.assign(f.n_parts, 0);
+                ps.first = k;
+            }
+            VSC_HIP(ctx, hipStreamWaitEvent(ctx->stream2, ctx->piece_ev[3 * k], 0));
+            VSC_HIP(ctx, hipEventRecord(ctx->piece_ev[3 * k + 1], ctx->stream2));
+            VSC_HIP(ctx, piece_partition(ctx, ps, k, sa.part_cap, to, (const uint64_t *)ctx->keys_a.p, (uint64_t *)ctx->keys_b.p,
+                                         kRecPosShift + f.pos_pad + f.key_bits - ps.bits, caps.slot_cap, true, ctx->stream2));
+            VSC_HIP(ctx, hipEventRecord(ctx->piece_ev[3 * k + 2], ctx->stream2));
+            ps.done = to;
+            ps.launched++;
+        }
         VSC_HIP(ctx, hipMemcpyAsync(cnt, ctx->counters.p, sizeof cnt, hipMemcpyDeviceToHost, ctx->stream));
         if (algo == VSC_ALGO_SEED)
             VSC_HIP(ctx, hipMemcpyAsync(&list_total, (const uint32_t *)ctx->seed_poff.p + kLists, sizeof list_total, hipMemcpyDeviceToHost, ctx->stream));
@@ -1374,16 +1575,19 @@
         f.ht.lap("search kernel + sync");
         t.passes++;
         if (!cnt[kCntOverflow]) break;
+        if (n_pieces > 1) VSC_HIP(ctx, hipStreamSynchronize(ctx->stream2));
+        ps = PieceSort{};
         if (tries >= 2) return fail(ctx, VSC_ERR_DEVICE, "vsc_search: hit buffer overflowed repeatedly");
         if (algo == VSC_ALGO_SEED) {
             uint64_t need = 0;
             for (int q = 0; q < f.n_parts; ++q) need = std::max<uint64_t>(need, cnt[kCntPart + 4 * q] + cnt[kCntPart + 4 * q + 2]);
-            sa.part_cap = need + (need >> 6) + 4096 + (uint64_t)(sa.group_out ? n_groups : n_groups * kWavesPerGroup) * sa.reserve;
+            sa.part_cap = need + (need >> 6) + 4096 + (uint64_t)n_pieces * owners * sa.reserve;
             f.cap = sa.part_cap * f.n_parts;
         } else {
             f.cap = cnt[kCntHits] + (cnt[kCntHits] >> 6) + 4096;
         }
     }
+    idle.armed = false;
     float ms = 0;
     VSC_HIP(ctx, hipEventElapsedTime(&ms, ctx->ev[0], ctx->ev[7]));
     t.prep_ms += ms;
@@ -1408,7 +1612,7 @@
         for (int q = 0; q < f.n_parts; ++q) {
             const uint64_t placed = cnt[kCntPart + 4 * q], real = placed - cnt[kCntPart + 4 * q + 1];
             fullest = std::max(fullest, (double)placed / std::min<uint32_t>(kRegionReads, n_guides - (uint32_t)q * kRegionReads));
-            if (placed) f.segs.push_back(SortSeg{(uint64_t)q * sa.part_cap, (uint64_t)q * sa.part_cap, f.n, (uint32_t)placed,
+            if (placed || ps.active) f.segs.push_back(SortSeg{(uint64_t)q * sa.part_cap, (uint64_t)q * sa.part_cap, f.n, (uint32_t)placed,
                                                  guide_base + (uint32_t)q * kRegionReads});
             f.n += real;
         }
@@ -1435,6 +1639,7 @@
 int sort_pass(vsc_ctx *ctx, const vsc_genome *genome, PassFound &f, vsc_hits *hits, uint64_t used, uint64_t projected, vsc_timing &t)
 {
     SortInfo info;
+    StreamsIdle idle{ctx, f.pieces.active};
     if (f.n > 0) {
         uint64_t *src = (uint64_t *)ctx->keys_a.p, *other = nullptr;
         if (f.algo == VSC_ALGO_SCAN && !f.selected) {
@@ -1499,7 +1704,7 @@
             rows.rows_first = used;
         }
         VSC_HIP(ctx, bin_sort(ctx, genome, std::move(f.segs), src, other, f.key_bits, f.pos_pad, f.pos_base, hits->d_records, ctx->ev[3],
-                              &info, f.algo == VSC_ALGO_SEED || f.selected ? &ctx->keys_b : nullptr, slots, f.bases ? &rows : nullptr));
+                              &info, f.algo == VSC_ALGO_SEED || f.selected ? &ctx->keys_b : nullptr, slots, f.bases ? &rows : nullptr, &f.pieces));
     } else {
         VSC_HIP(ctx, hipEventRecord(ctx->ev[3], ctx->stream));
     }
@@ -1507,6 +1712,10 @@
     float ms = 0;
     VSC_HIP(ctx, hipEventElapsedTime(&ms, ctx->ev[2], ctx->ev[3]));
     t.sort_ms += ms;
+    for (unsigned k = f.pieces.first; f.pieces.active && k < f.pieces.first + f.pieces.launched; ++k) {
+        VSC_HIP(ctx, hipEventElapsedTime(&ms, ctx->piece_ev[3 * k + 1], ctx->piece_ev[3 * k + 2]));
+        t.sort_ms += ms;
+    }
     t.sort_levels = std::max(t.sort_levels, info.levels);
     t.sort_bin_bits = std::max(t.sort_bin_bits, info.bin_bits);
     t.sort_bytes += info.bytes;
@@ -1715,7 +1924,7 @@
         if (!hits) return fail(ctx, VSC_ERR_NOMEM, (std::string(who) + ": out of host memory").c_str());
         hits->ctx = ctx;
         PassFound f;
-        int prc = find_pass(ctx, genome, guides + first, count, first, params, rows && t.algorithm == VSC_ALGO_SEED, t, f);
+        int prc = find_pass(ctx, genome, guides + first, count, first, params, rows && t.algorithm == VSC_ALGO_SEED, t, f, !rows);
         if (prc == VSC_OK) prc = sort_pass(ctx, genome, f, hits, 0, 0, t);
         if (prc == VSC_OK) {
             hits->n = f.n;
@@ -1754,7 +1963,7 @@
         const uint32_t count = std::min<uint32_t>(kMaxPassReads, n_guides - first);
         const uint64_t projected = first ? (uint64_t)((double)used / first * n_guides * 1.02) + 4096 : 0;
         PassFound f;
-        int prc = find_pass(ctx, genome, guides + first, count, first, params, false, t, f);
+        int prc = find_pass(ctx, genome, guides + first, count, first, params, false, t, f, true);
         if (prc == VSC_OK) prc = sort_pass(ctx, genome, f, hits, used, projected, t);
         if (prc != VSC_OK) {
             vsc_hits_free(hits);
diff --git a/varscot_amd/csrc/vsc_internal.h b/varscot_amd/csrc/vsc_internal.h
--- a/varscot_amd/csrc/vsc_internal.h
+++ b/varscot_amd/csrc/vsc_internal.h
@@ -69,6 +69,8 @@
 constexpr int kSortThreads = 512;
 constexpr int kSortItems = 16;
 constexpr int kSortTile = kSortThreads * kSortItems;
+constexpr int kSortThreadsSmall = 256;
+constexpr int kSortTileSmall = kSortThreadsSmall * kSortItems;
 constexpr int kFinThreads = 512;
 constexpr int kFinItems = 16;
 constexpr int kSortCap = kFinThreads * kFinItems - 128;
@@ -128,6 +130,7 @@
     uint32_t xcd_tiles;
     uint32_t slot_cap;
     uint32_t *overflow;
+    uint32_t tile_records;
 };
 
 struct FinArgs {
@@ -189,6 +192,7 @@
     const uint32_t *edge_bits;
     const uint2 *guides;
     uint32_t n_chunks;
+    uint32_t chunk_first, chunk_end;
     const uint32_t *poff;
     uint32_t max_mm, k_half;
     uint32_t k_seg0, k_seg1;
diff --git a/varscot_amd/csrc/vsc_objects.h b/varscot_amd/csrc/vsc_objects.h
--- a/varscot_amd/csrc/vsc_objects.h
+++ b/varscot_amd/csrc/vsc_objects.h
@@ -35,6 +35,10 @@
     }
 };
 
+constexpr unsigned kMaxPieces = 64;
+constexpr size_t kPieceSnapWords = kCntPart + 4 * kParts;
+constexpr size_t kPieceTabBytes = (kParts * sizeof(SortSeg) + (kParts + 1) * sizeof(uint32_t) + 255) / 256 * 256;
+
 inline vsc_debug_params default_debug_params()
 {
     vsc_debug_params d{};
@@ -58,6 +62,12 @@
     hipStream_t stream = nullptr;
     bool own_stream = false;
     hipEvent_t ev[8] = {nullptr, nullptr, nullptr, nullptr, nullptr, nullptr, nullptr, nullptr};
+    hipStream_t stream2 = nullptr;
+    std::vector<hipEvent_t> piece_ev;
+    unsigned long long *piece_snap = nullptr;
+    vsc::DeviceBuf piece_tabs;
+    std::vector<std::vector<vsc::SortSeg>> piece_segs;
+    std::vector<std::vector<uint32_t>> piece_tile0;
     std::string err;
     vsc_timing timing{};
     vsc_debug_params dbg = vsc::default_debug_params();
diff --git a/varscot_amd/csrc/vsc_seed.hip b/varscot_amd/csrc/vsc_seed.hip
--- a/varscot_amd/csrc/vsc_seed.hip
+++ b/varscot_amd/csrc/vsc_seed.hip
@@ -629,7 +629,7 @@
     const uint32_t lane_tag = w.lane << kTokLaneShift;
     unsigned long long pairs = 0, visited = 0;
 
-    const uint32_t slice_len = (a.n_chunks + kCursors - 1) / kCursors;
+    const uint32_t slice_len = (a.chunk_end - a.chunk_first + kCursors - 1) / kCursors;
     uint32_t slice = uniform((kShared ? blockIdx.x : blockIdx.x * kWavesPerGroup + wave) % kCursors), exhausted = 0;
     const uint32_t wave_u = uniform(wave);
     for (uint32_t iter = 0;; ++iter) {
@@ -643,7 +643,7 @@
             off = (uint32_t)atomicAdd(&a.counters[kCursorBase + slice * kCursorStride], (unsigned long long)kSlicedGrab);
         }
         off = uniform(off);
-        const uint32_t slice_begin = slice * slice_len, slice_end = min(slice_begin + slice_len, a.n_chunks);
+        const uint32_t slice_begin = a.chunk_first + slice * slice_len, slice_end = min(slice_begin + slice_len, a.chunk_end);
         if (slice_begin + off >= slice_end) {
             if (++exhausted == (uint32_t)kCursors) break;
             slice = (slice + 1) % kCursors;
diff --git a/varscot_amd/csrc/vsc_sort.hip b/varscot_amd/csrc/vsc_sort.hip
--- a/varscot_amd/csrc/vsc_sort.hip
+++ b/varscot_amd/csrc/vsc_sort.hip
@@ -6,9 +6,10 @@
 namespace {
 
 constexpr int kLaneRun = 2;
+template <int kThreads = kSortThreads>
 __device__ __forceinline__ uint32_t tile_record(int k, uint32_t t)
 {
-    return (uint32_t)(k / kLaneRun) * (uint32_t)(kLaneRun * kSortThreads) + t * (uint32_t)kLaneRun + (uint32_t)(k % kLaneRun);
+    return (uint32_t)(k / kLaneRun) * (uint32_t)(kLaneRun * kThreads) + t * (uint32_t)kLaneRun + (uint32_t)(k % kLaneRun);
 }
 
 template <int kThreads>
@@ -17,7 +18,7 @@
     const uint32_t t = threadIdx.x, lane = t % kWave, wave = t / kWave;
     const uint32_t per = n > (uint32_t)kThreads ? n / kThreads : 1u;
     const bool mine = t * per < n;
-    uint32_t v[4] = {0u, 0u, 0u, 0u};
+    uint32_t v[(1 << kSortMaxBinBits) / kThreads] = {};
     uint32_t sum = 0;
     if (mine)
         for (uint32_t i = 0; i < per; ++i) {
@@ -148,14 +149,16 @@
     return hipGetLastError();
 }
 
-template <bool kPairs, bool kSide = false>
-__global__ __launch_bounds__(kSortThreads) void bin_partition_kernel(const SortArgs a)
-{
-    __shared__ uint64_t s_rec[kSortTile];
+template <bool kPairs, bool kSide = false, int kThreads = kSortThreads>
+__global__ __launch_bounds__(kThreads) void bin_partition_kernel(const SortArgs a)
+{
+    constexpr int kTile = kThreads * kSortItems;
+    if (kThreads == kSortThreadsSmall) __builtin_amdgcn_s_setprio(3);
+    __shared__ uint64_t s_rec[kTile];
     __shared__ uint32_t s_cnt[(1 << kSortMaxBinBits) + kWave];
     __shared__ uint32_t s_gbase[kPairs ? (1 << kSortMaxBinBits) : 1];
     __shared__ uint32_t s_over[(1 << kSortMaxBinBits) / 32 + 1];
-    __shared__ uint32_t s_wave[kSortThreads / kWave];
+    __shared__ uint32_t s_wave[kThreads / kWave];
     const uint32_t t = threadIdx.x;
     const uint32_t nbins = 1u << a.bin_bits;
     uint32_t tile = blockIdx.x;
@@ -165,17 +168,17 @@
     }
     const uint32_t seg = segment_of_tile(a.seg_tile0, a.n_segs, tile);
     const SortSeg sg = a.segs[seg];
-    const uint32_t first = (tile - a.seg_tile0[seg]) * (uint32_t)kSortTile;
-    const uint32_t n = min(sg.n_in - first, (uint32_t)kSortTile);
-    for (uint32_t b = t; b < nbins + kWave; b += kSortThreads) s_cnt[b] = 0;
-    for (uint32_t b = t; b < (1u << kSortMaxBinBits) / 32u + 1u; b += kSortThreads) s_over[b] = 0;
+    const uint32_t first = (tile - a.seg_tile0[seg]) * (uint32_t)kTile;
+    const uint32_t n = min(sg.n_in - first, (uint32_t)kTile);
+    for (uint32_t b = t; b < nbins + kWave; b += kThreads) s_cnt[b] = 0;
+    for (uint32_t b = t; b < (1u << kSortMaxBinBits) / 32u + 1u; b += kThreads) s_over[b] = 0;
     block_sync();
     uint64_t r[kSortItems];
     uint32_t bin[kSortItems];
     uint32_t side[kSide ? kSortItems : 1];
 #pragma unroll
     for (int k = 0; k < kSortItems; ++k) {
-        const uint32_t i = tile_record(k, t);
+        const uint32_t i = tile_record<kThreads>(k, t);
         const bool in_tile = i < n;
         const uint64_t at = sg.in_off + first + (in_tile ? i : 0u);
         if (kSide) side[k] = a.side_in[at];
@@ -197,11 +200,11 @@
         bin[k] |= rank << 16;
     }
     block_sync();
-    constexpr int kOwnBins = (1 << kSortMaxBinBits) / kSortThreads;
+    constexpr int kOwnBins = (1 << kSortMaxBinBits) / kThreads;
     uint32_t own_at[kOwnBins];
 #pragma unroll
     for (int j = 0; j < kOwnBins; ++j) {
-        const uint32_t b = t + (uint32_t)j * kSortThreads;
+        const uint32_t b = t + (uint32_t)j * kThreads;
         const uint32_t c = b < nbins ? s_cnt[b] : 0u;
         uint32_t at = c ? atomicAdd(&a.cursor[((size_t)seg << a.bin_bits) + b], c) : 0u;
         if (a.slot_cap && c && at + c > a.slot_cap) {
@@ -212,7 +215,7 @@
         own_at[j] = at;
         if (kPairs && b < nbins) s_gbase[b] = at;
     }
-    const uint32_t total = block_exclusive_scan<kSortThreads>(s_cnt, nbins, s_wave);
+    const uint32_t total = block_exclusive_scan<kThreads>(s_cnt, nbins, s_wave);
 #pragma unroll
     for (int k = 0; k < kSortItems; ++k) {
         const uint32_t slot = s_cnt[bin[k] & 0xFFFFu] + (bin[k] >> 16);
@@ -223,7 +226,7 @@
     if (!kPairs) {
 #pragma unroll
         for (int j = 0; j < kOwnBins; ++j) {
-            const uint32_t b = t + (uint32_t)j * kSortThreads;
+            const uint32_t b = t + (uint32_t)j * kThreads;
             if (b < nbins) s_cnt[b] = own_at[j] - s_cnt[b];
         }
         block_sync();
@@ -234,7 +237,7 @@
 #pragma unroll
         for (int j = 0; j < kSortItems / 2; ++j) slot_bin[j] = 0;
     }
-    for (uint32_t i = t; i < total; i += kSortThreads) {
+    for (uint32_t i = t; i < total; i += kThreads) {
         const uint64_t x = s_rec[i];
         uint32_t b;
         if (kPairs) {
@@ -255,7 +258,7 @@
             a.out[sg.out_off + in_bin] = x;
         }
         if (kSide) {
-            const uint32_t j = i / kSortThreads;
+            const uint32_t j = i / kThreads;
 #pragma unroll
             for (int q = 0; q < kSortItems / 2; ++q)
                 if ((uint32_t)q == (j >> 1)) slot_bin[q] |= b << ((j & 1u) * 16u);
@@ -270,7 +273,7 @@
         block_sync();
 #pragma unroll
         for (int j = 0; j < kSortItems; ++j) {
-            const uint32_t i = t + (uint32_t)j * kSortThreads;
+            const uint32_t i = t + (uint32_t)j * kThreads;
             if (i < total) {
                 const uint32_t b = (slot_bin[j >> 1] >> ((j & 1) * 16)) & 0xFFFFu;
                 const uint32_t in_bin = s_cnt[b] + i;
@@ -289,6 +292,12 @@
 {
     if (args.n_tiles == 0) return hipSuccess;
     const unsigned blocks = args.xcd_tiles ? 8u * args.xcd_tiles : args.n_tiles;
+    if (args.tile_records == (uint32_t)kSortTileSmall) {
+        if (args.pair_keys || args.side_in) return hipErrorInvalidValue;
+        hipLaunchKernelGGL((bin_partition_kernel<false, false, kSortThreadsSmall>), dim3(blocks), dim3(kSortThreadsSmall), 0, stream, args);
+        return hipGetLastError();
+    }
+    if (args.tile_records != 0 && args.tile_records != (uint32_t)kSortTile) return hipErrorInvalidValue;
     if (args.pair_keys)
         hipLaunchKernelGGL(bin_partition_kernel<true>, dim3(blocks), dim3(kSortThreads), 0, stream, args);
     else if (args.side_in)
```
